# zhoujun-7/VPHO

Hardware: AMD Instinct MI355X
Metric: eval images/sec (bs=64, sample_num=100, steps=50); MPJPE delta vs ref (higher is better)
Workload: dtype f32; 1 GPU; vpho_net.forward(mode=predict), README eval config (BASELINE.json configs[1]); per_gpu_batch=64, sample_num=100, sampling_steps=50, topk_hand=30, topk_obj=10, crop=256x256, pipeline_depth=3, parallelism=dp1, score_mfma=f32, conv_mfma=f32, winograd_3x3=True

## Files before the change

include/vpho_hip.h:

```cpp
#ifndef VPHO_HIP_H
#define VPHO_HIP_H

#if defined(__GNUC__) || defined(__clang__)
#define VPHO_API __attribute__((visibility("default")))
#else
#define VPHO_API
#endif

#ifdef __cplusplus
extern "C" {
#endif

VPHO_API const char* vpho_last_error(void);
VPHO_API int vpho_abi_version(void);

VPHO_API int vpho_prof_enable(int kernel_class, int on);
VPHO_API int vpho_prof_collect(int kernel_class, double* total_ms, long long* launches, double* total_flops, double* total_bytes);

typedef struct {
    const float* x; const float* w; const float* bias;
    const float* in_scale; const float* in_shift;
    const float* res; float* y;
    int N, H, W, Cin, x_ld;
    int Cout, KH, KW, stride, pad_y, pad_x, OH, OW;
    long long y_sn, y_sy, y_sx;
    long long r_sn, r_sy, r_sx;
    float in_slope, out_slope;
    int w_ld, splits;
    long long x_split, w_split, y_split;
    const float* gate;
    float gate_slope;
    const int* row_map;
    const int* row_count;
    int rows_hint;
    int rows_scatter;
    const void* w_planes;
    int plane_terms;
    const float* res_up;
    int ru_H, ru_W, ru_ld;
    const float* x2;
    int Cin2, x2_ld, stride2, H2, W2;
    int groups;
    long long x_group, w_group, bias_group, y_group, res_group, x2_group, pre_group, ru_group;
    float* stats;
    int* stats_rows;
    int stats_cap;
    const float* bn_x; const float* bn_mean; const float* bn_invstd; const float* bn_gamma; const float* bn_beta;
} vpho_conv_desc;
VPHO_API int vpho_conv2d_nhwc_f32(const vpho_conv_desc* d, void* stream);
VPHO_API int vpho_conv3x3_winograd_nhwc_f32(const float* x, const float* u, const float* bias, int N, int H, int W, int Cin, int x_ld, int Cout,
                                   float out_slope, float* y, int y_ld, void* stream);
VPHO_API int vpho_conv3x3_winograd_grouped_nhwc_f32(const float* x, long long x_group, const float* u, const float* bias, int groups, int N, int H, int W,
                                           int Cin, int x_ld, int Cout, float out_slope, float* y, int y_ld, void* stream);
VPHO_API int vpho_winograd_window_tiles_i32(const int* wins, int N, int* tile_base, void* stream);
VPHO_API int vpho_conv3x3_winograd_scatter_nhwc_f32(const float* x, const float* u, const float* bias, int N, int H, int W, int Cin, int x_ld, int Cout,
                                           float out_slope, const int* wins, const int* tile_base, float* y, int y_ld, void* stream);
VPHO_API int vpho_winograd_weights_f32(const float* w_packed, int Cout, int Cin, int for_input_gradient, float* u, void* stream);
VPHO_API int vpho_winograd_weights_multi_f32(const void* segments, int n_segments, long long total_blocks, void* stream);
VPHO_API int vpho_conv3x3_winograd_gate_nhwc_f32(const float* x, const float* u, const float* gate, float gate_slope, int N, int H, int W, int Cin,
                                        int x_ld, int Cout, float* y, int y_ld, void* stream);
VPHO_API int vpho_conv3x3_winograd_stats_nhwc_f32(const float* x, const float* u, const float* bias, int N, int H, int W, int Cin, int x_ld, int Cout,
                                         float out_slope, float* y, int y_ld, float* stats, int stats_cap, int* stats_rows, const float* bn_x,
                                         const float* bn_mean, const float* bn_invstd, const float* bn_gamma, const float* bn_beta,
                                         float gate_slope, void* stream);
VPHO_API int vpho_conv3x3_winograd_rows_nhwc_f32(const float* x, const float* u, const float* bias, int N, int H, int W, int Cin, int x_ld, int Cout,
                                        float out_slope, const int* wins, const int* tile_base, int tiles_hint, float* y_rows, int y_ld,
                                        void* stream);

typedef struct {
    int D, Dp, nheads;
    const float *t_W, *t_w, *t_b, *pe0_w, *pe0_b, *pe2_w, *pe2_b, *w1_t, *w1_p, *w1_f, *b1, *w2, *b2;
    const void* w1_p_split;
    int split_terms;
} vpho_score_weights;

VPHO_API long long vpho_score_workspace_bytes(const vpho_score_weights* w, int bs, int S);

VPHO_API int vpho_score_eval(const vpho_score_weights* w, const float* feat_img, int bs, int S, const float* x, float t,
                    float* out, void* workspace, long long workspace_bytes, void* stream);

typedef struct {
    int nfev;
    int n_accepted, n_rejected;
    int nan_count;
    int status;
    int n_log;
} vpho_ode_stats;

VPHO_API int vpho_ode_sample(const vpho_score_weights* w, const float* feat_img, int bs, int S, const float* init_x,
                    double T0, double eps, int num_steps, double rtol, double atol,
                    void* xs_out, int xs_is_f64, void* x_out, int x_is_f64,
                    void* workspace, long long workspace_bytes,
                    vpho_ode_stats* stats_host, double* step_log_host, int step_log_cap, void* stream);

VPHO_API int vpho_nchw_to_nhwc_f32(const float* x, int N, int C, int H, int W, float* y, int ldy, void* stream);
VPHO_API int vpho_nhwc_to_nchw_f32(const float* x, int N, int H, int W, int C, int ldx, float* y, void* stream);
VPHO_API int vpho_maxpool_nhwc_f32(const float* x, int N, int H, int W, int C, int k, int stride, int pad, float* y, void* stream);
VPHO_API int vpho_resize_bilinear_nhwc_f32(const float* x, int N, int H, int W, int C, int ldx, int OH, int OW,
                                  float* y, int ldy, int c_off, int accumulate, void* stream);
VPHO_API int vpho_roi_align_nhwc_f32(const float* feat, int N, int H, int W, int C, const float* boxes, float spatial_scale,
                            int out_size, const unsigned char* flip_w, float* out, int ldo, int c_off, void* stream);
VPHO_API int vpho_roi_windows_i32(const float* boxes_a, const float* boxes_b, int N, int H, int W, float spatial_scale, int dilate,
                         int* wins, int* row_map, int* row_count, void* stream);
VPHO_API int vpho_resize_bilinear_rows_nhwc_f32(const float* x, int N, int H, int W, int C, int ldx, int OH, int OW, float* y, int ldy, int c_off,
                                       int accumulate, const int* row_map, const int* row_count, int rows_hint, void* stream);
VPHO_API int vpho_roi_align_window_nhwc_f32(const float* feat_rows, const int* wins, int N, int H, int W, int C, const float* boxes,
                                   float spatial_scale, int out_size, const unsigned char* flip_w, float* out, int ldo, int c_off, int rows_hint,
                                   void* stream);
VPHO_API int vpho_roi_align_window_dual_nhwc_f32(const float* feat_rows, const int* wins, int N, int H, int W, int C, const float* boxes,
                                        float spatial_scale, int out_size, const unsigned char* flip_w, float* out, int ldo, int c_off,
                                        const unsigned char* flip_w2, float* out2, int ldo2, int c_off2, int rows_hint, void* stream);
VPHO_API int vpho_align_heatmap_nhwc_f32(const float* hm, int N, int size, int C, const float* bbox, const float* bbox_rect,
                                const unsigned char* flip_w, float* out, void* stream);
VPHO_API int vpho_linear_acc64_f32(const float* x, int rows, int cin, int ld_x, const float* w, const float* bias, int cout, float out_slope,
                          float* y, int ld_y, void* stream);
VPHO_API int vpho_nerf_embed_f32(const float* g, int N, const unsigned char* flip_x, float* out, void* stream);
VPHO_API int vpho_cross_tokens_f32(const float* proj_hand, const float* proj_obj, const float* grav_emb, const float* pe,
                          int bs, float* out, void* stream);
VPHO_API int vpho_mha_f32(const float* qkv, int S, int B, int E, int nhead, float* out, void* stream);
VPHO_API int vpho_mha_dropout_f32(const float* qkv, int S, int B, int E, int nhead, const float* drop_mask, float* out, void* stream);
VPHO_API int vpho_add_layernorm_f32(const float* x, const float* r, const float* gamma, const float* beta, long long rows, int E,
                           float eps, float* out, void* stream);
VPHO_API int vpho_force_local_f32(const float* scale, int ld_scale, const float* logits, int ld_logits, const float* anchor,
                         float friction, long long rows, int group, int group_stride, int off_scale, int off_logits,
                         float* out, void* stream);
VPHO_API int vpho_rot6d_to_axis_angle_f32(const float* x, long long rows, int rot_per_row, int ldx, float* out, int ldo, void* stream);
VPHO_API int vpho_append_betas_f32(const float* betas, long long rows, long long rows_per_image, float* out, int ldo, void* stream);

typedef struct {
    const float *v_template;
    const float *shapedirs;
    const float *posedirs_t;
    const float *J_regressor;
    const float *weights;
    const float *tip_posedirs_t;
    const float *posedirs_mfma;
} vpho_mano_tables;
VPHO_API int vpho_mano_shape_f32(const vpho_mano_tables* t, const float* betas, int n_img, float* v_shaped, float* J, void* stream);
VPHO_API int vpho_mano_fk_f32(const vpho_mano_tables* t, const float* pose, int ld_pose, long long n_hands, int hands_per_image,
                     const float* v_shaped, const float* J, const unsigned char* ho3d_per_image,
                     float* verts, float* joints, void* stream);

typedef struct { const float* kpt; const float* vert; const float* com; int n_kpt, n_vert, n_obj; } vpho_obj_tables;
typedef struct { const int* face_idx; const float* anchor_weight; const float* vert2joint; const int* skeleton; } vpho_anchor_tables;

VPHO_API int vpho_hand_candidates_f32(const float* diff_pose, int ld_diff, const float* reg_pose, int bs, int S, float* pose, void* stream);
VPHO_API int vpho_hand_heat_f32(const float* joints, const float* root, const float* Kmat, const float* bbox, const float* heatmap,
                       int bs, int C, int J, int H, int W, const int* observe_host, int n_obs, float* out, void* stream);
VPHO_API int vpho_hand_fuse_level_f32(const float* hv, int n_obs, float* pose, int bs, int C, int k, int level,
                             float* val, int* idx, float* topk_pose, float* score_out, void* stream);
VPHO_API int vpho_topk_f32(const float* scores, int rows_outer, int n, int F, int k, float* val, int* idx, void* stream);
VPHO_API int vpho_topk_weights_f32(const float* val, int rows, int k, float* w, void* stream);
VPHO_API int vpho_obj_heat_score(const double* pose, int n, const double* transl_override, const float* root, const vpho_obj_tables* t,
                        const int* obj_id, const unsigned char* is_right, const float* Kmat, const float* bbox,
                        const float* heatmap, int bs, int H, int W, float* score, void* stream);
VPHO_API int vpho_obj_cross_candidates(const double* pose, int n, const int* transl_idx, const int* rot_idx, int bs, int ko, double* cand, void* stream);
VPHO_API int vpho_obj_physics_score(const double* cand, int n, const float* root, const vpho_obj_tables* t, const int* obj_id,
                           const unsigned char* is_right, const float* force_point, const float* force_global, int bs,
                           float* score, void* stream);
VPHO_API int vpho_obj_fuse_f64(const double* pose, int n, const int* idx_a, const float* w_a, const int* idx_b, const float* w_b,
                      const unsigned char* pick_b, int bs, int k, double* fused, void* stream);
VPHO_API int vpho_obj_verts_f32(const double* pose, const float* root, const vpho_obj_tables* t, const int* obj_id,
                       const unsigned char* is_right, int bs, float* out, void* stream);
VPHO_API int vpho_force_anchor_f32(const vpho_anchor_tables* t, const float* verts, const float* root, const float* force_local,
                          long long n_hands, int hands_per_image, float* force_point, float* force_global, void* stream);
VPHO_API int vpho_hand_phys_candidates_f32(const float* agg_pose, int ld_agg, const float* betas, const float* topk_pose, int bs, int k,
                                  float* out, void* stream);
VPHO_API int vpho_hand_phys_score_f32(const float* force_point, const float* force_global, const float* obj_vert, int n_vert,
                             int bs, int n_cand, float* finger_score, void* stream);
VPHO_API int vpho_hand_phys_fuse_f32(const float* cand, int n_cand, const int* idx, int bs, int k, float* out, void* stream);

VPHO_API int vpho_heatmap_peak_f32(const float* heatmap, long long n_maps, int H, int W, float* peak, int* ind, void* stream);
VPHO_API int vpho_hand_pt2d_score_f32(const float* joints, const float* root, const float* Kmat, const float* bbox, const float* peak,
                             int bs, int C, int per_joint, float* score, void* stream);
VPHO_API int vpho_obj_pt2d_score(const double* pose, int n, const float* root, const vpho_obj_tables* t, const int* obj_id,
                        const unsigned char* is_right, const float* Kmat, const float* bbox, const float* peak, int bs,
                        float* score, void* stream);
VPHO_API int vpho_hand_pose_fuse_f32(const float* pose, int ld_pose, int C, const int* idx, const float* w, int bs, int n, float* fused,
                            void* stream);
VPHO_API int vpho_hand_joint_gather_mean_f32(const float* joints, const int* idx, int bs, int C, int k, float* fused, void* stream);

VPHO_API int vpho_hand_metrics_f32(const float* pd, const float* gt, int n_img, int n_pts, float* mean_err, float* pa_mean_err,
                          float* per_point, void* stream);

typedef struct vpho_obj_metric_tables {
    const double* bbox3d;
    const double* verts_sampled;
    const double* verts;
    const int* vert_offset;
    const double* diameter;
    int n_obj, n_sampled;
} vpho_obj_metric_tables;
VPHO_API int vpho_obj_9d_to_rt_f64(const double* pose9, const float* root_joint, int n, double* rt, void* stream);
VPHO_API long long vpho_obj_metrics_workspace_bytes(const vpho_obj_metric_tables* t, int n_img, int max_verts);
VPHO_API int vpho_obj_metrics_f64(const vpho_obj_metric_tables* t, const double* pd_rt, const double* gt_rt, const double* cam_intr,
                         const int* obj_id, int n_img, int max_verts, double* out, void* workspace, long long workspace_bytes,
                         void* stream);

VPHO_API int vpho_hand_metrics_multi_f32(const float* pd, const float* gt, const float* root_joint, const unsigned char* is_right, int n_img,
                                int n_hyp, int n_pts, float* mean_err, float* pa_mean_err, void* stream);
VPHO_API long long vpho_obj_metrics_multi_workspace_bytes(const vpho_obj_metric_tables* t, int n_img, int n_hyp, int max_verts);
VPHO_API int vpho_obj_metrics_multi_f64(const vpho_obj_metric_tables* t, const double* pd_rt, const double* gt_rt, const double* cam_intr,
                               const int* obj_id, int n_img, int n_hyp, int max_verts, double* out, double* best, double* mean,
                               void* workspace, long long workspace_bytes, void* stream);

VPHO_API int vpho_hand_bench_multi_f32(const float* pd, const float* gt, const float* root_joint, const unsigned char* is_right, int n_img,
                              int n_hyp, int n_pts, double f_thresh_lo, double f_thresh_hi, const double* auc_thresh, const double* auc_g,
                              int n_thresh, int with_fscore, double* values, int* counts, void* stream);
VPHO_API int vpho_hand_bench_table_f64(const double* per, int n_img, int n_hyp, double* one, double* best, double* mean, void* stream);

VPHO_API long long vpho_infer_record_bytes(int n_joint, int n_vert);
VPHO_API int vpho_infer_pack_f32(const float* reg_hand_joint, const float* reg_hand_vert, const float* agg_hand_joint, const float* agg_hand_vert,
                        const double* agg_obj_6d, const float* root_joint, const unsigned char* is_right, int n_img, int n_joint,
                        int n_vert, void* records, void* records_host, void* stream);

#define VPHO_PEN_TRI_STRIDE 28
#define VPHO_PEN_RESOLUTION 512
typedef struct vpho_obj_mesh_tables {
    const double* tri;
    const int* tri_offset;
    const double* scale;
    const double* translate;
    int n_obj;
} vpho_obj_mesh_tables;
VPHO_API int vpho_hand_obj_penetration_f64(const vpho_obj_mesh_tables* t, const float* verts, int n, int V, const double* obj_rt,
                                  const int* obj_id, double contact_thresh, double* sd, unsigned char* inside, double* per_image,
                                  void* stream);

#define VPHO_PEN_COLUMNS 64
#define VPHO_PEN_CLUSTER 16
typedef struct vpho_obj_mesh_accel {
    const int* col_offset;
    const int* col_tri;
    const int* clu_offset;
    const double* clu_sphere;
    const double* clu_geo;
} vpho_obj_mesh_accel;
VPHO_API int vpho_hand_obj_penetration_multi_f64(const vpho_obj_mesh_tables* t, const vpho_obj_mesh_accel* acc, const float* verts, int n, int S,
                                        int V, const double* obj_rt, const int* obj_id, double contact_thresh, double* per_hyp,
                                        double* sd, unsigned char* inside, double* table, void* stream);

#define VPHO_VOL_TRI_STRIDE 19
typedef struct vpho_obj_solids {
    const float* pts;
    const int* pt_offset;
    int n_obj, max_pts;
} vpho_obj_solids;
VPHO_API long long vpho_hand_obj_intersection_workspace_bytes(int n, int F);
VPHO_API int vpho_hand_obj_intersection_f64(const vpho_obj_mesh_tables* t, const vpho_obj_solids* solids, const int* faces, int F, const float* verts,
                                   int n, int V, const double* obj_rt, const int* obj_id, double pitch, double* out, unsigned char* flags,
                                   void* workspace, long long workspace_bytes, void* stream);
typedef struct vpho_obj_solid_columns {
    const int* col_start;
    const int* col_offset;
    int n_obj, max_cols;
} vpho_obj_solid_columns;
VPHO_API long long vpho_hand_obj_intersection_multi_workspace_bytes(int n, int S, int F);
VPHO_API int vpho_hand_obj_intersection_multi_f64(const vpho_obj_mesh_tables* t, const vpho_obj_solids* solids, const vpho_obj_solid_columns* cols,
        const int* faces, int F, const float* verts , int n, int S, int V, const double* obj_rt ,
        const int* obj_id , double pitch, double* per_hyp , double* table ,
        unsigned char* flags , void* workspace, long long workspace_bytes, void* stream);

VPHO_API int vpho_anchor_frames_f32(const vpho_anchor_tables* t, const float* verts, long long n_hands, float* pts, float* frames, void* stream);
VPHO_API int vpho_force_optimize_f32(const float* pts, const float* frames, const float* gravity, const float* com, const float* force_contact,
                            const unsigned char* is_grasped, int n_batches, int B, int iters, int phase1_iters, float lr,
                            float* force_local, float* force_global, float* scale, float* weight, float* losses, void* stream);
// ... 84 lines not shown
```

vpho_amd/csrc/metrics.hip:

```cpp
#include <type_traits>
#include "common.h"
#include "rot.h"
#include "procrustes.h"
#include <algorithm>
#include "../../include/vpho_hip.h"

namespace {

using vpho::sym3_eig;
using vpho::wave_sum;
using vpho::similarity_from_cov;

__device__ inline double block_sum(double v, double* red) {
    const int tid = threadIdx.x;
    red[tid] = v;
    __syncthreads();
    for (int o = blockDim.x / 2; o > 0; o >>= 1) {
        if (tid < o) red[tid] += red[tid + o];
        __syncthreads();
    }
    const double r = red[0];
    __syncthreads();
    return r;
}

__global__ __launch_bounds__(256) void hand_metrics_kernel(const float* __restrict__ pd, const float* __restrict__ gt, int n,
                                                           float* __restrict__ mean_err, float* __restrict__ pa_mean_err,
                                                           float* __restrict__ per_point) {
    __shared__ double red[256];
    __shared__ double T[12];
    const int b = blockIdx.x, tid = threadIdx.x;
    const float* A = pd + (long long)b * n * 3;
    const float* B = gt + (long long)b * n * 3;
    double sa[3] = {0, 0, 0}, sb[3] = {0, 0, 0}, se = 0;
    for (int i = tid; i < n; i += 256) {
        double d2 = 0;
        for (int c = 0; c < 3; ++c) { sa[c] += A[i * 3 + c]; sb[c] += B[i * 3 + c]; const double d = (double)B[i * 3 + c] - A[i * 3 + c]; d2 += d * d; }
        const double e = sqrt(d2);
        se += e;
        if (per_point) per_point[(long long)b * n + i] = (float)e;
    }
    double cA[3], cB[3];
    for (int c = 0; c < 3; ++c) { cA[c] = block_sum(sa[c], red) / n; cB[c] = block_sum(sb[c], red) / n; }
    const double me = block_sum(se, red) / n;
    double h[9] = {0}, va = 0;
    for (int i = tid; i < n; i += 256) {
        double a[3], bb[3];
        for (int c = 0; c < 3; ++c) { a[c] = A[i * 3 + c] - cA[c]; bb[c] = B[i * 3 + c] - cB[c]; va += a[c] * a[c]; }
        for (int r = 0; r < 3; ++r) for (int c = 0; c < 3; ++c) h[r * 3 + c] += a[r] * bb[c];
    }
    double H[3][3];
    for (int k = 0; k < 9; ++k) H[k / 3][k % 3] = block_sum(h[k], red) / n;
    const double varA = block_sum(va, red) / n;
    if (tid == 0) {
        double M[3][3], w[3], V[3][3], U[3][3], s[3];
        for (int i = 0; i < 3; ++i) for (int j = 0; j < 3; ++j) { M[i][j] = 0; for (int k = 0; k < 3; ++k) M[i][j] += H[k][i] * H[k][j]; }
        sym3_eig(M, w, V);
        for (int k = 0; k < 3; ++k) s[k] = sqrt(w[k] > 0 ? w[k] : 0.0);
        for (int k = 0; k < 3; ++k) {
            double u[3] = {0, 0, 0};
            for (int i = 0; i < 3; ++i) for (int j = 0; j < 3; ++j) u[i] += H[i][j] * V[j][k];
            const double nu = sqrt(u[0] * u[0] + u[1] * u[1] + u[2] * u[2]);
            if (k < 2 || nu > 1e-12 * (s[0] + 1e-300)) for (int i = 0; i < 3; ++i) U[i][k] = u[i] / (nu > 0 ? nu : 1.0);
            else {
                U[0][2] = U[1][0] * U[2][1] - U[2][0] * U[1][1];
                U[1][2] = U[2][0] * U[0][1] - U[0][0] * U[2][1];
                U[2][2] = U[0][0] * U[1][1] - U[1][0] * U[0][1];
            }
        }
        auto build = [&](double R[3][3]) { for (int i = 0; i < 3; ++i) for (int j = 0; j < 3; ++j) { R[i][j] = 0; for (int k = 0; k < 3; ++k) R[i][j] += V[i][k] * U[j][k]; } };
        double R[3][3];
        build(R);
        const double det = R[0][0] * (R[1][1] * R[2][2] - R[1][2] * R[2][1]) - R[0][1] * (R[1][0] * R[2][2] - R[1][2] * R[2][0]) +
                           R[0][2] * (R[1][0] * R[2][1] - R[1][1] * R[2][0]);
        if (det < 0) { s[2] = -s[2]; for (int i = 0; i < 3; ++i) V[i][2] = -V[i][2]; build(R); }
        const double c = (s[0] + s[1] + s[2]) / varA;
        for (int i = 0; i < 3; ++i) {
            double t = cB[i];
            for (int j = 0; j < 3; ++j) { T[i * 3 + j] = c * R[i][j]; t -= c * R[i][j] * cA[j]; }
            T[9 + i] = t;
        }
    }
    __syncthreads();
    double sp = 0;
    for (int i = tid; i < n; i += 256) {
        double d2 = 0;
        for (int r = 0; r < 3; ++r) {
            const double al = T[r * 3] * A[i * 3] + T[r * 3 + 1] * A[i * 3 + 1] + T[r * 3 + 2] * A[i * 3 + 2] + T[9 + r];
            const double d = (double)B[i * 3 + r] - al;
            d2 += d * d;
        }
        sp += sqrt(d2);
    }
    const double pa = block_sum(sp, red) / n;
    if (tid == 0) { mean_err[b] = (float)me; pa_mean_err[b] = (float)pa; }
}

__global__ void obj_9d_to_rt_kernel(const double* __restrict__ pose9, const float* __restrict__ root, int n, double* __restrict__ rt) {
    const int i = blockIdx.x * blockDim.x + threadIdx.x;
    if (i >= n) return;
    vpho::obj_9d_to_rt(pose9 + (long long)i * 9, root + (long long)i * 3, rt + (long long)i * 12);
}

struct ObjWs { float *pd_s, *gt_s, *pd_f, *gt_f, *d_s, *d_p2g, *d_g2p; long long bytes; };

__host__ __device__ inline long long ows_align(long long v) { return (v + 255) / 256 * 256; }

inline ObjWs obj_carve(int n_img, int ns, int vmax, char* base) {
    long long off = 0;
    ObjWs w;
    auto take = [&](long long b) { char* p = base ? base + off : nullptr; off += ows_align(b); return (float*)p; };
    w.pd_s = take((long long)n_img * ns * 12); w.gt_s = take((long long)n_img * ns * 12);
    w.pd_f = take((long long)n_img * vmax * 12); w.gt_f = take((long long)n_img * vmax * 12);
    w.d_s = take((long long)n_img * ns * 4); w.d_p2g = take((long long)n_img * vmax * 4); w.d_g2p = take((long long)n_img * vmax * 4);
    w.bytes = off;
    return w;
}

__device__ inline void rt_apply(const double* rt, const double* v, double* o) {
    for (int r = 0; r < 3; ++r) o[r] = v[0] * rt[r * 4 + 0] + v[1] * rt[r * 4 + 1] + v[2] * rt[r * 4 + 2] + rt[r * 4 + 3];
}

__global__ __launch_bounds__(256) void obj_transform_kernel(const vpho_obj_metric_tables t, const double* __restrict__ pd_rt,
                                                            const double* __restrict__ gt_rt, const int* __restrict__ obj_id,
                                                            int vmax, ObjWs w) {
    const int b = blockIdx.x, o = obj_id[b];
    const int nf = t.vert_offset[o + 1] - t.vert_offset[o];
    const int i = blockIdx.y * 256 + threadIdx.x;
    if (i >= t.n_sampled + nf) return;
    const bool full = i >= t.n_sampled;
    const int k = full ? i - t.n_sampled : i;
    const double* v = full ? t.verts + ((long long)t.vert_offset[o] + k) * 3 : t.verts_sampled + ((long long)o * t.n_sampled + k) * 3;
    double p[3], g[3];
    rt_apply(pd_rt + (long long)b * 12, v, p);
    rt_apply(gt_rt + (long long)b * 12, v, g);
    float* po = full ? w.pd_f + ((long long)b * vmax + k) * 3 : w.pd_s + ((long long)b * t.n_sampled + k) * 3;
    float* go = full ? w.gt_f + ((long long)b * vmax + k) * 3 : w.gt_s + ((long long)b * t.n_sampled + k) * 3;
    for (int c = 0; c < 3; ++c) { po[c] = (float)p[c]; go[c] = (float)g[c]; }
}

__global__ __launch_bounds__(256) void obj_nn_kernel(const vpho_obj_metric_tables t, const int* __restrict__ obj_id, int vmax, ObjWs w) {
    __shared__ float tile[256 * 3];
    const int b = blockIdx.x, job = blockIdx.y, o = obj_id[b];
    const int n = job == 0 ? t.n_sampled : t.vert_offset[o + 1] - t.vert_offset[o];
    const int ld = job == 0 ? t.n_sampled : vmax;
    const float* src = (job == 0 ? w.pd_s : job == 1 ? w.pd_f : w.gt_f) + (long long)b * ld * 3;
    const float* dst = (job == 0 ? w.gt_s : job == 1 ? w.gt_f : w.pd_f) + (long long)b * ld * 3;
    float* out = (job == 0 ? w.d_s : job == 1 ? w.d_p2g : w.d_g2p) + (long long)b * ld;
    if (blockIdx.z * 256 >= n) return;
    const int i = blockIdx.z * 256 + threadIdx.x;
    const bool live = i < n;
    const float x = live ? src[i * 3] : 0.f, y = live ? src[i * 3 + 1] : 0.f, z = live ? src[i * 3 + 2] : 0.f;
    float best = INFINITY;
    for (int j0 = 0; j0 < n; j0 += 256) {
        const int m = min(256, n - j0);
        __syncthreads();
        for (int q = threadIdx.x; q < m * 3; q += 256) tile[q] = dst[(long long)j0 * 3 + q];
        __syncthreads();
        for (int j = 0; j < m; ++j) {
            const float dx = x - tile[j * 3], dy = y - tile[j * 3 + 1], dz = z - tile[j * 3 + 2];
            const float d2 = (dx * dx + dy * dy) + dz * dz;
            best = d2 < best ? d2 : best;
        }
    }
    if (live) out[i] = sqrtf(best);
}

__device__ inline float block_minmax(float v, bool is_max, float* red) {
    const int tid = threadIdx.x;
    red[tid] = v;
    __syncthreads();
    for (int o = blockDim.x / 2; o > 0; o >>= 1) {
        if (tid < o) red[tid] = is_max ? fmaxf(red[tid], red[tid + o]) : fminf(red[tid], red[tid + o]);
        __syncthreads();
    }
    const float r = red[0];
    __syncthreads();
    return r;
// ... 292 lines not shown
    }
    double s_add = 0, s_rep = 0;
    float mn[2][3], mx[2][3];
    for (int c = 0; c < 3; ++c) { mn[0][c] = mn[1][c] = INFINITY; mx[0][c] = mx[1][c] = -INFINITY; }
    for (int i = tid; i < ns; i += 256) {
        double p[3], g[3], pp[2], gp[2];
        const double* v = t.verts_sampled + ((long long)o * ns + i) * 3;
        rt_apply(prt, v, p);
        rt_apply(grt, v, g);
        float pf[3], gf[3];
        for (int c = 0; c < 3; ++c) { pf[c] = (float)p[c]; gf[c] = (float)g[c]; }
        const float dx = pf[0] - gf[0], dy = pf[1] - gf[1], dz = pf[2] - gf[2];
        s_add += (double)sqrtf((dx * dx + dy * dy) + dz * dz);
        for (int c = 0; c < 3; ++c) {
            mn[0][c] = fminf(mn[0][c], pf[c]); mx[0][c] = fmaxf(mx[0][c], pf[c]);
            mn[1][c] = fminf(mn[1][c], gf[c]); mx[1][c] = fmaxf(mx[1][c], gf[c]);
        }
        for (int r = 0; r < 2; ++r) {
            pp[r] = (p[0] * K[r * 3] + p[1] * K[r * 3 + 1] + p[2] * K[r * 3 + 2]) / (p[2] + 1e-7);
            gp[r] = (g[0] * K[r * 3] + g[1] * K[r * 3 + 1] + g[2] * K[r * 3 + 2]) / (g[2] + 1e-7);
        }
        s_rep += sqrt((pp[0] - gp[0]) * (pp[0] - gp[0]) + (pp[1] - gp[1]) * (pp[1] - gp[1]));
    }
    const double add = block_sum(s_add, red) / ns, rep = block_sum(s_rep, red) / ns;
    float bmn[2][3], bmx[2][3];
    for (int k = 0; k < 2; ++k)
        for (int c = 0; c < 3; ++c) { bmn[k][c] = block_minmax(mn[k][c], false, redf); bmx[k][c] = block_minmax(mx[k][c], true, redf); }
    if (tid == 0) {
        double acc[3][7];
        for (int j = 0; j < 3; ++j)
            for (int c = 0; c < 7; ++c) {
                double a = 0;
                for (int q = 0; q < w.chunks; ++q) a += w.part[(((long long)bs * 3 + j) * w.chunks + q) * 8 + c];
                acc[j][c] = a;
            }
        const double adds = acc[0][0] / ns, mp = acc[1][0] / nf, mg = acc[2][0] / nf;
        const int sel[3][8] = {{0, 1, 0, 0, 1, 0, 1, 1}, {0, 0, 1, 0, 1, 1, 0, 1}, {0, 0, 0, 1, 0, 1, 1, 1}};
        float s2 = 0.f;
        for (int k = 0; k < 8; ++k) {
            float d2 = 0.f;
            for (int c = 0; c < 3; ++c) {
                const float a = sel[c][k] ? bmx[0][c] : bmn[0][c], g = sel[c][k] ? bmx[1][c] : bmn[1][c];
                d2 += (a - g) * (a - g);
            }
            s2 += sqrtf(d2);
        }
        const double diam = t.diameter[o];
        double* r = out + (long long)bs * 16;
        r[0] = mce; r[1] = oce; r[2] = (double)(s2 / 8.f); r[3] = add; r[4] = adds;
        r[5] = add <= diam * 0.1 ? 1.0 : 0.0; r[6] = adds <= diam * 0.1 ? 1.0 : 0.0; r[7] = rep; r[8] = rep < 5 ? 1.0 : 0.0;
        r[9] = 0.5 * (mp + mg);
        for (int k = 0; k < 6; ++k) {
            const float prec = (float)(acc[1][1 + k] / nf), rec = (float)(acc[2][1 + k] / nf);
            r[10 + k] = (double)((2.f * prec * rec) / ((prec + rec) + 1e-6f));
        }
    }
}

__global__ void obj_multi_reduce_kernel(const double* __restrict__ per, int n_img, int S, double* __restrict__ best, double* __restrict__ mean) {
    const int i = blockIdx.x * blockDim.x + threadIdx.x;
    if (i >= n_img * 16) return;
    const int b = i / 16, c = i % 16;
    const bool is_max = c == 5 || c == 6 || c == 8 || c >= 10;
    const double* p = per + (long long)b * S * 16 + c;
    double bv = p[0], sv = p[0];
    for (int s = 1; s < S; ++s) {
        const double v = p[(long long)s * 16];
        bv = is_max ? (v > bv ? v : bv) : (v < bv ? v : bv);
        sv += v;
    }
    if (best) best[i] = bv;
    if (mean) mean[i] = sv / S;
}

}

extern "C" int vpho_hand_metrics_f32(const float* pd, const float* gt, int n_img, int n_pts, float* mean_err, float* pa_mean_err,
                                     float* per_point, void* stream) {
    VPHO_REQUIRE(pd && gt && mean_err && pa_mean_err && n_img > 0 && n_pts >= 3, "vpho_hand_metrics_f32: bad argument");
    hipLaunchKernelGGL(hand_metrics_kernel, dim3(n_img), dim3(256), 0, (hipStream_t)stream, pd, gt, n_pts, mean_err, pa_mean_err, per_point);
    return vpho::check_launch("hand_metrics_kernel");
}

extern "C" long long vpho_obj_metrics_workspace_bytes(const vpho_obj_metric_tables* t, int n_img, int max_verts) {
    if (!t || n_img <= 0 || max_verts <= 0 || t->n_sampled <= 0) return -1;
    return obj_carve(n_img, t->n_sampled, max_verts, nullptr).bytes;
}

extern "C" int vpho_obj_metrics_f64(const vpho_obj_metric_tables* t, const double* pd_rt, const double* gt_rt, const double* cam_intr,
                                    const int* obj_id, int n_img, int max_verts, double* out, void* workspace, long long workspace_bytes,
                                    void* stream) {
    VPHO_REQUIRE(t && t->bbox3d && t->verts_sampled && t->verts && t->vert_offset && t->diameter && t->n_obj > 0 && t->n_sampled > 0,
                 "vpho_obj_metrics_f64: bad tables");
    VPHO_REQUIRE(pd_rt && gt_rt && cam_intr && obj_id && out && workspace && n_img > 0 && max_verts > 0, "vpho_obj_metrics_f64: bad argument");
    const ObjWs w = obj_carve(n_img, t->n_sampled, max_verts, (char*)workspace);
    VPHO_REQUIRE(workspace_bytes >= w.bytes, "vpho_obj_metrics_f64: workspace %lld < %lld bytes", workspace_bytes, w.bytes);
    hipStream_t s = (hipStream_t)stream;
    const int pts = t->n_sampled + max_verts;
    hipLaunchKernelGGL(obj_transform_kernel, dim3(n_img, (pts + 255) / 256), dim3(256), 0, s, *t, pd_rt, gt_rt, obj_id, max_verts, w);
    const int chunks = (std::max(t->n_sampled, max_verts) + 255) / 256;
    hipLaunchKernelGGL(obj_nn_kernel, dim3(n_img, 3, chunks), dim3(256), 0, s, *t, obj_id, max_verts, w);
    hipLaunchKernelGGL(obj_metrics_kernel, dim3(n_img), dim3(256), 0, s, *t, pd_rt, gt_rt, cam_intr, obj_id, max_verts, w, out);
    return vpho::check_launch("obj_metrics kernels");
}

extern "C" int vpho_obj_9d_to_rt_f64(const double* pose9, const float* root_joint, int n, double* rt, void* stream) {
    VPHO_REQUIRE(pose9 && root_joint && rt && n > 0, "vpho_obj_9d_to_rt_f64: bad argument");
    hipLaunchKernelGGL(obj_9d_to_rt_kernel, dim3((n + 255) / 256), dim3(256), 0, (hipStream_t)stream, pose9, root_joint, n, rt);
    return vpho::check_launch("obj_9d_to_rt_kernel");
}

extern "C" int vpho_hand_metrics_multi_f32(const float* pd, const float* gt, const float* root_joint, const unsigned char* is_right, int n_img,
                                           int n_hyp, int n_pts, float* mean_err, float* pa_mean_err, void* stream) {
    VPHO_REQUIRE(pd && gt && root_joint && is_right && mean_err && pa_mean_err && n_img > 0 && n_hyp > 0 && n_pts >= 3 &&
                 (long long)n_img * n_hyp <= 0x7fffffff, "vpho_hand_metrics_multi_f32: bad argument");
    hipLaunchKernelGGL(hand_metrics_multi_kernel, dim3(n_img * n_hyp), dim3(64), 0, (hipStream_t)stream, pd, gt, root_joint, is_right, n_hyp,
                       n_pts, mean_err, pa_mean_err);
    return vpho::check_launch("hand_metrics_multi_kernel");
}

extern "C" long long vpho_obj_metrics_multi_workspace_bytes(const vpho_obj_metric_tables* t, int n_img, int n_hyp, int max_verts) {
    if (!t || n_img <= 0 || n_hyp <= 0 || max_verts <= 0 || t->n_sampled <= 0 || (long long)n_img * n_hyp > 0x7fffffff) return -1;
    return mh_carve(n_img, n_hyp, t->n_sampled, max_verts, nullptr).bytes;
}

extern "C" int vpho_obj_metrics_multi_f64(const vpho_obj_metric_tables* t, const double* pd_rt, const double* gt_rt, const double* cam_intr,
                                          const int* obj_id, int n_img, int n_hyp, int max_verts, double* out, double* best, double* mean,
                                          void* workspace, long long workspace_bytes, void* stream) {
    VPHO_REQUIRE(t && t->bbox3d && t->verts_sampled && t->verts && t->vert_offset && t->diameter && t->n_obj > 0 && t->n_sampled > 0,
                 "vpho_obj_metrics_multi_f64: bad tables");
    VPHO_REQUIRE(pd_rt && gt_rt && cam_intr && obj_id && out && workspace && n_img > 0 && n_hyp > 0 && max_verts > 0 &&
                 (long long)n_img * n_hyp <= 0x7fffffff, "vpho_obj_metrics_multi_f64: bad argument");
    const MhWs w = mh_carve(n_img, n_hyp, t->n_sampled, max_verts, (char*)workspace);
    VPHO_REQUIRE(workspace_bytes >= w.bytes, "vpho_obj_metrics_multi_f64: workspace %lld < %lld bytes", workspace_bytes, w.bytes);
    VPHO_REQUIRE(w.chunks <= 65535, "vpho_obj_metrics_multi_f64: %d query chunks exceed the grid", w.chunks);
    hipStream_t s = (hipStream_t)stream;
    const int rows = n_img * n_hyp;
    hipLaunchKernelGGL(obj_multi_nn_kernel, dim3(rows, 3, w.chunks), dim3(256), 0, s, *t, pd_rt, gt_rt, obj_id, n_hyp, w);
    hipLaunchKernelGGL(obj_multi_metrics_kernel, dim3(rows), dim3(256), 0, s, *t, pd_rt, gt_rt, cam_intr, obj_id, n_hyp, w, out);
    if (best || mean)
        hipLaunchKernelGGL(obj_multi_reduce_kernel, dim3((n_img * 16 + 255) / 256), dim3(256), 0, s, out, n_img, n_hyp, best, mean);
    return vpho::check_launch("obj_metrics_multi kernels");
}
```

vpho_amd/csrc/misc.hip:

```cpp
#include "common.h"
#include <cstdint>
#include "rot.h"
#include "../../include/vpho_hip.h"

namespace {

inline int nblocks(long long n, int bs = 256) { return (int)((n + bs - 1) / bs); }

__global__ void nchw_to_nhwc_kernel(const float* __restrict__ x, int N, int C, int H, int W, float* __restrict__ y, int ldy) {
    const long long i = (long long)blockIdx.x * blockDim.x + threadIdx.x;
    const long long total = (long long)N * H * W * ldy;
    if (i >= total) return;
    const int c = (int)(i % ldy);
    const long long p = i / ldy;
    const long long hw = (long long)H * W;
    const long long n = p / hw, r = p - n * hw;
    y[i] = c < C ? x[(n * C + c) * hw + r] : 0.f;
}

__global__ void nhwc_to_nchw_kernel(const float* __restrict__ x, int N, int H, int W, int C, int ldx, float* __restrict__ y) {
    const long long i = (long long)blockIdx.x * blockDim.x + threadIdx.x;
    const long long hw = (long long)H * W, total = (long long)N * C * hw;
    if (i >= total) return;
    const long long r = i % hw;
    const long long nc = i / hw;
    const int c = (int)(nc % C);
    const long long n = nc / C;
    y[i] = x[(n * hw + r) * ldx + c];
}

__global__ void maxpool_nhwc_kernel(const float* __restrict__ x, int N, int H, int W, int C, int k, int stride, int pad,
                                    int OH, int OW, float* __restrict__ y) {
    const long long i = (long long)blockIdx.x * blockDim.x + threadIdx.x;
    const long long total = (long long)N * OH * OW * C;
    if (i >= total) return;
    const int c = (int)(i % C);
    long long p = i / C;
    const int ox = (int)(p % OW); p /= OW;
    const int oy = (int)(p % OH);
    const long long n = p / OH;
    float m = -INFINITY;
    for (int r = 0; r < k; ++r) {
        const int iy = oy * stride - pad + r;
        if (iy < 0 || iy >= H) continue;
        for (int s = 0; s < k; ++s) {
            const int ix = ox * stride - pad + s;
            if (ix < 0 || ix >= W) continue;
            m = fmaxf(m, x[((n * H + iy) * W + ix) * C + c]);
        }
    }
    y[i] = m;
}


template <int V>
__device__ inline void ldv(const float* __restrict__ p, float (&o)[V]) {
    if constexpr (V == 4) { const f32x4 t = *reinterpret_cast<const f32x4*>(p); o[0] = t[0]; o[1] = t[1]; o[2] = t[2]; o[3] = t[3]; }
    else o[0] = *p;
}
template <int V>
__device__ inline void stv(float* __restrict__ p, const float (&v)[V]) {
    if constexpr (V == 4) { f32x4 t; t[0] = v[0]; t[1] = v[1]; t[2] = v[2]; t[3] = v[3]; *reinterpret_cast<f32x4*>(p) = t; }
    else *p = v[0];
}

template <int V>
__global__ void resize_bilinear_nhwc_kernel(const float* __restrict__ x, int N, int H, int W, int C, int ldx, int OH, int OW,
                                            float* __restrict__ y, int ldy, int c_off, int accumulate,
                                            const int* __restrict__ row_map, const int* __restrict__ row_count) {
    const long long i = (long long)blockIdx.x * blockDim.x + threadIdx.x;
    const int CV = C / V;
    const long long total = (long long)N * OH * OW * CV;
    if (i >= total) return;
    const int c = (int)(i % CV) * V;
    long long p = i / CV;
    if (row_map) {
        if (p >= *row_count) return;
        p = row_map[p];
    }
    const int ox = (int)(p % OW); p /= OW;
    const int oy = (int)(p % OH);
    const long long n = p / OH;
    int y0, y1, x0, x1; float ly, lx;
    lin_src(oy, (float)H / (float)OH, H, y0, y1, ly);
    lin_src(ox, (float)W / (float)OW, W, x0, x1, lx);
    const float hy = 1.f - ly, hx = 1.f - lx;
    const float* b = x + n * H * W * (long long)ldx + c;
    float a00[V], a01[V], a10[V], a11[V], o[V];
    ldv<V>(b + ((long long)y0 * W + x0) * ldx, a00); ldv<V>(b + ((long long)y0 * W + x1) * ldx, a01);
    ldv<V>(b + ((long long)y1 * W + x0) * ldx, a10); ldv<V>(b + ((long long)y1 * W + x1) * ldx, a11);
    float* op = y + ((n * OH + oy) * OW + ox) * (long long)ldy + c_off + c;
    if (accumulate) ldv<V>(op, o);
#pragma unroll
    for (int u = 0; u < V; ++u) {
        const float v = hy * (hx * a00[u] + lx * a01[u]) + ly * (hx * a10[u] + lx * a11[u]);
        o[u] = accumulate ? (o[u] + v) : v;
    }
    stv<V>(op, o);
}

struct RoiWin { int base, y0, x0, w, h; };

template <int V>
__device__ inline void roi_bilinear(const float* __restrict__ f, int H, int W, int ld, float y, float x, float (&acc)[V],
                                    const RoiWin* win = nullptr) {
    if (y < -1.0f || y > (float)H || x < -1.0f || x > (float)W) {
#pragma unroll
        for (int u = 0; u < V; ++u) acc[u] += 0.f;
        return;
    }
    if (y <= 0.f) y = 0.f;
    if (x <= 0.f) x = 0.f;
    int yl = (int)y, xl = (int)x, yh, xh;
    if (yl >= H - 1) { yh = yl = H - 1; y = (float)yl; } else yh = yl + 1;
    if (xl >= W - 1) { xh = xl = W - 1; x = (float)xl; } else xh = xl + 1;
    const float ly = y - (float)yl, lx = x - (float)xl, hy = 1.f - ly, hx = 1.f - lx;
    float a[V], b[V], c[V], d[V];
    if (win) {
        const int wy0 = min(max(yl - win->y0, 0), win->h - 1), wy1 = min(max(yh - win->y0, 0), win->h - 1);
        const int wx0 = min(max(xl - win->x0, 0), win->w - 1), wx1 = min(max(xh - win->x0, 0), win->w - 1);
        ldv<V>(f + ((long long)wy0 * win->w + wx0) * ld, a); ldv<V>(f + ((long long)wy0 * win->w + wx1) * ld, b);
        ldv<V>(f + ((long long)wy1 * win->w + wx0) * ld, c); ldv<V>(f + ((long long)wy1 * win->w + wx1) * ld, d);
    } else {
        ldv<V>(f + ((long long)yl * W + xl) * ld, a); ldv<V>(f + ((long long)yl * W + xh) * ld, b);
        ldv<V>(f + ((long long)yh * W + xl) * ld, c); ldv<V>(f + ((long long)yh * W + xh) * ld, d);
    }
#pragma unroll
    for (int u = 0; u < V; ++u) acc[u] += hy * hx * a[u] + hy * lx * b[u] + ly * hx * c[u] + ly * lx * d[u];
}

template <int V>
__global__ void roi_align_nhwc_kernel(const float* __restrict__ feat, int N, int H, int W, int C, const float* __restrict__ boxes,
                                      float scale, int P, const unsigned char* __restrict__ flip_w,
                                      float* __restrict__ out, int ldo, int c_off, const RoiWin* __restrict__ wins,
                                      float* __restrict__ out2 = nullptr, int ldo2 = 0, int c_off2 = 0, const unsigned char* __restrict__ flip_w2 = nullptr) {
    const long long i = (long long)blockIdx.x * blockDim.x + threadIdx.x;
    const int CV = C / V;
    const long long total = (long long)N * P * P * CV;
    if (i >= total) return;
    const int c = (int)(i % CV) * V;
    long long p = i / CV;
    const int pw = (int)(p % P); p /= P;
    const int ph = (int)(p % P);
    const int n = (int)(p / P);
    const float x1 = boxes[n * 4 + 0] * scale, y1 = boxes[n * 4 + 1] * scale;
    const float x2 = boxes[n * 4 + 2] * scale, y2 = boxes[n * 4 + 3] * scale;
    const float rw = fmaxf(x2 - x1, 1.f), rh = fmaxf(y2 - y1, 1.f);
    const float bh = rh / (float)P, bw = rw / (float)P;
    const int gh = (int)ceilf(rh / (float)P), gw = (int)ceilf(rw / (float)P);
    const float cnt = fmaxf((float)(gh * gw), 1.f);
    RoiWin win;
    if (wins) win = wins[n];
    const float* f = feat + (wins ? (long long)win.base : (long long)n * H * W) * C + c;
    float acc[V];
#pragma unroll
    for (int u = 0; u < V; ++u) acc[u] = 0.f;
    for (int iy = 0; iy < gh; ++iy) {
        const float y = y1 + ph * bh + ((float)iy + 0.5f) * bh / (float)gh;
        for (int ix = 0; ix < gw; ++ix) {
            const float x = x1 + pw * bw + ((float)ix + 0.5f) * bw / (float)gw;
            roi_bilinear<V>(f, H, W, C, y, x, acc, wins ? &win : nullptr);
        }
    }
    const int ow = (flip_w && flip_w[n]) ? P - 1 - pw : pw;
#pragma unroll
    for (int u = 0; u < V; ++u) acc[u] = acc[u] / cnt;
    stv<V>(out + (((long long)n * P + ph) * P + ow) * ldo + c_off + c, acc);
    if (out2) {
        const int ow2 = (flip_w2 && flip_w2[n]) ? P - 1 - pw : pw;
        stv<V>(out2 + (((long long)n * P + ph) * P + ow2) * ldo2 + c_off2 + c, acc);
    }
}

__global__ __launch_bounds__(256) void roi_window_kernel(const float* __restrict__ boxes_a, const float* __restrict__ boxes_b, int N, int H, int W,
                                                         float scale, int dilate, RoiWin* __restrict__ wins, int* __restrict__ count) {
    for (int n0 = 0; n0 < N; n0 += 256) {
        const int n = n0 + threadIdx.x;
        if (n < N) {
            float lo_x = 3.0e38f, lo_y = 3.0e38f, hi_x = -3.0e38f, hi_y = -3.0e38f;
            for (int k = 0; k < 2; ++k) {
                const float* b = k == 0 ? boxes_a : boxes_b;
// ... 276 lines not shown
                                   const float* __restrict__ anchor, float friction, long long rows, int group, int group_stride,
                                   int off_scale, int off_logits, float* __restrict__ out) {
    const long long r = (long long)blockIdx.x * blockDim.x + threadIdx.x;
    if (r >= rows) return;
    const long long base = (r / group) * group_stride + r % group;
    const long long rs = base + off_scale, rl = base + off_logits;
    float w[8];
    for (int pass = 0; pass < 2; ++pass) {
        float mx = -INFINITY;
        for (int i = 0; i < 8; ++i) { if (pass == 0) w[i] = logits[rl * ld_logits + i]; mx = fmaxf(mx, w[i]); }
        float s = 0.f;
        for (int i = 0; i < 8; ++i) { w[i] = expf(w[i] - mx); s += w[i]; }
        for (int i = 0; i < 8; ++i) w[i] /= s;
    }
    float d[3] = {0.f, 0.f, 0.f};
    for (int i = 0; i < 8; ++i) {
        d[0] += w[i] * (anchor[i * 3 + 0] * friction);
        d[1] += w[i] * (anchor[i * 3 + 1] * friction);
        d[2] += w[i] * anchor[i * 3 + 2];
    }
    const float nrm = sqrtf(d[0] * d[0] + d[1] * d[1] + d[2] * d[2]) + 1e-8f;
    const float sc = fabsf(scale[rs * ld_scale]);
    for (int k = 0; k < 3; ++k) out[r * 3 + k] = d[k] / nrm * sc;
}

__global__ void rot6d_to_aa_kernel(const float* __restrict__ x, long long n_rot, int rot_per_row, int ldx, float* __restrict__ out, int ldo) {
    const long long i = (long long)blockIdx.x * blockDim.x + threadIdx.x;
    if (i >= n_rot) return;
    const long long row = i / rot_per_row;
    const int j = (int)(i - row * rot_per_row);
    float R[9], q[4], aa[3];
    vpho::rot6d_to_matrix(x + row * ldx + 6 * j, R);
    vpho::matrix_to_quaternion(R, q);
    vpho::quaternion_to_axis_angle(q, aa);
    float* o = out + row * ldo + 3 * j;
    o[0] = aa[0]; o[1] = aa[1]; o[2] = aa[2];
}

__global__ void append_betas_kernel(const float* __restrict__ betas, long long rows, long long rows_per_image, float* __restrict__ out, int ldo) {
    const long long i = (long long)blockIdx.x * blockDim.x + threadIdx.x;
    if (i >= rows * 10) return;
    const long long row = i / 10;
    const int k = (int)(i - row * 10);
    out[row * ldo + 48 + k] = betas[(row / rows_per_image) * 10 + k];
}

}

#define LAUNCH1D(kernel, total, stream, ...) \
    hipLaunchKernelGGL(kernel, dim3(nblocks(total)), dim3(256), 0, (hipStream_t)(stream), __VA_ARGS__)

extern "C" int vpho_nchw_to_nhwc_f32(const float* x, int N, int C, int H, int W, float* y, int ldy, void* stream) {
    VPHO_REQUIRE(x && y && N > 0 && C > 0 && H > 0 && W > 0 && ldy >= C, "vpho_nchw_to_nhwc_f32: bad argument");
    LAUNCH1D(nchw_to_nhwc_kernel, (long long)N * H * W * ldy, stream, x, N, C, H, W, y, ldy);
    return vpho::check_launch("nchw_to_nhwc_kernel");
}

extern "C" int vpho_nhwc_to_nchw_f32(const float* x, int N, int H, int W, int C, int ldx, float* y, void* stream) {
    VPHO_REQUIRE(x && y && N > 0 && C > 0 && H > 0 && W > 0 && ldx >= C, "vpho_nhwc_to_nchw_f32: bad argument");
    LAUNCH1D(nhwc_to_nchw_kernel, (long long)N * H * W * C, stream, x, N, H, W, C, ldx, y);
    return vpho::check_launch("nhwc_to_nchw_kernel");
}

extern "C" int vpho_maxpool_nhwc_f32(const float* x, int N, int H, int W, int C, int k, int stride, int pad, float* y, void* stream) {
    VPHO_REQUIRE(x && y && N > 0 && C > 0 && k > 0 && stride > 0 && pad >= 0 && 2 * pad <= k, "vpho_maxpool_nhwc_f32: bad argument");
    const int OH = (H + 2 * pad - k) / stride + 1, OW = (W + 2 * pad - k) / stride + 1;
    VPHO_REQUIRE(OH > 0 && OW > 0, "vpho_maxpool_nhwc_f32: empty output");
    LAUNCH1D(maxpool_nhwc_kernel, (long long)N * OH * OW * C, stream, x, N, H, W, C, k, stride, pad, OH, OW, y);
    return vpho::check_launch("maxpool_nhwc_kernel");
}

extern "C" int vpho_resize_bilinear_nhwc_f32(const float* x, int N, int H, int W, int C, int ldx, int OH, int OW,
                                             float* y, int ldy, int c_off, int accumulate, void* stream) {
    VPHO_REQUIRE(x && y && N > 0 && C > 0 && H > 0 && W > 0 && OH > 0 && OW > 0 && ldx >= C && ldy >= c_off + C && c_off >= 0,
                 "vpho_resize_bilinear_nhwc_f32: bad argument");
    vpho::ProfScope prof(vpho::PROF_RESIZE, (hipStream_t)stream, 0.0, 4.0 * N * C * ((double)H * W + (double)OH * OW * (accumulate ? 2 : 1)));
    if (C % 4 == 0 && ldx % 4 == 0 && ldy % 4 == 0 && c_off % 4 == 0 && ((uintptr_t)x | (uintptr_t)y) % 16 == 0)
        LAUNCH1D(resize_bilinear_nhwc_kernel<4>, (long long)N * OH * OW * (C / 4), stream, x, N, H, W, C, ldx, OH, OW, y, ldy, c_off, accumulate, (const int*)nullptr, (const int*)nullptr);
    else
        LAUNCH1D(resize_bilinear_nhwc_kernel<1>, (long long)N * OH * OW * C, stream, x, N, H, W, C, ldx, OH, OW, y, ldy, c_off, accumulate, (const int*)nullptr, (const int*)nullptr);
    return vpho::check_launch("resize_bilinear_nhwc_kernel");
}

extern "C" int vpho_resize_bilinear_rows_nhwc_f32(const float* x, int N, int H, int W, int C, int ldx, int OH, int OW, float* y, int ldy, int c_off,
                                                  int accumulate, const int* row_map, const int* row_count, int rows_hint, void* stream) {
    VPHO_REQUIRE(x && y && row_map && row_count && N > 0 && H > 0 && W > 0 && C > 0 && OH > 0 && OW > 0 && ldx >= C && ldy >= c_off + C && c_off >= 0,
                 "vpho_resize_bilinear_rows_nhwc_f32: bad argument");
    const double px = rows_hint > 0 ? (double)rows_hint : (double)N * OH * OW;
    vpho::ProfScope prof(vpho::PROF_RESIZE, (hipStream_t)stream, 0.0, 4.0 * C * ((double)N * H * W + px * (accumulate ? 2 : 1)));
    if (C % 4 == 0 && ldx % 4 == 0 && ldy % 4 == 0 && c_off % 4 == 0 && ((uintptr_t)x | (uintptr_t)y) % 16 == 0)
        LAUNCH1D(resize_bilinear_nhwc_kernel<4>, (long long)N * OH * OW * (C / 4), stream, x, N, H, W, C, ldx, OH, OW, y, ldy, c_off, accumulate, row_map, row_count);
    else
        LAUNCH1D(resize_bilinear_nhwc_kernel<1>, (long long)N * OH * OW * C, stream, x, N, H, W, C, ldx, OH, OW, y, ldy, c_off, accumulate, row_map, row_count);
    return vpho::check_launch("resize_bilinear_nhwc_kernel(rows)");
}

extern "C" int vpho_roi_align_nhwc_f32(const float* feat, int N, int H, int W, int C, const float* boxes, float spatial_scale,
                                       int out_size, const unsigned char* flip_w, float* out, int ldo, int c_off, void* stream) {
    VPHO_REQUIRE(feat && boxes && out && N > 0 && C > 0 && out_size > 0 && ldo >= c_off + C && c_off >= 0, "vpho_roi_align_nhwc_f32: bad argument");
    vpho::ProfScope prof(vpho::PROF_ROI_ALIGN, (hipStream_t)stream, 0.0, 4.0 * N * C * ((double)H * W + (double)out_size * out_size));
    if (C % 4 == 0 && ldo % 4 == 0 && c_off % 4 == 0 && ((uintptr_t)feat | (uintptr_t)out) % 16 == 0)
        LAUNCH1D(roi_align_nhwc_kernel<4>, (long long)N * out_size * out_size * (C / 4), stream, feat, N, H, W, C, boxes, spatial_scale, out_size, flip_w, out, ldo, c_off, (const RoiWin*)nullptr);
    else
        LAUNCH1D(roi_align_nhwc_kernel<1>, (long long)N * out_size * out_size * C, stream, feat, N, H, W, C, boxes, spatial_scale, out_size, flip_w, out, ldo, c_off, (const RoiWin*)nullptr);
    return vpho::check_launch("roi_align_nhwc_kernel");
}

extern "C" int vpho_roi_windows_i32(const float* boxes_a, const float* boxes_b, int N, int H, int W, float spatial_scale, int dilate,
                                    int* wins, int* row_map, int* row_count, void* stream) {
    VPHO_REQUIRE(boxes_a && wins && row_map && row_count && N > 0 && H > 0 && W > 0 && dilate >= 0, "vpho_roi_windows_i32: bad argument");
    VPHO_REQUIRE((long long)N * H * W < (1ll << 31), "vpho_roi_windows_i32: map too large");
    static_assert(sizeof(RoiWin) == 5 * sizeof(int), "window record = 5 ints");
    hipStream_t s = (hipStream_t)stream;
    hipLaunchKernelGGL(roi_window_kernel, dim3(1), dim3(256), 0, s, boxes_a, boxes_b, N, H, W, spatial_scale, dilate, (RoiWin*)wins, row_count);
    hipLaunchKernelGGL(roi_rows_kernel, dim3((H * W + 255) / 256, N), dim3(256), 0, s, (const RoiWin*)wins, H, W, row_map);
    return vpho::check_launch("roi_window_kernel");
}

extern "C" int vpho_roi_align_window_nhwc_f32(const float* feat_rows, const int* wins, int N, int H, int W, int C, const float* boxes,
                                              float spatial_scale, int out_size, const unsigned char* flip_w, float* out, int ldo, int c_off,
                                              int rows_hint, void* stream) {
    VPHO_REQUIRE(feat_rows && wins && boxes && out && N > 0 && C > 0 && out_size > 0 && ldo >= c_off + C && c_off >= 0, "vpho_roi_align_window_nhwc_f32: bad argument");
    const double rows_read = rows_hint > 0 ? (double)rows_hint : (double)N * H * W;
    vpho::ProfScope prof(vpho::PROF_ROI_ALIGN, (hipStream_t)stream, 0.0, 4.0 * C * (rows_read + (double)N * out_size * out_size));
    if (C % 4 == 0 && ldo % 4 == 0 && c_off % 4 == 0 && ((uintptr_t)feat_rows | (uintptr_t)out) % 16 == 0)
        LAUNCH1D(roi_align_nhwc_kernel<4>, (long long)N * out_size * out_size * (C / 4), stream, feat_rows, N, H, W, C, boxes, spatial_scale, out_size, flip_w, out, ldo, c_off, (const RoiWin*)wins);
    else
        LAUNCH1D(roi_align_nhwc_kernel<1>, (long long)N * out_size * out_size * C, stream, feat_rows, N, H, W, C, boxes, spatial_scale, out_size, flip_w, out, ldo, c_off, (const RoiWin*)wins);
    return vpho::check_launch("roi_align_nhwc_kernel(window)");
}

extern "C" int vpho_roi_align_window_dual_nhwc_f32(const float* feat_rows, const int* wins, int N, int H, int W, int C, const float* boxes,
                                                   float spatial_scale, int out_size, const unsigned char* flip_w, float* out, int ldo, int c_off,
                                                   const unsigned char* flip_w2, float* out2, int ldo2, int c_off2, int rows_hint, void* stream) {
    VPHO_REQUIRE(feat_rows && wins && boxes && out && out2 && N > 0 && C > 0 && out_size > 0 && ldo >= c_off + C && c_off >= 0 && ldo2 >= c_off2 + C && c_off2 >= 0,
                 "vpho_roi_align_window_dual_nhwc_f32: bad argument");
    const double rows_read = rows_hint > 0 ? (double)rows_hint : (double)N * H * W;
    vpho::ProfScope prof(vpho::PROF_ROI_ALIGN, (hipStream_t)stream, 0.0, 4.0 * C * (rows_read + 2.0 * N * out_size * out_size));
    if (C % 4 == 0 && ldo % 4 == 0 && c_off % 4 == 0 && ldo2 % 4 == 0 && c_off2 % 4 == 0 && ((uintptr_t)feat_rows | (uintptr_t)out | (uintptr_t)out2) % 16 == 0)
        LAUNCH1D(roi_align_nhwc_kernel<4>, (long long)N * out_size * out_size * (C / 4), stream, feat_rows, N, H, W, C, boxes, spatial_scale, out_size, flip_w, out, ldo, c_off, (const RoiWin*)wins, out2, ldo2, c_off2, flip_w2);
    else
        LAUNCH1D(roi_align_nhwc_kernel<1>, (long long)N * out_size * out_size * C, stream, feat_rows, N, H, W, C, boxes, spatial_scale, out_size, flip_w, out, ldo, c_off, (const RoiWin*)wins, out2, ldo2, c_off2, flip_w2);
    return vpho::check_launch("roi_align_nhwc_kernel(window, two destinations)");
}

extern "C" int vpho_align_heatmap_nhwc_f32(const float* hm, int N, int size, int C, const float* bbox, const float* bbox_rect,
                                           const unsigned char* flip_w, float* out, void* stream) {
    VPHO_REQUIRE(hm && bbox && bbox_rect && out && N > 0 && size > 1 && C > 0, "vpho_align_heatmap_nhwc_f32: bad argument");
    LAUNCH1D(align_heatmap_kernel, (long long)N * size * size * C, stream, hm, N, size, C, bbox, bbox_rect, flip_w, out);
    return vpho::check_launch("align_heatmap_kernel");
}

extern "C" int vpho_nerf_embed_f32(const float* g, int N, const unsigned char* flip_x, float* out, void* stream) {
    VPHO_REQUIRE(g && out && N > 0, "vpho_nerf_embed_f32: bad argument");
    LAUNCH1D(nerf_embed_kernel, (long long)N * 64, stream, g, N, flip_x, out);
    return vpho::check_launch("nerf_embed_kernel");
}

extern "C" int vpho_cross_tokens_f32(const float* proj_hand, const float* proj_obj, const float* grav_emb, const float* pe,
                                     int bs, float* out, void* stream) {
    VPHO_REQUIRE(proj_hand && proj_obj && grav_emb && pe && out && bs > 0 && bs <= 5000, "vpho_cross_tokens_f32: bad argument");
    LAUNCH1D(cross_tokens_kernel, (long long)bs * 65 * 512, stream, proj_hand, proj_obj, grav_emb, pe, bs, out);
    return vpho::check_launch("cross_tokens_kernel");
}

extern "C" int vpho_mha_dropout_f32(const float* qkv, int S, int B, int E, int nhead, const float* drop_mask, float* out, void* stream) {
// ... 77 lines not shown
```

vpho_amd/csrc/score_ode.hip:

```cpp
#include "common.h"
#include <type_traits>
#include "../../include/vpho_hip.h"
#include <cmath>
#include <cstdlib>
#include <cstring>
#include <vector>
#include <mutex>
#include <unordered_map>
#include <algorithm>

VPHO_STAMP_DECL(head)

namespace {

#ifndef HEAD_ABLATE
#define HEAD_ABLATE 0
#endif
constexpr int HB_K = 16;
constexpr double SIGMA_MIN = 0.01, SIGMA_MAX = 50.0;

struct TimeList { float t[8]; };

struct RkCtl {
    double t, h_abs, h, t_new, err, dense_h;
// ... 954 lines not shown
    const int row = r0 + lrow_out;
    const bool live = row < a.R;
    const float* cim = a.cimg + (long long)(live ? row / a.S : 0) * a.NH + n * 256;
    float o0 = 0.f, o1 = 0.f, o2 = 0.f;
#pragma unroll
    for (int i = 0; i < TI; ++i) {
#pragma unroll
        for (int e = 0; e < 16; ++e) {
            const int j = 32 * TI * hh + 32 * i + (e & 3) + 8 * (e >> 2) + 4 * lh;
            const f32x4 t = *reinterpret_cast<const f32x4*>(Eb + j * 4);
            float h = acc[i][e] + cim[j] + t[0];
            h = h > 0.f ? h : 0.f;
            o0 += h * t[1]; o1 += h * t[2]; o2 += h * t[3];
        }
    }
    o0 += __shfl_xor(o0, 32);
    o1 += __shfl_xor(o1, 32);
    o2 += __shfl_xor(o2, 32);
    if (lh == 0) {
        float* ob = Ob + (hh * ROWS + lrow_out) * 4;
        ob[0] = o0; ob[1] = o1; ob[2] = o2;
    }
    __syncthreads();
    if (tid < ROWS) {
        const int orow = r0 + tid;
        float inv_std = a.inv_std_den, coef = a.coef;
        float* outp = a.out;
        if (a.ctl && a.ctl_mode == 1) {
            inv_std = a.ctl->inv_std[a.stage]; coef = a.ctl->coef[a.stage];
            outp = a.kbase + (long long)kslot(a.out_slot, a.ctl->kswap) * a.n_el;
        }
        if (orow < a.R) {
            int nans = 0;
#pragma unroll
            for (int dd = 0; dd < 3; ++dd) {
                float acc2 = Ob[tid * 4 + dd];
#pragma unroll
                for (int part = 1; part < PARTS; ++part) acc2 += Ob[(part * ROWS + tid) * 4 + dd];
                float sv = (acc2 + a.b2[n * 3 + dd]) / inv_std;
                if (a.rhs_mode) {
                    if (sv != sv) { sv = 0.f; ++nans; } else if (fabsf(sv) == INFINITY) sv = 0.f;
                    sv = 0.f - coef * sv;
                }
                outp[(long long)orow * a.D + n * 3 + dd] = sv;
            }
            if (nans) atomicAdd(a.nan_count, nans);
        }
    }
}

template <int TERMS>
__global__ __launch_bounds__(512) void score_head_split_kernel(const HeadArgs a) {
    extern __shared__ __attribute__((aligned(1024))) float smem[];
    if (ctl_skip(a.ctl, a.ctl_mode)) return;
    const int b = blockIdx.x, n_full = a.nheads * a.full_tiles;
    if (b < n_full) {
        head_tile_split<4, TERMS>(a, smem, b / a.full_tiles, (b % a.full_tiles) * 128);
    } else {
        const int q = b - n_full;
        head_tile_split<1, TERMS>(a, smem, q / a.tail_tiles, a.full_tiles * 128 + (q % a.tail_tiles) * 32);
    }
}

__global__ void stage_input_kernel(const double* __restrict__ y, KSlots ks, long long n_el, int D, int Dp,
                                   LinComb lc, float* __restrict__ X, double* __restrict__ ynew,
                                   const RkCtl* __restrict__ ctl, int ctl_mode, const double* ybuf0, const double* ybuf1) {
    if (ctl_skip(ctl, ctl_mode)) return;
    if (ctl && ctl_mode == 1) lc.h = ctl->h;
    if (ctl && ctl_mode == 2) y = ctl->parity ? ybuf1 : ybuf0;
    const long long i = (long long)blockIdx.x * blockDim.x + threadIdx.x;
    const long long R = n_el / D;
    if (i >= R * Dp) return;
    const long long r = i / Dp;
    const int c = (int)(i - r * Dp);
    if (c >= D) { X[i] = 0.f; return; }
    const long long e = r * D + c;
    double s = 0.0;
    for (int j = 0; j < lc.n; ++j) s += (double)ks.p[j][e] * lc.c[j];
    const double v = y[e] + s * lc.h;
    X[i] = (float)v;
    if (ynew) ynew[e] = v;
}

__global__ void f32_to_state_kernel(const float* __restrict__ x, long long n_el, int D, int Dp, double* __restrict__ y, float* __restrict__ X) {
    const long long i = (long long)blockIdx.x * blockDim.x + threadIdx.x;
    const long long R = n_el / D;
    if (i >= R * Dp) return;
    const long long r = i / Dp;
    const int c = (int)(i - r * Dp);
    if (c >= D) { X[i] = 0.f; return; }
    const float v = x[r * D + c];
    y[r * D + c] = (double)v;
    X[i] = v;
}

struct NormArgs {
    const double* y; const double* ynew; const float* Ka; const float* Kb; KSlots ks; long long n_el;
    double rtol, atol, h; double E[7]; int mode; double* partial;
    const RkCtl* ctl; const float* kbase; const double *ybuf0, *ybuf1;
};
__global__ __launch_bounds__(256) void norm_partial_kernel(const NormArgs a) {
    __shared__ double red[256];
    double s = 0.0;
    if (ctl_skip(a.ctl, 1)) return;
    KSlots ks = a.ks;
    const double *yv = a.y, *yn = a.ynew;
    double h = a.h;
    if (a.ctl) {
        const int par = a.ctl->parity, sw = a.ctl->kswap;
        yv = par ? a.ybuf1 : a.ybuf0; yn = par ? a.ybuf0 : a.ybuf1; h = a.ctl->h;
#pragma unroll
        for (int j = 0; j < 7; ++j) ks.p[j] = a.kbase + (long long)kslot(j, sw) * a.n_el;
    }
    for (long long i = (long long)blockIdx.x * 256 + threadIdx.x; i < a.n_el; i += (long long)gridDim.x * 256) {
        double v, scale;
        if (a.mode == 3) {
            double e = 0.0;
            for (int j = 0; j < 7; ++j) e += (double)ks.p[j][i] * a.E[j];
            v = e * h;
            scale = a.atol + fmax(fabs(yv[i]), fabs(yn[i])) * a.rtol;
        } else {
            scale = a.atol + fabs(yv[i]) * a.rtol;
            v = a.mode == 0 ? yv[i] : (a.mode == 1 ? (double)a.Ka[i] : (double)a.Kb[i] - (double)a.Ka[i]);
        }
        const double q = v / scale;
        s += q * q;
    }
    red[threadIdx.x] = s;
    __syncthreads();
    for (int o = 128; o > 0; o >>= 1) {
        if (threadIdx.x < o) red[threadIdx.x] += red[threadIdx.x + o];
        __syncthreads();
    }
    if (threadIdx.x == 0) a.partial[blockIdx.x] = red[0];
}
__global__ __launch_bounds__(256) void norm_final_kernel(const double* __restrict__ partial, int n, double* __restrict__ out,
                                                         const RkCtl* __restrict__ ctl) {
    __shared__ double red[256];
    if (ctl_skip(ctl, 1)) return;
    double s = 0.0;
    for (int i = threadIdx.x; i < n; i += 256) s += partial[i];
    red[threadIdx.x] = s;
    __syncthreads();
    for (int o = 128; o > 0; o >>= 1) {
        if (threadIdx.x < o) red[threadIdx.x] += red[threadIdx.x + o];
        __syncthreads();
    }
    if (threadIdx.x == 0) *out = red[0];
}

constexpr int DENSE_MAX = 48;
struct DenseArgs { double P[7][4]; double p[DENSE_MAX][4]; int idx[DENSE_MAX]; int n; double h; };
__global__ void dense_kernel(const double* __restrict__ y_old, KSlots ks, long long n_el, int D,
                             DenseArgs da, void* __restrict__ xs, int is_f64, int num_steps) {
    const long long i = (long long)blockIdx.x * blockDim.x + threadIdx.x;
    if (i >= n_el) return;
    double q[4];
    for (int m = 0; m < 4; ++m) {
        double s = 0.0;
        for (int j = 0; j < 7; ++j) s += (double)ks.p[j][i] * da.P[j][m];
        q[m] = s;
    }
    const double y0 = y_old[i];
    const long long r = i / D;
    const int c = (int)(i - r * D);
    for (int st = 0; st < da.n; ++st) {
        double acc = 0.0;
        for (int m = 0; m < 4; ++m) acc += q[m] * da.p[st][m];
        const double v = da.h * acc + y0;
        const long long o = (r * num_steps + da.idx[st]) * D + c;
        if (is_f64) reinterpret_cast<double*>(xs)[o] = v; else reinterpret_cast<float*>(xs)[o] = (float)v;
    }
}

// ... 119 lines not shown
__global__ void dense_ctl_kernel(const RkCtl* __restrict__ c, const double* ybuf0, const double* ybuf1, const float* __restrict__ kbase,
                                 long long n_el, int D, DenseP dp, void* __restrict__ xs, int is_f64, int num_steps) {
    const int first = c->dense_first, last = c->dense_last;
    if (first >= last) return;
    const long long i = (long long)blockIdx.x * blockDim.x + threadIdx.x;
    if (i >= n_el) return;
    const double* y_old = c->dense_parity ? ybuf1 : ybuf0;
    const int sw = c->dense_kswap;
    double q[4];
    for (int m = 0; m < 4; ++m) {
        double s = 0.0;
        for (int j = 0; j < 7; ++j) s += (double)kbase[(long long)kslot(j, sw) * n_el + i] * dp.P[j][m];
        q[m] = s;
    }
    const double y0 = y_old[i], h = c->dense_h;
    const long long r = i / D;
    const int cc = (int)(i - r * D);
    for (int st = first; st < last; ++st) {
        const double* p = c->dense_p + 4 * st;
        double acc = 0.0;
        for (int m = 0; m < 4; ++m) acc += q[m] * p[m];
        const double v = h * acc + y0;
        const long long o = (r * num_steps + st) * D + cc;
        if (is_f64) reinterpret_cast<double*>(xs)[o] = v; else reinterpret_cast<float*>(xs)[o] = (float)v;
    }
}

inline long long align_up(long long v) { return (v + 255) / 256 * 256; }

struct Workspace {
    float *cimg, *ct, *X, *P1, *P2, *K, *tmp;
    double *y, *ynew, *partial, *result;
    int* nan_count;
    RkCtl* ctl; double *te, *dense_p, *log;
    long long bytes;
};
constexpr int CTL_MAX_STEPS = 1024, CTL_LOG_CAP = 512;

Workspace carve(const vpho_score_weights& w, int bs, int S, char* base) {
    const long long R = (long long)bs * S, NH = (long long)w.nheads * 256;
    long long off = 0;
    Workspace ws;
    auto take = [&](long long b) { char* p = base ? base + off : nullptr; off += align_up(b); return p; };
    ws.cimg = (float*)take(bs * NH * 4);
    ws.ct = (float*)take(8 * NH * 4);
    ws.X = (float*)take(R * w.Dp * 4);
    ws.P1 = (float*)take(R * 256 * 4);
    ws.P2 = (float*)take(R * 256 * 4);
    ws.K = (float*)take(7 * R * w.D * 4);
    ws.tmp = (float*)take(R * w.D * 4);
    ws.y = (double*)take(R * w.D * 8);
    ws.ynew = (double*)take(R * w.D * 8);
    ws.partial = (double*)take(1024 * 8);
    ws.result = (double*)take(64);
    ws.nan_count = (int*)take(64);
    ws.ctl = (RkCtl*)take(sizeof(RkCtl));
    ws.te = (double*)take(CTL_MAX_STEPS * 8);
    ws.dense_p = (double*)take(CTL_MAX_STEPS * 4 * 8);
    ws.log = (double*)take(CTL_LOG_CAP * 4 * 8);
    ws.bytes = off;
    return ws;
}

int check_weights(const vpho_score_weights* w) {
    VPHO_REQUIRE(w != nullptr, "score weights: null");
    VPHO_REQUIRE(w->nheads > 0 && w->D == w->nheads * 3 && w->Dp >= w->D && w->Dp % 4 == 0, "score weights: D=%d Dp=%d nheads=%d inconsistent", w->D, w->Dp, w->nheads);
    VPHO_REQUIRE(w->t_W && w->t_w && w->t_b && w->pe0_w && w->pe0_b && w->pe2_w && w->pe2_b && w->w1_t && w->w1_p && w->w1_f && w->b1 && w->w2 && w->b2, "score weights: null tensor");
    return 0;
}

int linear(const float* x, int rows, int cin, const float* wt, const float* bias, int cout, float slope, float* y, hipStream_t s) {
    vpho_conv_desc d;
    memset(&d, 0, sizeof(d));
    d.x = x; d.w = wt; d.bias = bias; d.y = y;
    d.N = rows; d.H = 1; d.W = 1; d.Cin = cin; d.x_ld = cin; d.Cout = cout; d.KH = 1; d.KW = 1; d.stride = 1;
    d.OH = 1; d.OW = 1; d.y_sx = cout; d.y_sy = cout; d.y_sn = cout; d.in_slope = 1.f; d.out_slope = slope;
    return vpho_conv2d_nhwc_f32(&d, s);
}

float sigma_f32(float t) { return (float)SIGMA_MIN * (float)std::pow(SIGMA_MAX / SIGMA_MIN, (double)t); }

struct Ctx {
    const vpho_score_weights* w; Workspace ws; int bs, S; long long R, n_el; int NH; hipStream_t s;
};

int prepare_cimg(Ctx& c, const float* feat_img) {
    return linear(feat_img, c.bs, 1024, c.w->w1_f, c.w->b1, c.NH, 1.f, c.ws.cimg, c.s);
}

int embed_times(Ctx& c, const float* ts, int n, int ctl_mode = 0) {
    TimeList tl;
    for (int i = 0; i < 8; ++i) tl.t[i] = (ts && i < n) ? ts[i] : 0.f;
    hipLaunchKernelGGL(time_embed_kernel, dim3((c.NH + 255) / 256, n), dim3(256), 0, c.s, *c.w, tl, c.NH, c.ws.ct,
                       ctl_mode ? c.ws.ctl : (const RkCtl*)nullptr, ctl_mode);
    return vpho::check_launch("time_embed_kernel");
}

struct CtlCall { int mode = 0, stage = 0, out_slot = 0, write_ynew = 0; };

int eval_net(Ctx& c, const float* X, float t, int rhs_mode, float coef, float* out, int ct_slot = -1,
             const LinComb* lc = nullptr, const double* y = nullptr, double* ynew = nullptr, const KSlots* ks = nullptr,
             CtlCall cc = CtlCall()) {
    if (ct_slot < 0) {
        if (int e = embed_times(c, &t, 1, cc.mode == 2 ? 2 : 0)) return e;
        ct_slot = 0;
    }
    {
        PoseEncArgs pa;
        memset(&pa, 0, sizeof(pa));
        pa.X = X; pa.Dp = c.w->Dp; pa.w0 = c.w->pe0_w; pa.b0 = c.w->pe0_b; pa.w2 = c.w->pe2_w; pa.b2 = c.w->pe2_b;
        pa.out = c.ws.P2; pa.R = (int)c.R;
        if (lc) { pa.use_lc = 1; pa.lc = *lc; pa.y = y; if (ks) pa.ks = *ks; pa.D = c.w->D; pa.ynew = ynew; }
        pa.ctl = cc.mode ? c.ws.ctl : nullptr; pa.ctl_mode = cc.mode; pa.write_ynew = cc.write_ynew; pa.kbase = c.ws.K; pa.n_el = c.n_el;
        pa.ybuf0 = c.ws.y; pa.ybuf1 = c.ws.ynew;
        const int K1 = (pa.Dp + 31) / 32 * 32;
        const char* pe_env = getenv("VPHO_PE_RING");
        const bool pe_ring = pe_env && atoi(pe_env);
        const dim3 pe_grid((unsigned)((c.R + PE_ROWS - 1) / PE_ROWS));
        vpho::ProfScope pe_prof(vpho::PROF_POSE_ENC, c.s, 2.0 * (double)c.R * 256.0 * (K1 + 256.0), 0.0);
        if (pe_ring) {
            const size_t pe_lds = (size_t)(PE_NST * PE_STAGE + PE_ROWS * PE_H_LD + 512 + PE_ROWS * (K1 + 4)) * sizeof(float);
            VPHO_DYN_LDS(pose_encoder_kernel, 150 * 1024);
            VPHO_REQUIRE(pe_lds <= 150 * 1024, "pose encoder: input dimension %d too large for the LDS tile", pa.Dp);
            hipLaunchKernelGGL(pose_encoder_kernel, pe_grid, dim3(512), pe_lds, c.s, pa);
        } else {
            const size_t pe_lds = (size_t)(PE_ROWS * PE_H_LD + 512) * sizeof(float);
            VPHO_REQUIRE(K1 <= 128 && (pa.Dp & 3) == 0, "pose encoder: input dimension %d (padded %d) not supported (<= 128, multiple of 4)", c.w->D, pa.Dp);
            const char* rows_env = getenv("VPHO_PE_ROWS");
            const bool rows64 = rows_env ? atoi(rows_env) == 64 : c.R > 8192;
            if (rows64) {
                const size_t lds64 = (size_t)(2 * PE_ROWS * PE_H_LD + 512) * sizeof(float);
                const dim3 grid64((unsigned)((c.R + 2 * PE_ROWS - 1) / (2 * PE_ROWS)));
                VPHO_DYN_LDS(pose_encoder_reg64_kernel<1>, lds64); VPHO_DYN_LDS(pose_encoder_reg64_kernel<2>, lds64);
                VPHO_DYN_LDS(pose_encoder_reg64_kernel<3>, lds64); VPHO_DYN_LDS(pose_encoder_reg64_kernel<4>, lds64);
                switch (K1 / 32) {
                    case 1: hipLaunchKernelGGL(pose_encoder_reg64_kernel<1>, grid64, dim3(512), lds64, c.s, pa); break;
                    case 2: hipLaunchKernelGGL(pose_encoder_reg64_kernel<2>, grid64, dim3(512), lds64, c.s, pa); break;
                    case 3: hipLaunchKernelGGL(pose_encoder_reg64_kernel<3>, grid64, dim3(512), lds64, c.s, pa); break;
                    default: hipLaunchKernelGGL(pose_encoder_reg64_kernel<4>, grid64, dim3(512), lds64, c.s, pa); break;
                }
            } else
            switch (K1 / 32) {
                case 1: hipLaunchKernelGGL(pose_encoder_reg_kernel<1>, pe_grid, dim3(512), pe_lds, c.s, pa); break;
                case 2: hipLaunchKernelGGL(pose_encoder_reg_kernel<2>, pe_grid, dim3(512), pe_lds, c.s, pa); break;
                case 3: hipLaunchKernelGGL(pose_encoder_reg_kernel<3>, pe_grid, dim3(512), pe_lds, c.s, pa); break;
                default: hipLaunchKernelGGL(pose_encoder_reg_kernel<4>, pe_grid, dim3(512), pe_lds, c.s, pa); break;
            }
        }
        if (int e = vpho::check_launch("pose_encoder_kernel")) return e;
    }
    VPHO_REQUIRE((double)c.R * 256.0 * 4.0 < 4.0e9, "score head: %lld hypothesis rows exceed the 32-bit buffer offsets", (long long)c.R);
    HeadArgs a;
    a.w1p = c.w->w1_p; a.p2 = c.ws.P2; a.cimg = c.ws.cimg; a.ct = c.ws.ct + (long long)ct_slot * c.NH; a.w2 = c.w->w2; a.b2 = c.w->b2;
    a.out = out; a.nan_count = c.ws.nan_count; a.R = (int)c.R; a.S = c.S; a.NH = c.NH; a.D = c.w->D;
    a.inv_std_den = sigma_f32(t) + 1e-7f; a.coef = coef; a.rhs_mode = rhs_mode;
    a.ctl = cc.mode ? c.ws.ctl : nullptr; a.ctl_mode = cc.mode; a.stage = cc.stage; a.out_slot = cc.out_slot; a.kbase = c.ws.K; a.n_el = c.n_el;
    size_t lds = (size_t)(2 * (256 + 128) * HB_K + 256 * 4 + 2 * 128 * 4) * sizeof(float);
    if (getenv("VPHO_HEAD_LDS")) lds = (size_t)atoi(getenv("VPHO_HEAD_LDS"));
    VPHO_DYN_LDS(score_head_kernel<true>, lds);
    VPHO_DYN_LDS(score_head_kernel<false>, lds);
    VPHO_DYN_LDS(score_head_epi0_kernel<true>, lds);
    VPHO_DYN_LDS(score_head_epi0_kernel<false>, lds);
    static const int tail_on = getenv("VPHO_HEAD_TAIL") ? atoi(getenv("VPHO_HEAD_TAIL")) : 1;
    static int slots_of[64] = {0};
    int dev = 0;
    VPHO_HIP(hipGetDevice(&dev));
// ... 37 lines not shown
            return vpho::check_launch("score_head_pers_kernel");
        }
        const char* epi_s = getenv("VPHO_HEAD_EPI");
        if (epi_s && atoi(epi_s) == 0) {
            if (cb) hipLaunchKernelGGL(score_head_epi0_kernel<true>, grid, dim3(512), lds, c.s, a);
            else    hipLaunchKernelGGL(score_head_epi0_kernel<false>, grid, dim3(512), lds, c.s, a);
        } else if (cb) hipLaunchKernelGGL(score_head_kernel<true>, grid, dim3(512), lds, c.s, a);
        else           hipLaunchKernelGGL(score_head_kernel<false>, grid, dim3(512), lds, c.s, a);
    }
    return vpho::check_launch("score_head_kernel");
}

int eval_rhs(Ctx& c, const float* X, double t, float* out, int ct_slot = -1, const LinComb* lc = nullptr,
             const double* y = nullptr, double* ynew = nullptr, const KSlots* ks = nullptr, bool first_call = false) {
    const float tf = (float)t;
    const double sigma = first_call ? (double)sigma_f32(tf) : SIGMA_MIN * std::pow(SIGMA_MAX / SIGMA_MIN, t);
    const double g = sigma * std::sqrt(2.0 * (std::log(SIGMA_MAX) - std::log(SIGMA_MIN)));
    const float coef = (float)(0.5 * g * g);
    return eval_net(c, X, tf, 1, coef, out, ct_slot, lc, y, ynew, ks);
}

double* pinned_slot() {
    static thread_local double* p = nullptr;
    if (!p) { if (hipHostMalloc((void**)&p, 64, hipHostMallocDefault) != hipSuccess) p = nullptr; }
    return p;
}

int enqueue_norm(Ctx& c, NormArgs na, double* out_dev, bool ctl = false) {
    const int nb = (int)std::min<long long>(1024, (c.n_el + 255) / 256);
    na.n_el = c.n_el; na.partial = c.ws.partial;
    na.ctl = ctl ? c.ws.ctl : nullptr; na.kbase = c.ws.K; na.ybuf0 = c.ws.y; na.ybuf1 = c.ws.ynew;
    hipLaunchKernelGGL(norm_partial_kernel, dim3(nb), dim3(256), 0, c.s, na);
    hipLaunchKernelGGL(norm_final_kernel, dim3(1), dim3(256), 0, c.s, c.ws.partial, nb, out_dev, ctl ? c.ws.ctl : (const RkCtl*)nullptr);
    return vpho::check_launch("norm kernels");
}

int reduce_norm(Ctx& c, NormArgs na, double* value) {
    if (int e = enqueue_norm(c, na, c.ws.result)) return e;
    double* h = pinned_slot();
    VPHO_REQUIRE(h != nullptr, "hipHostMalloc failed");
    VPHO_HIP(hipMemcpyAsync(h, c.ws.result, 8, hipMemcpyDeviceToHost, c.s));
    VPHO_HIP(hipStreamSynchronize(c.s));
    *value = std::sqrt(*h) / std::sqrt((double)c.n_el);
    return 0;
}

const double RK_C[6] = {0, 1.0 / 5, 3.0 / 10, 4.0 / 5, 8.0 / 9, 1};
const double RK_A[6][5] = {
    {0, 0, 0, 0, 0},
    {1.0 / 5, 0, 0, 0, 0},
    {3.0 / 40, 9.0 / 40, 0, 0, 0},
    {44.0 / 45, -56.0 / 15, 32.0 / 9, 0, 0},
    {19372.0 / 6561, -25360.0 / 2187, 64448.0 / 6561, -212.0 / 729, 0},
    {9017.0 / 3168, -355.0 / 33, 46732.0 / 5247, 49.0 / 176, -5103.0 / 18656}};
const double RK_B[6] = {35.0 / 384, 0, 500.0 / 1113, 125.0 / 192, -2187.0 / 6784, 11.0 / 84};
const double RK_E[7] = {-71.0 / 57600, 0, 71.0 / 16695, -71.0 / 1920, 17253.0 / 339200, -22.0 / 525, 1.0 / 40};
const double RK_P[7][4] = {
    {1, -8048581381.0 / 2820520608, 8663915743.0 / 2820520608, -12715105075.0 / 11282082432},
    {0, 0, 0, 0},
    {0, 131558114200.0 / 32700410799, -68118460800.0 / 10900136933, 87487479700.0 / 32700410799},
    {0, -1754552775.0 / 470086768, 14199869525.0 / 1410260304, -10690763975.0 / 1880347072},
    {0, 127303824393.0 / 49829197408, -318862633887.0 / 49829197408, 701980252875.0 / 199316789632},
    {0, -282668133.0 / 205662961, 2019193451.0 / 616988883, -1453857185.0 / 822651844},
    {0, 40617522.0 / 29380423, -110615467.0 / 29380423, 69997945.0 / 29380423}};

}

extern "C" long long vpho_score_workspace_bytes(const vpho_score_weights* w, int bs, int S) {
    if (!w || bs <= 0 || S <= 0) return -1;
    return carve(*w, bs, S, nullptr).bytes;
}

extern "C" int vpho_score_eval(const vpho_score_weights* w, const float* feat_img, int bs, int S, const float* x, float t,
                               float* out, void* workspace, long long workspace_bytes, void* stream) {
    if (int e = check_weights(w)) return e;
    VPHO_REQUIRE(bs > 0 && S > 0 && feat_img && x && out && workspace, "vpho_score_eval: bad argument");
    Ctx c;
    c.w = w; c.bs = bs; c.S = S; c.R = (long long)bs * S; c.n_el = c.R * w->D; c.NH = w->nheads * 256; c.s = (hipStream_t)stream;
    c.ws = carve(*w, bs, S, (char*)workspace);
    VPHO_REQUIRE(workspace_bytes >= c.ws.bytes, "vpho_score_eval: workspace %lld < %lld bytes", workspace_bytes, c.ws.bytes);
    VPHO_HIP(hipMemsetAsync(c.ws.nan_count, 0, 4, c.s));
    if (int e = prepare_cimg(c, feat_img)) return e;
    const int nb = (int)((c.R * w->Dp + 255) / 256);
    hipLaunchKernelGGL(f32_to_state_kernel, dim3(nb), dim3(256), 0, c.s, x, c.n_el, w->D, w->Dp, c.ws.y, c.ws.X);
    return eval_net(c, c.ws.X, t, 0, 0.f, out);
}

namespace {

int ode_sample_host(Ctx& c, const float* feat_img, const float* init_x, double T0, double eps, int num_steps, double rtol, double atol,
                    void* xs_out, int xs_is_f64, void* x_out, int x_is_f64, vpho_ode_stats* st, double* step_log, int step_log_cap) {
    const vpho_score_weights* w = c.w;
    const long long n_el = c.n_el;
    const int D = w->D, Dp = w->Dp;
    const int nbX = (int)((c.R * Dp + 255) / 256), nbE = (int)((n_el + 255) / 256);
    KSlots ks;
    for (int j = 0; j < 7; ++j) ks.p[j] = c.ws.K + (long long)j * n_el;
    auto Kp = [&](int j) { return const_cast<float*>(ks.p[j]); };

    VPHO_HIP(hipMemsetAsync(c.ws.nan_count, 0, 4, c.s));
    if (int e = prepare_cimg(c, feat_img)) return e;
    double* y = c.ws.y;
    double* ynew = c.ws.ynew;
    hipLaunchKernelGGL(f32_to_state_kernel, dim3(nbX), dim3(256), 0, c.s, init_x, n_el, D, Dp, y, c.ws.X);

    std::vector<double> te(num_steps);
    {
        const int div = num_steps > 1 ? num_steps - 1 : 1;
        const double step = (eps - T0) / div;
        for (int i = 0; i < num_steps; ++i) te[i] = (double)i * step + T0;
        if (num_steps > 1) te[num_steps - 1] = eps;
    }
    const double direction = -1.0, tf = eps, max_step = 10.0;
    double t = T0;
    int next_idx = 0;
    auto log_step = [&](double tt, double hh, double err, int acc) {
        if (step_log && st->n_log < step_log_cap) {
            double* p = step_log + 4 * st->n_log;
            p[0] = tt; p[1] = hh; p[2] = err; p[3] = acc;
        }
        ++st->n_log;
    };

    if (int e = eval_rhs(c, c.ws.X, t, Kp(0), -1, nullptr, nullptr, nullptr, nullptr, true)) return e;
    ++st->nfev;
    double h_abs;
    {
        NormArgs na;
        memset(&na, 0, sizeof(na));
        na.y = y; na.rtol = rtol; na.atol = atol;
        double d0, d1, d2;
        na.mode = 0;
        if (int e = reduce_norm(c, na, &d0)) return e;
        na.mode = 1; na.Ka = Kp(0);
        if (int e = reduce_norm(c, na, &d1)) return e;
        const double interval = std::fabs(tf - t);
        double h0 = (d0 < 1e-5 || d1 < 1e-5) ? 1e-6 : 0.01 * d0 / d1;
        h0 = std::min(h0, interval);
        LinComb lc;
        memset(&lc, 0, sizeof(lc));
        lc.n = 1; lc.c[0] = 1.0; lc.h = h0 * direction;
        hipLaunchKernelGGL(stage_input_kernel, dim3(nbX), dim3(256), 0, c.s, y, ks, n_el, D, Dp, lc, c.ws.X, (double*)nullptr,
                           (const RkCtl*)nullptr, 0, (const double*)nullptr, (const double*)nullptr);
        if (int e = eval_rhs(c, c.ws.X, t + h0 * direction, Kp(1))) return e;
        ++st->nfev;
        na.mode = 2; na.Ka = Kp(0); na.Kb = Kp(1);
        if (int e = reduce_norm(c, na, &d2)) return e;
        d2 /= h0;
        double h1 = (d1 <= 1e-15 && d2 <= 1e-15) ? std::max(1e-6, h0 * 1e-3) : std::pow(0.01 / std::max(d1, d2), 1.0 / 5.0);
        h_abs = std::min(std::min(100 * h0, h1), std::min(interval, max_step));
    }

    const double SAFETY = 0.9, MIN_FACTOR = 0.2, MAX_FACTOR = 10.0, ERR_EXP = -1.0 / 5.0;
    while (t != tf) {
        const double min_step = 10 * std::fabs(std::nextafter(t, direction * INFINITY) - t);
        if (h_abs > max_step) h_abs = max_step; else if (h_abs < min_step) h_abs = min_step;
        bool accepted = false, rejected = false;
        double h = 0, t_new = t;
        while (!accepted) {
            if (h_abs < min_step) { st->status = 1; return vpho::fail("vpho_ode_sample: step size underflow at t=%g", t); }
            h = h_abs * direction;
            t_new = t + h;
            if (direction * (t_new - tf) > 0) t_new = tf;
            h = t_new - t;
            h_abs = std::fabs(h);
            {
                float ts[6];
                for (int s = 1; s < 6; ++s) ts[s - 1] = (float)(t + RK_C[s] * h);
                ts[5] = (float)(t + h);
                if (int e = embed_times(c, ts, 6)) return e;
            }
            for (int s = 1; s < 6; ++s) {
                LinComb lc;
                memset(&lc, 0, sizeof(lc));
                lc.n = s; lc.h = h;
                for (int j = 0; j < s; ++j) lc.c[j] = RK_A[s][j];
                if (int e = eval_rhs(c, nullptr, t + RK_C[s] * h, Kp(s), s - 1, &lc, y, nullptr, &ks)) return e;
            }
            {
                LinComb lc;
                memset(&lc, 0, sizeof(lc));
                lc.n = 6; lc.h = h;
                for (int j = 0; j < 6; ++j) lc.c[j] = RK_B[j];
                if (int e = eval_rhs(c, nullptr, t + h, Kp(6), 5, &lc, y, ynew, &ks)) return e;
            }
            st->nfev += 6;
            NormArgs na;
// ... 7 lines not shown
                if (rejected) factor = std::min(1.0, factor);
                log_step(t, h, err, 1);
                h_abs *= factor;
                accepted = true;
                ++st->n_accepted;
            } else {
                log_step(t, h, err, 0);
                h_abs *= std::max(MIN_FACTOR, SAFETY * std::pow(err, ERR_EXP));
                rejected = true;
                ++st->n_rejected;
            }
        }
        while (next_idx < num_steps && te[next_idx] >= t_new) {
            DenseArgs da;
            for (int j = 0; j < 7; ++j) for (int m = 0; m < 4; ++m) da.P[j][m] = RK_P[j][m];
            da.h = h;
            da.n = 0;
            while (da.n < DENSE_MAX && next_idx < num_steps && te[next_idx] >= t_new) {
                const double x = (te[next_idx] - t) / h;
                double* pp = da.p[da.n];
                pp[0] = x; pp[1] = x * x; pp[2] = pp[1] * x; pp[3] = pp[2] * x;
                da.idx[da.n++] = next_idx++;
            }
            hipLaunchKernelGGL(dense_kernel, dim3(nbE), dim3(256), 0, c.s, y, ks, n_el, D, da, xs_out, xs_is_f64, num_steps);
        }
        std::swap(y, ynew);
        std::swap(ks.p[0], ks.p[6]);
        t = t_new;
    }
    {
        const float tfl = (float)eps;
        hipLaunchKernelGGL(stage_input_kernel, dim3(nbX), dim3(256), 0, c.s, y, ks, n_el, D, Dp, LinComb{{0}, 0, 0.0}, c.ws.X, (double*)nullptr,
                           (const RkCtl*)nullptr, 0, (const double*)nullptr, (const double*)nullptr);
        if (int e = eval_net(c, c.ws.X, tfl, 0, 0.f, c.ws.tmp)) return e;
        ++st->nfev;
        const float g = sigma_f32(tfl) * (float)std::sqrt(2.0 * (std::log(SIGMA_MAX) - std::log(SIGMA_MIN)));
        const float stepf = (float)((1.0 - eps) / num_steps);
        hipLaunchKernelGGL(denoise_kernel, dim3(nbE), dim3(256), 0, c.s, y, c.ws.tmp, n_el, g, stepf, x_out, x_is_f64,
                           (const RkCtl*)nullptr, (const double*)nullptr, (const double*)nullptr);
    }
    if (int e = vpho::check_launch("ode tail")) return e;
    int nan_host = 0;
    VPHO_HIP(hipMemcpyAsync(&nan_host, c.ws.nan_count, 4, hipMemcpyDeviceToHost, c.s));
    VPHO_HIP(hipStreamSynchronize(c.s));
    st->nan_count = nan_host;
    return 0;
}

struct CtlHdr { RkCtl c; };
double* pinned_block(size_t bytes) {
    static thread_local char* p = nullptr;
    static thread_local size_t cap = 0;
    if (cap < bytes) {
        if (p) (void)hipHostFree(p);
        if (hipHostMalloc((void**)&p, bytes, hipHostMallocDefault) != hipSuccess) { p = nullptr; cap = 0; return nullptr; }
        cap = bytes;
    }
    return (double*)p;
}

int blocking_wait(hipStream_t s) {
    static thread_local hipEvent_t ev = nullptr;
    if (!ev) VPHO_HIP(hipEventCreateWithFlags(&ev, hipEventBlockingSync | hipEventDisableTiming));
    VPHO_HIP(hipEventRecord(ev, s));
    VPHO_HIP(hipEventSynchronize(ev));
    return 0;
}

int ode_sample_device(Ctx& c, const float* feat_img, const float* init_x, double T0, double eps, int num_steps, double rtol, double atol,
                      void* xs_out, int xs_is_f64, void* x_out, int x_is_f64, vpho_ode_stats* st, double* step_log, int step_log_cap) {
    const vpho_score_weights* w = c.w;
    const long long n_el = c.n_el;
    const int D = w->D, Dp = w->Dp;
    const int nbX = (int)((c.R * Dp + 255) / 256), nbE = (int)((n_el + 255) / 256);
    RkCtl* ctl = c.ws.ctl;
    KSlots ks;
    for (int j = 0; j < 7; ++j) ks.p[j] = c.ws.K + (long long)j * n_el;
    const double g_scale = std::sqrt(2.0 * (std::log(SIGMA_MAX) - std::log(SIGMA_MIN)));

    VPHO_HIP(hipMemsetAsync(c.ws.nan_count, 0, 4, c.s));
    RkSetup su{T0, eps, rtol, atol, g_scale, num_steps, CTL_LOG_CAP, c.ws.te, c.ws.dense_p, c.ws.log};
    hipLaunchKernelGGL(rk_setup_kernel, dim3(1), dim3(1), 0, c.s, ctl, su);
    if (int e = prepare_cimg(c, feat_img)) return e;
    hipLaunchKernelGGL(f32_to_state_kernel, dim3(nbX), dim3(256), 0, c.s, init_x, n_el, D, Dp, c.ws.y, c.ws.X);

    if (int e = eval_rhs(c, c.ws.X, T0, c.ws.K, -1, nullptr, nullptr, nullptr, nullptr, true)) return e;
    {
        NormArgs na;
        memset(&na, 0, sizeof(na));
        na.y = c.ws.y; na.rtol = rtol; na.atol = atol;
        na.mode = 0;
        if (int e = enqueue_norm(c, na, &ctl->d[0])) return e;
        na.mode = 1; na.Ka = ks.p[0];
        if (int e = enqueue_norm(c, na, &ctl->d[1])) return e;
        hipLaunchKernelGGL(rk_init1_kernel, dim3(1), dim3(1), 0, c.s, ctl, n_el);
        LinComb lc;
        memset(&lc, 0, sizeof(lc));
        lc.n = 1; lc.c[0] = 1.0;
        hipLaunchKernelGGL(stage_input_kernel, dim3(nbX), dim3(256), 0, c.s, c.ws.y, ks, n_el, D, Dp, lc, c.ws.X, (double*)nullptr,
                           (const RkCtl*)ctl, 1, (const double*)c.ws.y, (const double*)c.ws.ynew);
        if (int e = embed_times(c, nullptr, 1, 1)) return e;
        CtlCall cc;
        cc.mode = 1; cc.stage = 0; cc.out_slot = 1;
        if (int e = eval_net(c, c.ws.X, 0.f, 1, 0.f, nullptr, 0, nullptr, nullptr, nullptr, nullptr, cc)) return e;
        na.mode = 2; na.Ka = ks.p[0]; na.Kb = ks.p[1];
        if (int e = enqueue_norm(c, na, &ctl->d[2])) return e;
        hipLaunchKernelGGL(rk_init2_kernel, dim3(1), dim3(1), 0, c.s, ctl, n_el);
    }

    RkC kc;
    for (int i = 0; i < 6; ++i) kc.C[i] = RK_C[i];
    DenseP dp;
    for (int j = 0; j < 7; ++j) for (int m = 0; m < 4; ++m) dp.P[j][m] = RK_P[j][m];
    auto enqueue_attempt = [&]() -> int {
        hipLaunchKernelGGL(rk_begin_kernel, dim3(1), dim3(1), 0, c.s, ctl, kc);
        if (int e = embed_times(c, nullptr, 6, 1)) return e;
        for (int s = 1; s <= 6; ++s) {
            LinComb lc;
            memset(&lc, 0, sizeof(lc));
            lc.n = s < 6 ? s : 6;
            for (int j = 0; j < lc.n; ++j) lc.c[j] = s < 6 ? RK_A[s][j] : RK_B[j];
            CtlCall cc;
            cc.mode = 1; cc.stage = s - 1; cc.out_slot = s; cc.write_ynew = s == 6;
            if (int e = eval_net(c, nullptr, 0.f, 1, 0.f, nullptr, s - 1, &lc, nullptr, nullptr, nullptr, cc)) return e;
        }
        NormArgs na;
        memset(&na, 0, sizeof(na));
        na.mode = 3; na.rtol = rtol; na.atol = atol;
        for (int j = 0; j < 7; ++j) na.E[j] = RK_E[j];
        if (int e = enqueue_norm(c, na, c.ws.result, true)) return e;
        hipLaunchKernelGGL(rk_end_kernel, dim3(1), dim3(1), 0, c.s, ctl, (const double*)c.ws.result, n_el);
        hipLaunchKernelGGL(dense_ctl_kernel, dim3(nbE), dim3(256), 0, c.s, (const RkCtl*)ctl, (const double*)c.ws.y, (const double*)c.ws.ynew,
                           (const float*)c.ws.K, n_el, D, dp, xs_out, xs_is_f64, num_steps);
        return vpho::check_launch("rk attempt");
    };
    auto enqueue_final = [&]() -> int {
        const float tfl = (float)eps;
        hipLaunchKernelGGL(stage_input_kernel, dim3(nbX), dim3(256), 0, c.s, (const double*)c.ws.y, ks, n_el, D, Dp, LinComb{{0}, 0, 0.0}, c.ws.X,
                           (double*)nullptr, (const RkCtl*)ctl, 2, (const double*)c.ws.y, (const double*)c.ws.ynew);
        CtlCall cc;
        cc.mode = 2;
        if (int e = eval_net(c, c.ws.X, tfl, 0, 0.f, c.ws.tmp, -1, nullptr, nullptr, nullptr, nullptr, cc)) return e;
        const float g = sigma_f32(tfl) * (float)g_scale;
        const float stepf = (float)((1.0 - eps) / num_steps);
        hipLaunchKernelGGL(denoise_kernel, dim3(nbE), dim3(256), 0, c.s, (const double*)c.ws.y, c.ws.tmp, n_el, g, stepf, x_out, x_is_f64,
                           (const RkCtl*)ctl, (const double*)c.ws.y, (const double*)c.ws.ynew);
        return vpho::check_launch("ode tail");
    };

    static std::mutex hint_mu;
    static std::unordered_map<const void*, int> hint;
    int n_first = 10;
    {
        std::lock_guard<std::mutex> lk(hint_mu);
        auto it = hint.find((const void*)ctl);
        if (it != hint.end()) n_first = it->second;
    }
    const size_t hdr_bytes = sizeof(RkCtl) + 8;
    char* host = (char*)pinned_block(hdr_bytes + (size_t)CTL_LOG_CAP * 32);
    VPHO_REQUIRE(host != nullptr, "hipHostMalloc failed");
    RkCtl* hc = (RkCtl*)host;
    int* nan_host = (int*)(host + sizeof(RkCtl));
    int enq = 0;
    for (int round = 0;; ++round) {
        const int n = round == 0 ? std::max(1, n_first) : 2;
        for (int i = 0; i < n; ++i) if (int e = enqueue_attempt()) return e;
        enq += n;
        if (int e = enqueue_final()) return e;
        VPHO_HIP(hipMemcpyAsync(hc, ctl, sizeof(RkCtl), hipMemcpyDeviceToHost, c.s));
        VPHO_HIP(hipMemcpyAsync(nan_host, c.ws.nan_count, 4, hipMemcpyDeviceToHost, c.s));
        if (int e = blocking_wait(c.s)) return e;
        if (hc->done) break;
        VPHO_REQUIRE(enq < CTL_LOG_CAP, "vpho_ode_sample: no convergence after %d attempted steps", enq);
    }
    {
        std::lock_guard<std::mutex> lk(hint_mu);
        hint[(const void*)ctl] = hc->n_attempts;
    }
    st->nfev = hc->nfev + 1;
    st->n_accepted = hc->n_accepted; st->n_rejected = hc->n_rejected; st->status = hc->status; st->n_log = hc->n_log;
    st->nan_count = *nan_host;
    if (step_log && hc->n_log > 0) {
        const int n = std::min(std::min(hc->n_log, step_log_cap), CTL_LOG_CAP);
        if (n > 0) {
            double* lg = (double*)(host + hdr_bytes);
            VPHO_HIP(hipMemcpyAsync(lg, c.ws.log, (size_t)n * 32, hipMemcpyDeviceToHost, c.s));
            if (int e = blocking_wait(c.s)) return e;
            memcpy(step_log, lg, (size_t)n * 32);
        }
    }
    if (hc->status == 1) return vpho::fail("vpho_ode_sample: step size underflow at t=%g", hc->t);
    return 0;
}

}

extern "C" int vpho_ode_sample(const vpho_score_weights* w, const float* feat_img, int bs, int S, const float* init_x,
                               double T0, double eps, int num_steps, double rtol, double atol,
                               void* xs_out, int xs_is_f64, void* x_out, int x_is_f64, void* workspace, long long workspace_bytes,
                               vpho_ode_stats* st, double* step_log, int step_log_cap, void* stream) {
    if (int e = check_weights(w)) return e;
    VPHO_REQUIRE(bs > 0 && S > 0 && num_steps >= 1 && feat_img && init_x && xs_out && x_out && workspace && st, "vpho_ode_sample: bad argument");
    VPHO_REQUIRE(T0 > eps, "vpho_ode_sample: T0 must exceed eps (backward integration)");
    Ctx c;
    c.w = w; c.bs = bs; c.S = S; c.R = (long long)bs * S; c.n_el = c.R * w->D; c.NH = w->nheads * 256; c.s = (hipStream_t)stream;
    c.ws = carve(*w, bs, S, (char*)workspace);
    VPHO_REQUIRE(workspace_bytes >= c.ws.bytes, "vpho_ode_sample: workspace %lld < %lld bytes", workspace_bytes, c.ws.bytes);
    memset(st, 0, sizeof(*st));
    static const bool host_ctl = getenv("VPHO_RK_HOST") && atoi(getenv("VPHO_RK_HOST")) != 0;
    if (host_ctl || num_steps > CTL_MAX_STEPS)
        return ode_sample_host(c, feat_img, init_x, T0, eps, num_steps, rtol, atol, xs_out, xs_is_f64, x_out, x_is_f64, st, step_log, step_log_cap);
    return ode_sample_device(c, feat_img, init_x, T0, eps, num_steps, rtol, atol, xs_out, xs_is_f64, x_out, x_is_f64, st, step_log, step_log_cap);
}
```

vpho_amd/evaluate.py:

```python
import torch
import torch.distributed as dist

from .eval_layout import BLOCKS, RowLayout
from .ops_names import HAND_BENCH_SOURCES, HAND_BENCH_TABLE, HAND_METRIC_NAMES, MULTI_TABLES, OBJ_METRIC_NAMES, PHYSICS_SOURCES

ROW, MULTI, PHYS, PHYS_MULTI, VOL_MULTI, VOL, HAND_BENCH, HAND_BENCH_MULTI = (width for _, _, width, _ in BLOCKS)
ROW_BEST = ROW + MULTI
OBJ_COL = 12


def row_width(eval_best=False, eval_physics=False, physics_multi=False, volume_multi=False, eval_volume=False):
    return RowLayout.resolve(eval_best, eval_physics, physics_multi, eval_volume, volume_multi).width


def mje_mm(pd, gt):
    return (pd - gt).norm(dim=-1).mean(dim=-1) * 1000.0


def postprocess(out, root_joint, is_right):
    sgn = torch.where(is_right.bool(), 1.0, -1.0).to(out['agg_hand_joint'].dtype)[:, None, None]
    res = {}
    for k in ('reg_hand_joint', 'agg_hand_joint', 'reg_hand_vert', 'agg_hand_vert'):
        v = out[k].clone()
        v[..., 0] = v[..., 0] * sgn[..., 0]
# ... 101 lines not shown
        blk[:, 2:4] = meshes.volume(gt_vert.float().contiguous(), data['gt_obj_rt'].double().contiguous(), ids, h).flip(1).float()
    return blk


def hypotheses_to_camera(x, root_joint, is_right):
    sgn = torch.where(is_right.bool(), 1.0, -1.0).to(x.dtype)[:, None, None]
    v = x.clone()
    v[..., 0] = v[..., 0] * sgn
    return v + root_joint[:, None, None]


def _hypothesis_pairs(out, data):
    root = data['root_joint'].float().contiguous()
    return hypotheses_to_camera(out['diff_final_hand_vert'].float(), root, data['is_right']).contiguous(), _hypothesis_obj_rt(out, root)


def physics_multi_block(out, data, meshes):
    from .configs.args import cfg
    if not out['diff_final_hand_vert'].is_cuda:
        raise RuntimeError('physics_multi_block: the penetration metrics run on the GPU only (no CPU path)')
    verts, pd_rt = _hypothesis_pairs(out, data)
    table, _ = meshes.multi(verts, pd_rt, meshes.obj_ids(data['obj_name']), contact_thresh=float(cfg.physics_contact_thresh))
    return table.float()


def volume_multi_block(out, data, meshes):
    from .configs.args import cfg
    if not out['diff_final_hand_vert'].is_cuda:
        raise RuntimeError('volume_multi_block: the intersection volume runs on the GPU only (no CPU path)')
    verts, pd_rt = _hypothesis_pairs(out, data)
    table, _ = meshes.volume_multi(verts, pd_rt, meshes.obj_ids(data['obj_name']), float(cfg.physics_voxel_pitch))
    return table.float()


def hand_bench_width(multi=False):
    return HAND_BENCH + (HAND_BENCH_MULTI if multi else 0)


def _hand_bench_pair(pd_joint, pd_vert, data, gt_joint, gt_vert):
    from . import ops
    root = data['root_joint'].float().contiguous()
    c = lambda t: t.float().contiguous()
    j = ops.hand_bench_multi(c(pd_joint), c(gt_joint), root, data['is_right'], with_fscore=False)
    v = ops.hand_bench_multi(c(pd_vert), c(gt_vert), root, data['is_right'])
    return torch.cat([j[..., :2], v], -1)


def hand_bench_block(out, data, gt_joint, gt_vert):
    if not gt_joint.is_cuda:
        raise RuntimeError('hand_bench_block: the hand benchmark metrics run on the GPU only (no CPU path)')
    agg = _hand_bench_pair(out['agg_hand_joint'][:, None], out['agg_hand_vert'][:, None], data, gt_joint, gt_vert)[:, 0]
    reg = _hand_bench_pair(out['reg_hand_joint'][:, None], out['reg_hand_vert'][:, None], data, gt_joint, gt_vert)[:, 0]
    blk = torch.cat([agg, reg], 1).float()
    from .configs.args import cfg
    if cfg.aggregation_mode_hand == '2D_pt_joint':
        blk[:, 2:8] = float('nan')
    return blk


def hand_bench_multi_block(out, data, gt_joint, gt_vert):
    from . import ops
    if not gt_joint.is_cuda:
        raise RuntimeError('hand_bench_multi_block: the hand benchmark metrics run on the GPU only (no CPU path)')
    per = _hand_bench_pair(out['diff_final_hand_joint'], out['diff_final_hand_vert'], data, gt_joint, gt_vert).contiguous()
    return torch.cat(ops.hand_bench_table(per), 1).float()


def hand_bench_table(block):
    if block.shape[1] not in (HAND_BENCH, HAND_BENCH + HAND_BENCH_MULTI):
        raise ValueError(f'hand_bench_table: {block.shape[1]} columns, expected {HAND_BENCH} or {HAND_BENCH + HAND_BENCH_MULTI}')
    mean = block.double().mean(0)
    names = HAND_BENCH_SOURCES + (MULTI_TABLES if block.shape[1] > HAND_BENCH else ())
    return {src: {k: float(mean[8 * s + i]) for i, k in enumerate(HAND_BENCH_TABLE)} for s, src in enumerate(names)}


def metric_rows(out, data, gt_joint, gt_vert, first_index, assets=None, eval_best=False, eval_physics=False, physics_multi=False, volume_multi=False,
                eval_volume=False, eval_hand_bench=False, hand_bench_multi=False, layout=None):
    if layout is None:
        layout = RowLayout.resolve(eval_best, eval_physics, physics_multi, eval_volume, volume_multi, eval_hand_bench, hand_bench_multi)
    if assets is None and layout.has('physics'):
        raise ValueError('metric_rows: eval_physics needs the asset tables (object meshes)')
    if assets is None and layout.has('volume'):
        raise ValueError('metric_rows: eval_volume needs the asset tables (object meshes, hand faces)')
    pp = postprocess(out, data['root_joint'], data['is_right'])
    bs, dev = gt_joint.shape[0], gt_joint.device
    rows = torch.empty((bs, layout.width), device=dev, dtype=torch.float32)
    if torch.is_tensor(first_index):
        rows[:, 0] = first_index.to(device=rows.device, dtype=torch.float32).reshape(bs)
    else:
        rows[:, 0] = torch.arange(first_index, first_index + bs, device=rows.device, dtype=torch.float32)
    rows[:, 1] = mje_mm(pp['reg_hand_joint'], gt_joint)
    rows[:, 2] = mje_mm(pp['first_hand_joint'], gt_joint)
    rows[:, 3] = mje_mm(pp['agg_hand_joint'], gt_joint)
    rows[:, 4] = mje_mm(pp['agg_hand_vert'], gt_vert)
    rows[:, 5] = mje_mm(pp['agg_hand_joint'], pp['reg_hand_joint'])
    rows[:, 6] = out['agg_obj_6d'][:, 6:].float().norm(dim=-1)
    rows[:, 7] = data['is_right'].float()
    rows[:, 8:ROW] = 0.0
    if gt_joint.is_cuda:
        from . import ops
        c = lambda t: t.float().contiguous()
        rows[:, 8] = ops.hand_metrics(c(pp['reg_hand_joint']), c(gt_joint))[1] * 1000.0
        rows[:, 9] = ops.hand_metrics(c(pp['agg_hand_joint']), c(gt_joint))[1] * 1000.0
        rows[:, 10] = ops.hand_metrics(c(pp['agg_hand_vert']), c(gt_vert))[1] * 1000.0
        if assets is not None and 'gt_obj_rt' in data:
            rows[:, OBJ_COL:OBJ_COL + 16] = object_metric_block(out, data, assets).float()
    for name, block in (('multi', lambda: multi_hypothesis_block(out, data, gt_joint, gt_vert, assets)),
                        ('physics', lambda: physics_block(pp, out, data, gt_vert, physics_meter(assets, dev))),
                        ('physics_multi', lambda: physics_multi_block(out, data, physics_meter(assets, dev, multi=True))),
                        ('volume', lambda: volume_block(pp, out, data, gt_vert, physics_meter(assets, dev, volume=True))),
                        ('volume_multi', lambda: volume_multi_block(out, data, physics_meter(assets, dev, volume_multi=True))),
                        ('hand_bench', lambda: hand_bench_block(out, data, gt_joint, gt_vert)),
                        ('hand_bench_multi', lambda: hand_bench_multi_block(out, data, gt_joint, gt_vert))):
        if layout.has(name):
            rows[:, layout.slice(name)] = block()
    from .configs.args import cfg
    if cfg.aggregation_mode_hand == '2D_pt_joint':
        rows[:, 4] = float('nan')
        rows[:, 10] = float('nan')
        if layout.has('physics'):
            rows[:, layout.slice('physics')][:, 0:4] = float('nan')
        if layout.has('volume'):
            rows[:, layout.slice('volume')][:, 0:2] = float('nan')
    return rows


class _Pending:

    def __init__(self, fut):
        self._fut = fut

    def result(self, timeout=None):
        res, done = self._fut.result(timeout)
        done.synchronize()
        return res

    def done(self):
        return self._fut.done() and self._fut.result()[1].query()


class PipelinedPredictor:

    def __init__(self, model, depth=3):
        import threading
        from concurrent.futures import ThreadPoolExecutor
        from .model.engine import Engine
        self.model, self.depth = model, depth
        self.engines = [Engine(model) for _ in range(depth)]
        self.dev = self.engines[0].dev
        self.streams = [torch.cuda.Stream(device=self.dev) for _ in range(depth)]
        self.locks = [threading.Lock() for _ in range(depth)]
        self.pools = [ThreadPoolExecutor(max_workers=1, thread_name_prefix=f'vpho-predict-{i}') for i in range(depth)]
        self.n = 0
        import os
        self.sync_in_worker = os.environ.get('VPHO_PIPE_SYNC_IN_WORKER', '0') == '1'

    def submit(self, batch, post=None):
        from .configs.args import cfg
        bs = batch['rgb'].shape[0]
        noise_h = torch.randn(bs * cfg.sample_num, 96)
        noise_o = torch.randn(bs * cfg.sample_num, 9)
        slot = self.n % self.depth
        self.n += 1
        ready = torch.cuda.Event()
        ready.record(torch.cuda.current_stream(self.dev))

        def work():
            with self.locks[slot], torch.cuda.device(self.dev), torch.cuda.stream(self.streams[slot]), torch.no_grad():
                self.streams[slot].wait_event(ready)
                eng = self.engines[slot]
                out = eng.predict(batch, noise_hand=noise_h, noise_obj=noise_o)
                res = post(out, batch, eng) if post is not None else out
                done = torch.cuda.Event(blocking=True)
                done.record(self.streams[slot])
                if self.sync_in_worker:
                    done.synchronize()
                return res, done

        return _Pending(self.pools[slot].submit(work))

    def close(self):
        for p in self.pools:
            p.shutdown(wait=True)


def gather_rows(rows):
    from .launch import group_active
    if not group_active():
        return rows
# ... 85 lines not shown
```

vpho_amd/model/engine.py:

```python
import os

import torch

from .. import ops
from ..configs.args import cfg, AGGREGATION_MODES_HAND, AGGREGATION_MODES_OBJ
from . import pack as P

MANO_JOINT_LEVEL = {0: [0], 1: [1, 5, 9, 13, 17], 2: [2, 6, 10, 14, 18], 3: [3, 7, 11, 15, 19], 4: [4, 8, 12, 16, 20]}
PHY_TOPK = 5
DEFAULT_MODE = 'heatmap_cascade'


def _signature(model):
    import itertools
    v = p = 0
    for t in itertools.chain(model.parameters(), model.buffers()):
        v += t._version
        p ^= t.data_ptr()
    return v, p, str(next(model.parameters()).device)


def _stack2(a, b):
    if torch.is_tensor(a):
        return torch.stack([a, b]).contiguous()
# ... 127 lines not shown
        if b['down'] is not None and self.down_fuse and x.shape[-1] % 32 == 0 and y.shape[-1] % 32 == 0:
            return ops.conv2d_nhwc(y, *b['c3_down'], x2=x, stride2=b['stride'], out_slope=0.01, out=out, groups=groups, x2_shared=x_shared)
        r = x if b['down'] is None else ops.conv2d_nhwc(x, *b['down'], stride=b['stride'], groups=groups, x_shared=x_shared)
        return ops.conv2d_nhwc(y, *b['c3'], res=r, out_slope=0.01, out=out, groups=groups)

    def _layer(self, x, blocks, out=None, groups=1, x_shared=False):
        for i, b in enumerate(blocks):
            x = self._bottleneck(x, b, out if i == len(blocks) - 1 else None, groups, x_shared and i == 0)
        return x

    def _side(self):
        import contextlib
        if not self._two_streams:
            return contextlib.nullcontext()
        if self._feat_side is None:
            self._feat_side = torch.cuda.Stream(self.dev)
        self._feat_side.wait_stream(torch.cuda.current_stream())
        return torch.cuda.stream(self._feat_side)

    def _join(self):
        if self._two_streams:
            torch.cuda.current_stream().wait_stream(self._feat_side)

    def _stem(self, rgb):
        x = ops.nchw_to_nhwc(rgb, 4)
        c1 = ops.maxpool_nhwc(ops.conv2d_nhwc(x, *self.stem, kh=7, kw=7, stride=2, pad=3, out_slope=0.01), 3, 2, 1)
        return self._layer(c1, self.layers['layer1_h'])

    def _lateral(self, c, wb, p, rows=None, groups=1):
        if self.fpn_fuse:
            return ops.conv2d_nhwc(c, *wb, rows=rows, rows_scatter=rows is not None, res_up=p, groups=groups)
        q = ops.conv2d_nhwc(c, *wb, rows=rows, rows_scatter=rows is not None, groups=groups)
        return ops.resize_bilinear_nhwc(p, q.shape[1], q.shape[2], out=q, accumulate=True, rows=rows)

    def _top_down(self, fpn, sfx, c5, c4, c3, groups=1):
        p = ops.conv2d_nhwc(c5, *fpn['toplayer' + sfx], groups=groups)
        p = self._lateral(c4, fpn['latlayer1' + sfx], p, groups=groups)
        return self._lateral(c3, fpn['latlayer2' + sfx], p, groups=groups)

    def _fpn_out(self, br, c2, p3, win, halo):
        p = self._lateral(c2, self.fpn[f'latlayer3_{br}'], p3, rows=halo)
        return ops.conv3x3(p, *self.fpn[f'smooth3_{br}'], winograd=self.winograd, rows=win)

    def _hm_up(self, x, h, groups=1):
        y = ops.conv3x3(x, *h['c0'], winograd=self.winograd, groups=groups)
        y = ops.conv3x3(y, *h['c1'], winograd=self.winograd, groups=groups)
        N, H, W, _ = y.shape
        co = h['deconv_b'].shape[-1]
        up = torch.empty((N, 2 * H, 2 * W, co), device=y.device)
        for (py, px), (w, pady, padx) in h['deconv'].items():
            ops.conv2d_nhwc(y, w, h['deconv_b'], kh=2, kw=2, pad_y=pady, pad_x=padx, out_hw=(H, W), out_slope=0.0, groups=groups,
                            out_view=(up, 4 * H * W * co, 4 * W * co, 2 * co, (py * 2 * W + px) * co))
        return up

    def _encoder(self, x, e, groups=1):
        x = ops.conv2d_nhwc(x, *e['project'], groups=groups)
        stages = []
        for i, b in enumerate(e['blocks']):
            y = ops.conv2d_nhwc(x, *b['c1'], in_scale=b['pre'][0], in_shift=b['pre'][1], in_slope=0.01, out_slope=0.01, groups=groups)
            y = ops.conv3x3(y, *b['c2'], out_slope=0.01, winograd=self.winograd, groups=groups)
            x = ops.conv2d_nhwc(y, *b['c3'], res=x, groups=groups)
            if i % 2 == 1:
                x = ops.maxpool_nhwc(x, 2, 2, 0)
                stages.append(x)
        N = x.shape[0]
        return ops.nhwc_to_nchw(x).view(N, -1), stages

    def _cross(self, c, st_h, st_o, grav, flip_u8):
        bs = st_h.shape[0]
        ph = ops.conv3x3(st_h, *c['proj_hand'], winograd=self.winograd)
        po = ops.conv3x3(st_o, *c['proj_obj'], winograd=self.winograd)
        ge = ops.linear(ops.nerf_embed(grav, flip_u8), *c['grav'])
        x = ops.cross_tokens(ph, po, ge, c['pe']).view(bs * 65, 512)
        qkv = ops.linear(x, *c['in_proj'])
        o = ops.linear(ops.mha(qkv, bs, 65, 512, 2).view(bs * 65, 512), *c['out_proj'])
        x = ops.add_layernorm(x, o, *c['n1'])
        ff = ops.linear(ops.linear(x, *c['l1'], out_slope=0.0), *c['l2'])
        return ops.add_layernorm(x, ff, *c['n2'])

    def features(self, data):
        grouped = self.grouped and self.conv_terms == 0
        self._two_streams = self.feature_streams >= 2 and not grouped
        with ops.conv_split(self.conv_terms):
            rgb = data['rgb'].float().contiguous()
            bs = rgb.shape[0]
            f32 = lambda k: data[k].float().contiguous()
            left_u8 = (~data['is_right'].bool()).to(torch.uint8).contiguous()
            bb_h, bb_o, bb_hr, bb_or = f32('bbox_hand'), f32('bbox_obj'), f32('bbox_hand_rect'), f32('bbox_obj_rect')
            win_h = win_o = halo_h = halo_o = None
            if self.roi_window:
                fh, fw = rgb.shape[2] // 4, rgb.shape[3] // 4
                win_h = ops.roi_windows(bb_h, bb_hr, bs, fh, fw, 0.25)
                win_o = ops.roi_windows(bb_or, None, bs, fh, fw, 0.25)
                halo_h, halo_o = ops.roi_windows(bb_h, bb_hr, bs, fh, fw, 0.25, dilate=1), ops.roi_windows(bb_or, None, bs, fh, fw, 0.25, dilate=1)
            grav = f32('gravity').view(bs, 3)
            twin = self._twin_grouped if grouped else self._twin_per_branch
            (hand_feat, obj_feat, hf_hr, in_h, in_o, hm_hand, hm_obj, hand_heatmap, obj_heatmap, enc_h, enc_o, st_h, st_o) = twin(
                rgb, (bb_h, bb_o, bb_hr, bb_or), (win_h, win_o, halo_h, halo_o), left_u8)
            with self._side():
                tok_o = self._cross(self.cross['obj'], st_h, st_o, grav, left_u8)
            hmn = self.head_mano
            a64 = self.head64
            h = ops.linear(ops.linear(enc_h, *hmn['l0'], out_slope=0.01, acc64=a64), *hmn['l2'], out_slope=0.01, acc64=a64)
            pose = ops.rot6d_to_axis_angle(ops.linear(h, *hmn['pose'], acc64=a64), 16)
            shape = ops.linear(h, *hmn['shape'], acc64=a64)
            ctx = self.mano.shape(shape)
            ho3d = data['is_ho3d'].to(torch.uint8).contiguous() if 'is_ho3d' in data else None
            reg_vert, reg_joint = self.mano.fk(pose, ctx, 1, True, ho3d)
            tok_h = self._cross(self.cross['hand'], st_h, st_o, grav, left_u8)
            self._join()
            ph = self.phys
            scale = ops.linear(ops.linear(tok_h, *ph['s0'], out_slope=0.01), *ph['s2'])
            logits = ops.linear(ops.linear(tok_o, *ph['w0'], out_slope=0.01), *ph['w2'])
            force_local = ops.force_local(scale, logits, ph['anchor'], bs * 32, 32, 65, 0, 32).view(bs, 32, 3)
            return dict(hand_feat=hand_feat, obj_feat=obj_feat, roi_win_hand=win_h, roi_win_obj=win_o, hf_hr=hf_hr, enc_in_hand=in_h, enc_in_obj=in_o,
                        hm_hand_nhwc=hm_hand, hm_obj_nhwc=hm_obj, hand_heatmap=hand_heatmap, obj_heatmap=obj_heatmap,
                        encoding_hand=enc_h, encoding_obj=enc_o, stage_hand=st_h, stage_obj=st_o, mano_pose=pose, mano_shape=shape,
                        mano_ctx=ctx, reg_hand_vert=reg_vert, reg_hand_joint=reg_joint, tok_hand=tok_h, tok_obj=tok_o, force_local=force_local)

    def _twin_grouped(self, rgb, bb, win, left_u8):
        (bb_h, bb_o, bb_hr, bb_or), (win_h, win_o, halo_h, halo_o) = bb, win
        bs, R = rgb.shape[0], cfg.roi_size
        c2 = self._stem(rgb)
        c3 = self._layer(c2, self.g_layers['layer2'], groups=2, x_shared=True)
        c4 = self._layer(c3, self.g_layers['layer3'], groups=2)
        c5 = self._layer(c4, self.layers['layer4_h'])
        p3 = self._top_down(self.g_fpn, '', c5, c4, c3, groups=2)
        hand_feat = self._fpn_out('h', c2, p3[:bs], win_h, halo_h)
        obj_feat = self._fpn_out('o', c2, p3[bs:], win_o, halo_o)
        crop = torch.empty((2 * bs, R, R, 256), device=self.dev)
        enc_in = torch.zeros((2 * bs, R, R, self.g_enc['cin_pad']), device=self.dev)
        in_h, in_o = enc_in[:bs], enc_in[bs:]
        hf_hr = ops.roi_align_nhwc(hand_feat, bb_h, R, 0.25, win=win_h, out=crop[:bs])
        ops.roi_align_nhwc(hand_feat, bb_hr, R, 0.25, out=in_h, win=win_h)
        if win_o is not None:
            ops.roi_align_dual_nhwc(obj_feat, bb_or, R, 0.25, win_o, in_o, flip_w2=left_u8, out=crop[bs:])
        else:
            ops.roi_align_nhwc(obj_feat, bb_or, R, 0.25, out=crop[bs:])
            ops.roi_align_nhwc(obj_feat, bb_or, R, 0.25, flip_w=left_u8, out=in_o)
        up = self._hm_up(crop, self.g_hm, groups=2)
        hm_hand = ops.conv2d_nhwc(up[:bs], *self.hm['hand']['final'])
        hm_obj = ops.conv2d_nhwc(up[bs:], *self.hm['obj']['final'])
        ops.resize_bilinear_nhwc(ops.align_heatmap_nhwc(hm_hand, bb_h, bb_hr), R, R, out=in_h, c_off=256)
        ops.resize_bilinear_nhwc(ops.align_heatmap_nhwc(hm_obj, bb_o, bb_or, flip_w=left_u8), R, R, out=in_o, c_off=256)
        enc, st = self._encoder(enc_in, self.g_enc, groups=2)
        hand_heatmap, obj_heatmap = ops.nhwc_to_nchw(hm_hand), ops.nhwc_to_nchw(hm_obj)
        return (hand_feat, obj_feat, hf_hr, in_h[..., :self.enc['hand']['cin_pad']], in_o, hm_hand, hm_obj, hand_heatmap, obj_heatmap,
                enc[:bs], enc[bs:], st[1][:bs], st[1][bs:])

    def _twin_per_branch(self, rgb, bb, win, left_u8):
        (bb_h, bb_o, bb_hr, bb_or), (win_h, win_o, halo_h, halo_o) = bb, win
        bs, R, L = rgb.shape[0], cfg.roi_size, self.layers
        eh, eo = self.enc['hand'], self.enc['obj']
        in_h = torch.zeros((bs, R, R, eh['cin_pad']), device=self.dev)
        in_o = torch.zeros((bs, R, R, eo['cin_pad']), device=self.dev)
        c2 = self._stem(rgb)
        c4 = torch.empty((2 * bs, c2.shape[1] // 4, c2.shape[2] // 4, L['layer3_h'][-1]['c3'][0].shape[0]), device=c2.device)
        with self._side():
            c3o = self._layer(c2, L['layer2_o'])
            c4o = self._layer(c3o, L['layer3_o'], out=c4[bs:])
        c3h = self._layer(c2, L['layer2_h'])
        c4h = self._layer(c3h, L['layer3_h'], out=c4[:bs])
        self._join()
        c5 = self._layer(c4, L['layer4_h'])
        with self._side():
            obj_feat = self._fpn_out('o', c2, self._top_down(self.fpn, '_o', c5[bs:], c4o, c3o), win_o, halo_o)
            if win_o is not None:
                of_or_rect = ops.roi_align_dual_nhwc(obj_feat, bb_or, R, 0.25, win_o, in_o, flip_w2=left_u8)
            else:
                of_or_rect = ops.roi_align_nhwc(obj_feat, bb_or, R, 0.25)
                ops.roi_align_nhwc(obj_feat, bb_or, R, 0.25, flip_w=left_u8, out=in_o)
            hm_obj = ops.conv2d_nhwc(self._hm_up(of_or_rect, self.hm['obj']), *self.hm['obj']['final'])
            ops.resize_bilinear_nhwc(ops.align_heatmap_nhwc(hm_obj, bb_o, bb_or, flip_w=left_u8), R, R, out=in_o, c_off=256)
            enc_o, st_o = self._encoder(in_o, eo)
            obj_heatmap = ops.nhwc_to_nchw(hm_obj)
        hand_feat = self._fpn_out('h', c2, self._top_down(self.fpn, '_h', c5[:bs], c4h, c3h), win_h, halo_h)
        hf_hr = ops.roi_align_nhwc(hand_feat, bb_h, R, 0.25, win=win_h)
        ops.roi_align_nhwc(hand_feat, bb_hr, R, 0.25, out=in_h, win=win_h)
        hm_hand = ops.conv2d_nhwc(self._hm_up(hf_hr, self.hm['hand']), *self.hm['hand']['final'])
        ops.resize_bilinear_nhwc(ops.align_heatmap_nhwc(hm_hand, bb_h, bb_hr), R, R, out=in_h, c_off=256)
        enc_h, st_h = self._encoder(in_h, eh)
        hand_heatmap = ops.nhwc_to_nchw(hm_hand)
        self._join()
        return hand_feat, obj_feat, hf_hr, in_h, in_o, hm_hand, hm_obj, hand_heatmap, obj_heatmap, enc_h, enc_o, st_h[1], st_o[1]

    def _prior(self, rows, dim):
        if self.device_prior:
            return torch.randn((rows, dim), device=self.dev)
        key = (rows, dim)
        slot = self._pin.setdefault(key, dict(bufs=[torch.empty((rows, dim), pin_memory=True) for _ in range(2)], i=0))
        slot['i'] ^= 1
        return slot['bufs'][slot['i']].normal_()

    _AGG_F = ('mano_pose', 'mano_shape', 'hand_heatmap', 'obj_heatmap', 'force_local')
    _AGG_D = ('root_joint_flip', 'root_joint', 'cam_intr_crop_flip', 'bbox_hand', 'bbox_obj_rect', 'is_right', 'is_grasped')

    def _aggregate_from_tensors(self, t):
        f = {k: t['f_' + k] for k in self._AGG_F}
        f['mano_ctx'] = (t['f_ctx_v'], t['f_ctx_j'])
        data = {k: t['d_' + k] for k in self._AGG_D}
        S = t['obj_pose'].shape[1]
        k_hand, k_obj, mode_hand, mode_obj, weighted = self._agg_k
        return self.aggregate(f, data, t['final58'], t['obj_pose'], S, k_hand, k_obj, oid=t['oid'], mode_hand=mode_hand, mode_obj=mode_obj,
                              weighted=weighted)

    def aggregate_graphed(self, f, data, final58, obj_pose, S, k_hand, k_obj, mode_hand=DEFAULT_MODE, mode_obj=DEFAULT_MODE, weighted=True):
        self._check_modes(f, S, k_hand, k_obj, mode_hand, mode_obj)
        t = {'f_' + k: f[k] for k in self._AGG_F}
        t['f_ctx_v'], t['f_ctx_j'] = f['mano_ctx']
        t.update({'d_' + k: data[k] for k in self._AGG_D})
        t.update(final58=final58, obj_pose=obj_pose, oid=self.agg.obj_ids(data['obj_name']))
        self._agg_k = (k_hand, k_obj, mode_hand, mode_obj, bool(weighted))
        return self._aggregate_graph(t, (k_hand, k_obj, self.keep_states, mode_hand, mode_obj, bool(weighted)))

    @staticmethod
    def _check_modes(f, S, k_hand, k_obj, mode_hand, mode_obj):
        if mode_hand not in AGGREGATION_MODES_HAND:
            raise ops.VphoError(f'aggregation_mode_hand {mode_hand!r}: one of {AGGREGATION_MODES_HAND}')
        if mode_obj not in AGGREGATION_MODES_OBJ:
            raise ops.VphoError(f'aggregation_mode_obj {mode_obj!r}: one of {AGGREGATION_MODES_OBJ}')
        if mode_hand != DEFAULT_MODE and k_hand > S:
            raise ops.VphoError(f'aggregation_mode_hand {mode_hand}: topk_hand = {k_hand} exceeds sample_num = {S} (only the cascade adds the '
                                f'regression candidates)')
        if mode_obj != DEFAULT_MODE and k_obj > S:
            raise ops.VphoError(f'aggregation_mode_obj {mode_obj}: topk_obj = {k_obj} exceeds sample_num = {S}')
        for side, mode in (('hand', mode_hand), ('obj', mode_obj)):
            H, W = f[f'{side}_heatmap'].shape[-2:]
            if mode.startswith('2D_pt') and H != W:
                raise ops.VphoError(f'aggregation_mode_{side} {mode}: the heat maps must be square (got {H} x {W}); the reference reads the '
                                    f'peak through a transposed grid that is only defined for H = W')

    def _aggregate_hand_mode(self, mode, f, final58, root_flip, Kmat, bb_h, S, k, weighted):
        A, M = self.agg, self.mano
        bs = final58.shape[0] // S
        ctx = f['mano_ctx']
        cand = final58.view(bs, S, 58)
        info = {}
        if mode in ('heatmap', '2D_pt_pose', '2D_pt_joint'):
            _, joints = M.fk(final58, ctx, S, False)
            joints = joints.view(bs, S, 21, 3)
        if mode == 'heatmap':
            hv = A.hand_heat(joints, root_flip, Kmat, bb_h, f['hand_heatmap'], list(range(21)))
            val, idx, _, score = A.hand_fuse_level(hv, cand[:, :, :48].contiguous(), k, 0, want_scores=True)
            val, idx = val.view(bs, k), idx.view(bs, k)
            w = A.topk_weights(val) if weighted else None
            pose48 = A.hand_pose_fuse(cand, idx, w)
            info.update(topk=idx, val=val, score=score.view(bs, S), weight=w)
        elif mode == '2D_pt_pose':
            peak, ind = A.heatmap_peak(f['hand_heatmap'])
            score = A.hand_pt2d_score(joints, root_flip, Kmat, bb_h, peak)
            val, idx = A.topk(score, k)
            val, idx = val.view(bs, k), idx.view(bs, k)
            pose48 = A.hand_pose_fuse(cand, idx, None)
            info.update(topk=idx, val=val, score=score, peak=peak, peak_index=ind)
        elif mode == '2D_pt_joint':
            peak, ind = A.heatmap_peak(f['hand_heatmap'])
            score = A.hand_pt2d_score(joints, root_flip, Kmat, bb_h, peak, per_joint=True)
            val, idx = A.topk(score, k, 21)
            joint = A.hand_joint_gather_mean(joints, idx)
            info.update(topk=idx, val=val, score=score, peak=peak, peak_index=ind)
            return (torch.zeros((bs, 58), device=self.dev), torch.zeros((bs, 778, 3), device=self.dev), joint), info
        elif mode == 'average_all':
            pose48 = A.hand_pose_fuse(cand, None, None, n=S)
        else:
            pose48 = cand[:, 0, :48]
        mano = torch.cat([pose48, cand[:, 0, 48:]], -1).contiguous()
        vert, joint = M.fk(mano, ctx, 1, True)
        return (mano, vert, joint), info

    def _aggregate_obj_mode(self, mode, f, obj_pose, root, oid, isr, Kmat, bb_or, k):
        A = self.agg
        bs = obj_pose.shape[0]
        info = {}
        if mode == 'heatmap':
            score = A.obj_heat_score(obj_pose, root, oid, isr, Kmat, bb_or, f['obj_heatmap'])
            val, idx = A.topk(score, k)
            info.update(val=val.view(bs, k), score=score)
        elif mode == '2D_pt_pose':
            peak, ind = A.heatmap_peak(f['obj_heatmap'])
            score = A.obj_pt2d_score(obj_pose, root, oid, isr, Kmat, bb_or, peak)
            val, idx = A.topk(score, k)
            info.update(val=val.view(bs, k), score=score, peak=peak, peak_index=ind)
        else:
            n = k if mode == 'average_all' else 1
            idx = torch.arange(n, device=self.dev, dtype=torch.int32).repeat(bs, 1)
        idx = idx.view(bs, -1).contiguous()
        info['topk'] = idx
        return A.obj_fuse(obj_pose, idx, None), info

    def aggregate(self, f, data, final58, obj_pose, S, k_hand, k_obj, oid=None, mode_hand=DEFAULT_MODE, mode_obj=DEFAULT_MODE, weighted=True):
        self._check_modes(f, S, k_hand, k_obj, mode_hand, mode_obj)
        A, M = self.agg, self.mano
        bs = obj_pose.shape[0]
        if mode_hand != DEFAULT_MODE or mode_obj != DEFAULT_MODE:
            f32 = lambda k: data[k].float().contiguous()
            Kmat = f32('cam_intr_crop_flip').view(bs, 9)
            res, dbg = {}, {}
            if mode_hand == DEFAULT_MODE or mode_obj == DEFAULT_MODE:
                res, dbg = self.aggregate(f, data, final58, obj_pose, S, k_hand, k_obj, oid=oid)
            dbg.update(mode_hand=mode_hand, mode_obj=mode_obj)
            if mode_hand != DEFAULT_MODE:
                (mano, vert, joint), dbg['hand_mode'] = self._aggregate_hand_mode(mode_hand, f, final58, f32('root_joint_flip'), Kmat, f32('bbox_hand'),
                                                                                  S, k_hand, weighted)
                res.update(hand_agg_mano=mano, hand_agg_vert=vert, hand_agg_joint=joint)
            if mode_obj != DEFAULT_MODE:
                oid = A.obj_ids(data['obj_name']) if oid is None else oid
                isr = data['is_right'].to(torch.uint8).contiguous()
                res['obj_agg_6d'], dbg['obj_mode'] = self._aggregate_obj_mode(mode_obj, f, obj_pose, f32('root_joint'), oid, isr, Kmat,
                                                                              f32('bbox_obj_rect'), k_obj)
            return res, dbg
        f32 = lambda k: data[k].float().contiguous()
        root_flip, root, Kmat = f32('root_joint_flip'), f32('root_joint'), f32('cam_intr_crop_flip').view(bs, 9)
        bb_h, bb_or = f32('bbox_hand'), f32('bbox_obj_rect')
        isr = data['is_right'].to(torch.uint8).contiguous()
        ungrasp = (~data['is_grasped'].bool()).to(torch.uint8).contiguous()
        oid = A.obj_ids(data['obj_name']) if oid is None else oid
        ctx = f['mano_ctx']
        dbg = dict(hand_topk=[], hand_val=[])
        if self.keep_states:
            dbg['cascade_state'], dbg['hand_score'] = [], []
        pose = A.hand_candidates(final58, f['mano_pose'], bs, S)
        tp = None
        for level in range(4):
            observe = [j for l in range(level + 1, 5) for j in MANO_JOINT_LEVEL[l]]
            if self.keep_states:
                dbg['cascade_state'].append(pose.clone())
            _, joints = M.fk(pose.view(-1, 48), ctx, 2 * S, False)
            hv = A.hand_heat(joints.view(bs, 2 * S, 21, 3), root_flip, Kmat, bb_h, f['hand_heatmap'], observe)
            if self.keep_states:
                val, idx, tp, sc = A.hand_fuse_level(hv, pose, k_hand, level, want_topk_pose=(level == 3), want_scores=True)
                dbg['hand_score'].append(sc)
            else:
                val, idx, tp = A.hand_fuse_level(hv, pose, k_hand, level, want_topk_pose=(level == 3))
            dbg['hand_topk'].append(idx)
            dbg['hand_val'].append(val)
        fused_rows = pose.view(bs, 2 * S * 48)
        agg_vert, _ = M.fk(fused_rows, ctx, 1, True)
        fpnt, fglob = A.force_anchor(agg_vert, root_flip, f['force_local'], 1)
        hm_o = f['obj_heatmap']
        sc = A.obj_heat_score(obj_pose, root, oid, isr, Kmat, bb_or, hm_o)
        tv, ti = A.topk(sc, k_obj)
        transl = A.obj_fuse(obj_pose, ti.view(bs, -1), A.topk_weights(tv).view(bs, -1))[:, 6:].contiguous()
        sc2 = A.obj_heat_score(obj_pose, root, oid, isr, Kmat, bb_or, hm_o, transl_override=transl)
        _, ri = A.topk(sc2, k_obj)
        cand = A.obj_cross(obj_pose, ti.view(bs, -1), ri.view(bs, -1))
        ps = A.obj_physics_score(cand, root, oid, isr, fpnt, fglob)
        _, pi = A.topk(ps, PHY_TOPK)
        hs = A.obj_heat_score(cand, root, oid, isr, Kmat, bb_or, hm_o)
        hval, hi = A.topk(hs, PHY_TOPK)
        obj_fused = A.obj_fuse(cand, pi.view(bs, -1), None, hi.view(bs, -1), A.topk_weights(hval).view(bs, -1), ungrasp)
        obj_vert = A.obj_verts(obj_fused, root, oid, isr)
        cand58 = A.hand_phys_candidates(fused_rows, f['mano_shape'], tp)
        n_c = cand58.shape[1]
        cverts, _ = M.fk(cand58.view(-1, 58), ctx, n_c, True)
        fp2, fg2 = A.force_anchor(cverts, root_flip, f['force_local'], n_c)
        fs = A.hand_phys_score(fp2, fg2, obj_vert, bs, n_c)
        _, fidx = A.topk(fs, PHY_TOPK, 5)
        out58 = A.hand_phys_fuse(cand58, fidx)
        out_vert, out_joint = M.fk(out58, ctx, 1, True)
        dbg.update(transl_topk=ti, rot_topk=ri, phys_topk=pi, heat_topk=hi, phys_score=ps, transl_score=sc, rot_score=sc2, heat_score=hs, hand_phys_topk=fidx, hand_phys_score=fs, cand58=cand58, cand_vert=cverts, cand_force_point=fp2, cand_force_global=fg2,
                   cascade_pose=fused_rows[:, :48], force_point=fpnt, force_global=fglob, obj_vert=obj_vert, pose6d_candidate=cand, transl=transl)
        return dict(obj_agg_6d=obj_fused, hand_agg_mano=out58, hand_agg_vert=out_vert, hand_agg_joint=out_joint), dbg

    @torch.no_grad()
    def predict(self, data, noise_hand=None, noise_obj=None, mode_hand=None, mode_obj=None):
        S, T0, steps = cfg.sample_num, cfg.sample_T0, cfg.sampling_steps
        modes = dict(mode_hand=cfg.aggregation_mode_hand if mode_hand is None else mode_hand,
                     mode_obj=cfg.aggregation_mode_obj if mode_obj is None else mode_obj, weighted=bool(cfg.do_weighted_average))
        with torch.cuda.device(self.dev):
            if self.use_graphs:
                f = self._features_graph({k: v for k, v in data.items() if torch.is_tensor(v)}, (cfg.roi_size, cfg.heatmap_size, self.conv_terms, self.roi_window, self.feature_streams, self.winograd, self.fpn_fuse, self.down_fuse))
                keep = lambda t: t.clone()
            else:
                f = self.features(data)
                keep = lambda t: t
            bs = f['mano_pose'].shape[0]
            sig = 0.01 * (50 / 0.01) ** T0
            init_h = self._prior(bs * S, 96) if noise_hand is None else noise_hand.float()
            init_o = self._prior(bs * S, 9) if noise_obj is None else noise_obj.float()
            init_h, init_o = init_h.to(self.dev, non_blocking=True) * sig, init_o.to(self.dev, non_blocking=True) * sig
            out = dict(reg_hand_vert=keep(f['reg_hand_vert']), reg_hand_joint=keep(f['reg_hand_joint']), hand_heatmap=keep(f['hand_heatmap']),
                       obj_heatmap=keep(f['obj_heatmap']), force_local=keep(f['force_local']))
            main = torch.cuda.current_stream()
            if self._obj_stream is None:
                self._obj_stream = torch.cuda.Stream(device=self.dev)
            obj_stream = self._obj_stream
            obj_stream.wait_stream(main)

            def run_obj():
                with torch.cuda.device(self.dev), torch.cuda.stream(obj_stream):
                    return self.score_obj.sample(f['encoding_obj'], init_o, S, T0, steps, xs_f64=True, x_f64=True)

            concurrent = os.environ.get('VPHO_SERIAL_SAMPLERS', '0') != '1' and not self.serial_samplers
            fut = self._obj_worker.submit(run_obj) if concurrent else None
            xs_h, x_h, st_h = self.score_hand.sample(f['encoding_hand'], init_h, S, T0, steps, xs_f64=False, x_f64=False)
            inproc = torch.empty((bs * S * steps, 58), device=self.dev)
            ops.rot6d_to_axis_angle(xs_h.view(bs * S * steps, 96), 16, out=inproc)
            ops.append_betas(f['mano_shape'], inproc, S * steps)
            final = torch.empty((bs * S, 58), device=self.dev)
            ops.rot6d_to_axis_angle(x_h, 16, out=final)
            ops.append_betas(f['mano_shape'], final, S)
            out['diff_inprocess_hand_mano'] = inproc.view(bs, S, steps, 58)
            out['diff_final_hand_mano'] = final.view(bs, S, 58)
            ctx = f['mano_ctx']
            viz = inproc.view(bs * S, steps, 58)[0, ::10].contiguous()
            vv, vj = self.mano.fk(viz, ctx, viz.shape[0], True)
            out['diff_inprocess_hand_vert'], out['diff_inprocess_hand_joint'] = vv, vj
            fv, fj = self.mano.fk(final, ctx, S, True)
            out['diff_final_hand_vert'] = fv.view(bs, S, 778, 3)
            out['diff_final_hand_joint'] = fj.view(bs, S, 21, 3)
            xs_o, x_o, st_o = fut.result() if fut is not None else run_obj()
            main.wait_stream(obj_stream)
            for t in (xs_o, x_o):
                t.record_stream(main)
            out['diff_inprocess_obj_6d'] = xs_o.view(bs, S, steps, 9)
            out['diff_final_obj_6d'] = x_o.view(bs, S, 9)
            for name, st in (('hand', st_h), ('obj', st_o)):
                if st['nan_count']:
                    print("\033[31mWarning: NaN detected in score evaluation. \033[0m")
            x_o9 = out['diff_final_obj_6d']
            if self.use_graphs:
                agg, dbg = self.aggregate_graphed(f, data, final, x_o9, S, cfg.topk_hand, cfg.topk_obj, **modes)
            else:
                agg, dbg = self.aggregate(f, data, final, x_o9, S, cfg.topk_hand, cfg.topk_obj, **modes)
            out['agg_obj_6d'] = keep(agg['obj_agg_6d'])
            out['agg_hand_mano'] = keep(agg['hand_agg_mano'])
            out['agg_hand_vert'] = keep(agg['hand_agg_vert'])
            out['agg_hand_joint'] = keep(agg['hand_agg_joint'])
            self.last_info = dict(features=f, hand_ode=st_h, obj_ode=st_o, agg=dbg, hand_x6d=x_h)
        return out
```

vpho_amd/ops.py:

```python
import ctypes as C
import os

import torch

_HERE = os.path.dirname(os.path.abspath(__file__))
LIB_PATH = os.environ.get('VPHO_HIP_LIB') or os.path.join(_HERE, 'libvpho_hip.so')

if not os.path.exists(LIB_PATH):
    raise ImportError(f'{LIB_PATH} is missing: build the HIP extension first (python -m vpho_amd.build or '
                      f'__graft_entry__.build()); vpho_amd has no CPU fallback')
lib = C.CDLL(LIB_PATH)
lib.vpho_last_error.restype = C.c_char_p
lib.vpho_abi_version.restype = C.c_int
ABI_VERSION = 13
if lib.vpho_abi_version() != ABI_VERSION:
    raise ImportError(f'{LIB_PATH} implements ABI version {lib.vpho_abi_version()}, this binding expects {ABI_VERSION}: rebuild the '
                      f'extension (python -m vpho_amd.build --force)')
lib.vpho_obj_metrics_workspace_bytes.restype = C.c_longlong
lib.vpho_obj_metrics_multi_workspace_bytes.restype = C.c_longlong
lib.vpho_bn_workspace_bytes.restype = C.c_longlong
lib.vpho_conv2d_wgrad_workspace_bytes.restype = C.c_longlong
lib.vpho_mha_bwd_workspace_bytes.restype = C.c_longlong
lib.vpho_grad_sqnorm_workspace_bytes.restype = C.c_longlong
lib.vpho_infer_record_bytes.restype = C.c_longlong
# ... 330 lines not shown
    cap = (N * H * W + 255) // 256
    bn.stats = torch.empty((cap, BN_STAT_PLANES, cout), device=x.device, dtype=torch.float32)
    rows_out = C.c_int(0)
    bx = (bn.x, bn.mean, bn.invstd, bn.gamma, bn.beta) if bn.x is not None else (None,) * 5
    if bn.x is not None:
        assert bn.x.shape == out.shape and bn.x.is_contiguous()
    _call('vpho_conv3x3_winograd_stats_nhwc_f32', _f32(x), _f32(u), _f32(bias), I(N), I(H), I(W), I(cin), I(x_ld), I(cout), F(out_slope), _f32(out), I(cout),
          _f32(bn.stats), I(cap), C.byref(rows_out), *[_f32(t) for t in bx], F(gate_slope))
    bn.rows, bn.calls = rows_out.value, 1
    return out


def conv3x3_train(x, w, bias=None, out_slope=1.0, rows=None, bn=None):
    N, H, W, x_ld = x.shape
    cout, cin = w.shape[0], w.shape[1] // 9
    if not _TRAIN_WINOGRAD or not winograd_ok(H, W, cin, cout, x_ld) or w.shape[1] != 9 * cin:
        return conv2d_nhwc(x, w, bias, kh=3, kw=3, pad=1, out_slope=out_slope, bn=bn)
    u = winograd_weights_device(w)
    if bn is not None and FUSE_BN and rows is None and not _wino8():
        return _winograd_bn(x, u, bias, out_slope, cin, cout, bn)
    if rows is not None:
        assert rows.shape == (N, H, W)
        out = torch.zeros((N, H, W, cout), device=x.device, dtype=torch.float32)
        _call('vpho_conv3x3_winograd_scatter_nhwc_f32', _f32(x), _f32(u), _f32(bias), I(N), I(H), I(W), I(cin), I(x_ld), I(cout), F(out_slope),
              _i32(rows.wins), _i32(rows.tiles()), _f32(out), I(cout))
        return out
    return conv3x3_winograd(x, u, bias, out_slope)


def conv3x3_dgrad_winograd(dy, w, gate=None, rows=None, bn=None):
    N, H, W, ld = dy.shape
    cout, cin = w.shape[0], w.shape[1] // 9
    if not _TRAIN_WINOGRAD or not winograd_ok(H, W, cout, cin, ld) or w.shape[1] != 9 * cin:
        return None
    u = winograd_weights_device(w, for_input_gradient=True)
    if rows is not None and gate is None:
        assert rows.shape == (N, H, W)
        out = torch.zeros((N, H, W, cin), device=dy.device, dtype=torch.float32)
        _call('vpho_conv3x3_winograd_scatter_nhwc_f32', _f32(dy), _f32(u), None, I(N), I(H), I(W), I(cout), I(ld), I(cin), F(1.0),
              _i32(rows.wins), _i32(rows.tiles()), _f32(out), I(cin))
        return out
    if gate is None:
        return conv3x3_winograd(dy, u, None, 1.0)
    g, slope = gate
    if bn is not None and bn.x is not None and FUSE_BN and not _wino8():
        return _winograd_bn(dy, u, None, 1.0, cout, cin, bn, gate_slope=slope)
    assert g.shape == (N, H, W, cin) and g.is_contiguous()
    out = torch.empty((N, H, W, cin), device=dy.device, dtype=torch.float32)
    _call('vpho_conv3x3_winograd_gate_nhwc_f32', _f32(dy), _f32(u), _f32(g), F(slope), I(N), I(H), I(W), I(cout), I(ld), I(cin), _f32(out), I(cin))
    return out


def linear(x, w, bias=None, out_slope=1.0, out=None, acc64=False):
    rows, cin = x.shape
    if acc64:
        assert x.is_contiguous() and w.is_contiguous() and w.shape[1] == cin
        y = torch.empty((rows, w.shape[0]), device=x.device, dtype=torch.float32) if out is None else out
        _call('vpho_linear_acc64_f32', _f32(x), I(rows), I(cin), I(cin), _f32(w), _f32(bias), I(w.shape[0]), F(out_slope), _f32(y), I(y.shape[-1]))
        return y
    y = conv2d_nhwc(x.view(rows, 1, 1, cin), w, bias, out_slope=out_slope,
                    out=None if out is None else out.view(rows, 1, 1, w.shape[0]))
    return y.view(rows, w.shape[0])


class ScoreWeights(C.Structure):
    _fields_ = [('D', C.c_int), ('Dp', C.c_int), ('nheads', C.c_int)] + \
               [(k, C.c_void_p) for k in ('t_W', 't_w', 't_b', 'pe0_w', 'pe0_b', 'pe2_w', 'pe2_b', 'w1_t', 'w1_p',
                                          'w1_f', 'b1', 'w2', 'b2')] + [('w1_p_split', C.c_void_p), ('split_terms', C.c_int)]


class OdeStats(C.Structure):
    _fields_ = [(k, C.c_int) for k in ('nfev', 'n_accepted', 'n_rejected', 'nan_count', 'status', 'n_log')]


lib.vpho_score_workspace_bytes.restype = C.c_longlong
lib.vpho_maxpool_bwd_workspace_bytes.restype = C.c_longlong
lib.vpho_maxpool_bwd_workspace_bytes.argtypes = [C.c_int] * 7
lib.vpho_score_workspace_bytes.argtypes = [C.POINTER(ScoreWeights), C.c_int, C.c_int]
lib.vpho_score_eval.argtypes = [C.POINTER(ScoreWeights), C.c_void_p, C.c_int, C.c_int, C.c_void_p, C.c_float, C.c_void_p,
                                C.c_void_p, C.c_longlong, C.c_void_p]
lib.vpho_ode_sample.argtypes = [C.POINTER(ScoreWeights), C.c_void_p, C.c_int, C.c_int, C.c_void_p, C.c_double, C.c_double,
                                C.c_int, C.c_double, C.c_double, C.c_void_p, C.c_int, C.c_void_p, C.c_int, C.c_void_p, C.c_longlong,
                                C.POINTER(OdeStats), C.c_void_p, C.c_int, C.c_void_p]


class ScoreNet:

    def __init__(self, sd, prefix, device):
        g = lambda k: sd[f'{prefix}.{k}'].detach().to(device=device, dtype=torch.float32)
        w1, b1 = g('head.head.0.weight'), g('head.head.0.bias')
        w2, b2 = g('head.head.2.weight'), g('head.head.2.bias')
        n = w1.shape[0]
        self.nheads, self.D = n, 3 * n
        self.Dp = (self.D + 3) // 4 * 4
        NH = n * 256
        pe0 = g('pose_encoder.0.weight')
        t = dict(
            t_W=g('t_encoder.0.W').contiguous(), t_w=g('t_encoder.1.weight').contiguous(), t_b=g('t_encoder.1.bias').contiguous(),
            pe0_w=torch.nn.functional.pad(pe0, (0, self.Dp - self.D)).contiguous(), pe0_b=g('pose_encoder.0.bias').contiguous(),
            pe2_w=g('pose_encoder.2.weight').contiguous(), pe2_b=g('pose_encoder.2.bias').contiguous(),
            w1_t=w1[:, :128, :].permute(1, 0, 2).reshape(128, NH).contiguous(),
            w1_p=w1[:, 128:384, :].permute(0, 2, 1).reshape(NH, 256).contiguous(),
            w1_f=w1[:, 384:, :].permute(0, 2, 1).reshape(NH, 1024).contiguous(),
            b1=b1.reshape(NH).contiguous(),
            w2=torch.nn.functional.pad(w2, (0, 1)).reshape(NH, 4).contiguous(), b2=b2.reshape(n * 3).contiguous())
        self.tensors = t
        self.c = ScoreWeights()
        self.c.D, self.c.Dp, self.c.nheads = self.D, self.Dp, n
        for k, v in t.items():
            setattr(self.c, k, v.data_ptr())
        self.device = device
        self._ws = None
        self.set_split(os.environ.get('VPHO_SCORE_MFMA', 'f32'))

    def set_split(self, mode):
        terms = {'f32': 0, 'bf16x6': 6, 'bf16x9': 9}[mode]
        if terms and 'w1_p_split' not in self.tensors:
            w = self.tensors['w1_p'].view(self.nheads, 256, 256)
            h = w.to(torch.bfloat16)
            m = (w - h.float()).to(torch.bfloat16)
            l = (w - h.float() - m.float()).to(torch.bfloat16)
            assert torch.equal(h.float() + m.float() + l.float(), w)
            self.tensors['w1_p_split'] = torch.stack([h, m, l], 1).contiguous()
        self.c.w1_p_split = self.tensors['w1_p_split'].data_ptr() if terms else None
        self.c.split_terms = terms
        self.split_mode = mode

    def workspace(self, bs, S):
        need = lib.vpho_score_workspace_bytes(C.byref(self.c), bs, S)
        if self._ws is None or self._ws.numel() < need:
            self._ws = torch.empty(need, dtype=torch.uint8, device=self.device)
        return self._ws

    def score(self, feat_img, x, t, S):
        bs = feat_img.shape[0]
        ws = self.workspace(bs, S)
        out = torch.empty((bs * S, self.D), device=self.device, dtype=torch.float32)
        _check(lib.vpho_score_eval(C.byref(self.c), _ptr(feat_img, torch.float32), bs, S, _ptr(x, torch.float32), float(t),
                                   _ptr(out), _ptr(ws), ws.numel(), _stream()))
        return out

    def sample(self, feat_img, init_x, S, T0, num_steps, xs_f64, x_f64=True, eps=1e-5, rtol=3e-3, atol=3e-4, log_cap=4096):
        bs = feat_img.shape[0]
        R = bs * S
        assert init_x.shape == (R, self.D)
        ws = self.workspace(bs, S)
        xs = torch.empty((R, num_steps, self.D), device=self.device, dtype=torch.float64 if xs_f64 else torch.float32)
        x = torch.empty((R, self.D), device=self.device, dtype=torch.float64 if x_f64 else torch.float32)
        st = OdeStats()
        log = (C.c_double * (4 * log_cap))()
        _check(lib.vpho_ode_sample(C.byref(self.c), _ptr(feat_img, torch.float32), bs, S, _ptr(init_x, torch.float32),
                                   float(T0), float(eps), int(num_steps), float(rtol), float(atol), _ptr(xs),
                                   1 if xs_f64 else 0, _ptr(x), 1 if x_f64 else 0, _ptr(ws), ws.numel(), C.byref(st), log, log_cap,
                                   _stream()))
        n = min(st.n_log, log_cap)
        steps = [(log[4 * i], log[4 * i + 1], log[4 * i + 2], bool(log[4 * i + 3])) for i in range(n)]
        return xs, x, dict(nfev=st.nfev, n_accepted=st.n_accepted, n_rejected=st.n_rejected, nan_count=st.nan_count,
                           steps=steps)


def _i32(t):
    return _ptr(t, torch.int32)


def _u8(t):
    return None if t is None else _ptr(t, torch.uint8)


def _f32(t):
    return None if t is None else _ptr(t, torch.float32)


def _f64(t):
    return None if t is None else _ptr(t, torch.float64)


def _call(name, *args):
    _check(getattr(lib, name)(*args, _stream()))


def _new(shape, like, dtype=torch.float32):
    return torch.empty(shape, device=like.device, dtype=dtype)


LL, I, F = C.c_longlong, C.c_int, C.c_float


def nchw_to_nhwc(x, ld=None):
    N, Cc, H, W = x.shape
    ld = Cc if ld is None else ld
    y = _new((N, H, W, ld), x)
    _call('vpho_nchw_to_nhwc_f32', _f32(x), I(N), I(Cc), I(H), I(W), _f32(y), I(ld))
    return y


def nhwc_to_nchw(x, channels=None):
    N, H, W, ld = x.shape
    Cc = ld if channels is None else channels
    y = _new((N, Cc, H, W), x)
    _call('vpho_nhwc_to_nchw_f32', _f32(x), I(N), I(H), I(W), I(Cc), I(ld), _f32(y))
    return y


def maxpool_nhwc(x, k, stride, pad):
    N, H, W, Cc = x.shape
    OH, OW = (H + 2 * pad - k) // stride + 1, (W + 2 * pad - k) // stride + 1
    y = _new((N, OH, OW, Cc), x)
    _call('vpho_maxpool_nhwc_f32', _f32(x), I(N), I(H), I(W), I(Cc), I(k), I(stride), I(pad), _f32(y))
    return y


def resize_bilinear_nhwc(x, OH, OW, out=None, c_off=0, accumulate=False, channels=None, rows=None):
    N, H, W, ldx = x.shape
    Cc = ldx if channels is None else channels
    if out is None:
        out = _new((N, OH, OW, Cc), x)
    assert out.shape[:3] == (N, OH, OW)
    if rows is not None:
        assert rows.shape == (N, OH, OW)
        _call('vpho_resize_bilinear_rows_nhwc_f32', _f32(x), I(N), I(H), I(W), I(Cc), I(ldx), I(OH), I(OW), _f32(out), I(out.shape[-1]),
              I(c_off), I(1 if accumulate else 0), _ptr(rows.row_map, torch.int32), _ptr(rows.count, torch.int32),
              I(int(rows.count.item()) if _prof_on else 0))
        return out
    _call('vpho_resize_bilinear_nhwc_f32', _f32(x), I(N), I(H), I(W), I(Cc), I(ldx), I(OH), I(OW), _f32(out), I(out.shape[-1]),
          I(c_off), I(1 if accumulate else 0))
    return out


class RoiWindows:
    def __init__(self, wins, row_map, count, shape):
        self.wins, self.row_map, self.count, self.shape = wins, row_map, count, shape
        self._tiles = None

    def tiles(self):
        if self._tiles is None:
            self._tiles = torch.empty((self.shape[0] + 1,), device=self.wins.device, dtype=torch.int32)
            _call('vpho_winograd_window_tiles_i32', _i32(self.wins), I(self.shape[0]), _i32(self._tiles))
        return self._tiles

    def to_map(self, rows):
        n = int(self.count.item())
        N, H, W = self.shape
        idx = self.row_map[:n].long()
        full = torch.zeros((N * H * W, rows.shape[-1]), device=rows.device, dtype=rows.dtype)
        full[idx] = rows[:n]
        mask = torch.zeros((N * H * W,), device=rows.device, dtype=torch.bool)
        mask[idx] = True
        return full.view(N, H, W, -1), mask.view(N, H, W)


def roi_windows(boxes_a, boxes_b, N, H, W, spatial_scale, dilate=0):
    dev = boxes_a.device
    wins = torch.empty((N, 5), device=dev, dtype=torch.int32)
    row_map = torch.empty((N * H * W,), device=dev, dtype=torch.int32)
    count = torch.empty((1,), device=dev, dtype=torch.int32)
    _call('vpho_roi_windows_i32', _f32(boxes_a), _f32(boxes_b), I(N), I(H), I(W), F(spatial_scale), I(dilate), _ptr(wins, torch.int32),
          _ptr(row_map, torch.int32), _ptr(count, torch.int32))
    return RoiWindows(wins, row_map, count, (N, H, W))


def roi_align_nhwc(feat, boxes, out_size, spatial_scale, flip_w=None, out=None, c_off=0, win=None):
    if win is not None:
        N, H, W = win.shape
        Cc = feat.shape[-1]
        if out is None:
            out = _new((N, out_size, out_size, Cc), feat)
        _call('vpho_roi_align_window_nhwc_f32', _f32(feat), _ptr(win.wins, torch.int32), I(N), I(H), I(W), I(Cc), _f32(boxes),
              F(spatial_scale), I(out_size), _u8(flip_w), _f32(out), I(out.shape[-1]), I(c_off), I(int(win.count.item()) if _prof_on else 0))
        return out
    N, H, W, Cc = feat.shape
    if out is None:
        out = _new((N, out_size, out_size, Cc), feat)
    _call('vpho_roi_align_nhwc_f32', _f32(feat), I(N), I(H), I(W), I(Cc), _f32(boxes), F(spatial_scale), I(out_size), _u8(flip_w),
          _f32(out), I(out.shape[-1]), I(c_off))
    return out


def roi_align_dual_nhwc(feat, boxes, out_size, spatial_scale, win, out2, flip_w2=None, c_off2=0, out=None):
    N, H, W = win.shape
    Cc = feat.shape[-1]
    if out is None:
        out = _new((N, out_size, out_size, Cc), feat)
    assert out.shape == (N, out_size, out_size, Cc) and out.is_contiguous()
    _call('vpho_roi_align_window_dual_nhwc_f32', _f32(feat), _ptr(win.wins, torch.int32), I(N), I(H), I(W), I(Cc), _f32(boxes),
          F(spatial_scale), I(out_size), _u8(None), _f32(out), I(Cc), I(0), _u8(flip_w2), _f32(out2), I(out2.shape[-1]), I(c_off2),
          I(int(win.count.item()) if _prof_on else 0))
    return out


def align_heatmap_nhwc(hm, bbox, bbox_rect, flip_w=None):
    N, S, _, Cc = hm.shape
    out = torch.empty_like(hm)
    _call('vpho_align_heatmap_nhwc_f32', _f32(hm), I(N), I(S), I(Cc), _f32(bbox), _f32(bbox_rect), _u8(flip_w), _f32(out))
    return out


def nerf_embed(g, flip_x=None):
    N = g.shape[0]
    out = _new((N, 64), g)
    _call('vpho_nerf_embed_f32', _f32(g), I(N), _u8(flip_x), _f32(out))
    return out


def cross_tokens(proj_hand, proj_obj, grav_emb, pe):
    bs = proj_hand.shape[0]
    out = _new((bs, 65, 512), proj_hand)
    _call('vpho_cross_tokens_f32', _f32(proj_hand), _f32(proj_obj), _f32(grav_emb), _f32(pe), I(bs), _f32(out))
    return out
# ... 207 lines not shown
        _call('vpho_contact_detect_f32', _f32(obj_verts), _f32(obj_normals), _f32(hand_verts), I(n), I(no), I(nh), *args, _f32(oc), _i32(o2h))
        return hc, oc, o2h

    def force_contact(self, hand_contact, thresh=0.0):
        n, ld = hand_contact.shape
        fc, gr = _new((n, 32), hand_contact), _new((n,), hand_contact, torch.uint8)
        _call('vpho_force_contact_f32', C.byref(self.anchor), _f32(hand_contact), I(ld), I(n), F(thresh), _f32(fc), _u8(gr))
        return fc, gr

    def anchor_frames(self, verts):
        n = verts.shape[0]
        pts, frames = _new((n, 32, 3), verts), _new((n, 32, 3, 3), verts)
        _call('vpho_anchor_frames_f32', C.byref(self.anchor), _f32(verts), LL(n), _f32(pts), _f32(frames))
        return pts, frames

    def force_optimize(self, verts, gravity, com, force_contact, is_grasped, batch_size, iters=3000, phase1=300, lr=1e-3):
        n = verts.shape[0]
        assert n % batch_size == 0, 'pad the last batch: the batch-mean force loss couples the samples of a batch'
        pts, frames = self.anchor_frames(verts)
        fl, fg = _new((n, 32, 3), verts), _new((n, 32, 3), verts)
        scale, weight, losses = _new((n, 32), verts), _new((n, 32, 8), verts), _new((n // batch_size, 4), verts)
        _call('vpho_force_optimize_f32', _f32(pts), _f32(frames), _f32(gravity), _f32(com), _f32(force_contact), _u8(is_grasped),
              I(n // batch_size), I(batch_size), I(iters), I(phase1), F(lr), _f32(fl), _f32(fg), _f32(scale), _f32(weight), _f32(losses))
        return dict(force_local=fl, force_global=fg, scale=scale, weight=weight, losses=losses, force_point=pts, frames=frames)

    def hand_phys_candidates(self, agg_pose, betas, topk_pose):
        bs, k = topk_pose.shape[:2]
        out = _new((bs, k + 1, 58), agg_pose)
        _call('vpho_hand_phys_candidates_f32', _f32(agg_pose), I(agg_pose.shape[-1]), _f32(betas), _f32(topk_pose), I(bs), I(k), _f32(out))
        return out

    def hand_phys_score(self, force_point, force_global, obj_vert, bs, n_cand):
        out = _new((bs, n_cand, 5), force_point)
        _call('vpho_hand_phys_score_f32', _f32(force_point), _f32(force_global), _f32(obj_vert), I(obj_vert.shape[1]), I(bs), I(n_cand), _f32(out))
        return out

    def hand_phys_fuse(self, cand, idx):
        bs, n_cand = cand.shape[:2]
        out = _new((bs, 58), cand)
        _call('vpho_hand_phys_fuse_f32', _f32(cand), I(n_cand), _i32(idx), I(bs), I(idx.shape[-1]), _f32(out))
        return out

    def heatmap_peak(self, heatmap):
        bs, J, H, W = heatmap.shape
        peak, ind = _new((bs, J, 2), heatmap), _new((bs, J), heatmap, torch.int32)
        _call('vpho_heatmap_peak_f32', _f32(heatmap), LL(bs * J), I(H), I(W), _f32(peak), _i32(ind))
        return peak, ind

    def hand_pt2d_score(self, joints, root, K, bbox, peak, per_joint=False):
        bs, Cn = joints.shape[:2]
        score = _new((bs, Cn, 21) if per_joint else (bs, Cn), joints)
        _call('vpho_hand_pt2d_score_f32', _f32(joints), _f32(root), _f32(K), _f32(bbox), _f32(peak), I(bs), I(Cn), I(int(per_joint)), _f32(score))
        return score

    def obj_pt2d_score(self, pose, root, obj_id, is_right, K, bbox, peak):
        bs, n = pose.shape[:2]
        assert peak.shape[1] == self.obj.n_kpt
        score = _new((bs, n), root)
        _call('vpho_obj_pt2d_score', _f64(pose), I(n), _f32(root), C.byref(self.obj), _i32(obj_id), _u8(is_right), _f32(K), _f32(bbox), _f32(peak),
              I(bs), _f32(score))
        return score

    def hand_pose_fuse(self, pose, idx=None, w=None, n=None):
        bs, Cn, ld = pose.shape
        n = idx.shape[-1] if idx is not None else (Cn if n is None else n)
        fused = _new((bs, 48), pose)
        _call('vpho_hand_pose_fuse_f32', _f32(pose), I(ld), I(Cn), None if idx is None else _i32(idx), _f32(w), I(bs), I(n), _f32(fused))
        return fused

    def hand_joint_gather_mean(self, joints, idx):
        bs, Cn = joints.shape[:2]
        fused = _new((bs, 21, 3), joints)
        _call('vpho_hand_joint_gather_mean_f32', _f32(joints), _i32(idx), I(bs), I(Cn), I(idx.shape[-1]), _f32(fused))
        return fused


def hand_metrics(pd, gt, per_point=False):
    n, P, _ = pd.shape
    assert gt.shape == pd.shape
    me, pa = _new((n,), pd), _new((n,), pd)
    pp = _new((n, P), pd) if per_point else None
    _call('vpho_hand_metrics_f32', _f32(pd), _f32(gt), I(n), I(P), _f32(me), _f32(pa), _f32(pp))
    return (me, pa, pp) if per_point else (me, pa)


def hand_metrics_multi(pd, gt, root_joint, is_right):
    n, S, P, _ = pd.shape
    assert gt.shape == (n, P, 3) and root_joint.shape == (n, 3) and is_right.shape == (n,)
    me, pa = _new((n, S), pd), _new((n, S), pd)
    flag = is_right.to(device=pd.device, dtype=torch.uint8).contiguous()
    _call('vpho_hand_metrics_multi_f32', _f32(pd), _f32(gt), _f32(root_joint), _u8(flag), I(n), I(S), I(P), _f32(me), _f32(pa))
    return me, pa


HAND_BENCH_MAX_POINTS = 1024
_HAND_BENCH_TABLES = {}


def hand_bench_tables(device):
    key = str(torch.device(device))
    if key not in _HAND_BENCH_TABLES:
        import numpy as np
        from .ops_names import HAND_BENCH_AUC
        t = np.linspace(HAND_BENCH_AUC[0], HAND_BENCH_AUC[1], HAND_BENCH_AUC[2])
        n_t = t.shape[0]
        g = np.zeros(n_t + 1)
        for c in range(1, n_t + 1):
            j0 = n_t - c
            g[c] = ((t[-1] - t[j0]) + ((t[j0] - t[j0 - 1]) / 2 if j0 >= 1 else 0.0)) / (t[-1] - t[0])
        _HAND_BENCH_TABLES[key] = (torch.from_numpy(t).to(device), torch.from_numpy(g).to(device))
    return _HAND_BENCH_TABLES[key]


def hand_bench_multi(pd, gt, root_joint, is_right, with_fscore=True, counts=False):
    from .ops_names import HAND_BENCH_F_THRESH
    n, S, P, _ = pd.shape
    assert pd.shape == (n, S, P, 3) and gt.shape == (n, P, 3) and root_joint.shape == (n, 3) and is_right.shape == (n,)
    if P > HAND_BENCH_MAX_POINTS or P < 3:
        raise VphoError(f'hand_bench_multi: {P} points per hand, the kernel takes 3 .. {HAND_BENCH_MAX_POINTS}')
    if n * S > 0x7fffffff:
        raise VphoError(f'hand_bench_multi: {n} x {S} pairs, at most 2^31 - 1 in one call')
    values = _new((n, S, 6), pd, torch.float64)
    cnt = _new((n, S, 10), pd, torch.int32) if counts else None
    if n * S > 0:
        t, g = hand_bench_tables(pd.device)
        flag = is_right.to(device=pd.device, dtype=torch.uint8).contiguous()
        _call('vpho_hand_bench_multi_f32', _f32(pd), _f32(gt), _f32(root_joint), _u8(flag), I(n), I(S), I(P), C.c_double(HAND_BENCH_F_THRESH[0]),
              C.c_double(HAND_BENCH_F_THRESH[1]), _f64(t), _f64(g), I(t.shape[0]), I(1 if with_fscore else 0), _f64(values),
              _i32(cnt) if counts else None)
    return (values, cnt) if counts else values


def hand_bench_table(per):
    n, S, k = per.shape
    assert k == 8 and S > 0
    one, best, mean = (_new((n, 8), per, torch.float64) for _ in range(3))
    if n > 0:
        _call('vpho_hand_bench_table_f64', _f64(per), I(n), I(S), _f64(one), _f64(best), _f64(mean))
    return one, best, mean


def obj_9d_to_rt(pose9, root_joint):
    n = pose9.shape[0]
    rt = _new((n, 3, 4), pose9, torch.float64)
    _call('vpho_obj_9d_to_rt_f64', _f64(pose9), _f32(root_joint), I(n), _f64(rt))
    return rt


def infer_record_dtype(n_joint=21, n_vert=778):
    import numpy as np
    size = lib.vpho_infer_record_bytes(I(n_joint), I(n_vert))
    if size < 0:
        raise VphoError(f'vpho_infer_record_bytes: n_joint = {n_joint}, n_vert = {n_vert} (both positive, n_vert even)')
    a = 24 * (n_joint + n_vert)
    return np.dtype({'names': ['reg_joint', 'reg_vert', 'agg_joint', 'agg_vert', 'agg_vert_f16', 'pd_obj_rt'],
                     'formats': [('<f4', (n_joint, 3)), ('<f4', (n_vert, 3)), ('<f4', (n_joint, 3)), ('<f4', (n_vert, 3)), ('<f2', (n_vert, 3)),
                                 ('<f8', (3, 4))],
                     'offsets': [0, 12 * n_joint, 12 * (n_joint + n_vert), 12 * (2 * n_joint + n_vert), a, size - 96], 'itemsize': size})


class InferPacker:

    def __init__(self, device, max_batch, slots=3, n_joint=21, n_vert=778):
        self.device, self.max_batch, self.slots = torch.device(device), int(max_batch), int(slots)
        self.n_joint, self.n_vert = n_joint, n_vert
        self.dtype = infer_record_dtype(n_joint, n_vert)
# ... 644 lines not shown
```

Baseline: 2223 images/s.

## Fuse prior scaling into ODE init, add padded resize and fused metric-row kernel

Scaling of the ODE prior noise by sigma moves out of separate torch ops and into the state-init kernel through a new vpho_ode_sample_prior entry point. A bilinear-resize kernel that also zero-fills padding channels is added, along with a single kernel that computes the per-image hand metric rows: post-processing transform, MPJPE, PA-MPJPE and the object translation norm. Host-side dtype and flag conversions are replaced with helpers that skip copies when a tensor is already in the right form. Together these cut small kernel launches and temporaries, at the cost of more custom code paths to keep numerically equivalent.

Result: no change. 2229 images/s, median of 6 (+0.3%).

```diff
diff --git a/include/vpho_hip.h b/include/vpho_hip.h
--- a/include/vpho_hip.h
+++ b/include/vpho_hip.h
@@ -92,12 +92,19 @@
                     void* xs_out, int xs_is_f64, void* x_out, int x_is_f64,
                     void* workspace, long long workspace_bytes,
                     vpho_ode_stats* stats_host, double* step_log_host, int step_log_cap, void* stream);
+VPHO_API int vpho_ode_sample_prior(const vpho_score_weights* w, const float* feat_img, int bs, int S, const float* prior, double sigma,
+                    double T0, double eps, int num_steps, double rtol, double atol,
+                    void* xs_out, int xs_is_f64, void* x_out, int x_is_f64,
+                    void* workspace, long long workspace_bytes,
+                    vpho_ode_stats* stats_host, double* step_log_host, int step_log_cap, void* stream);
 
 VPHO_API int vpho_nchw_to_nhwc_f32(const float* x, int N, int C, int H, int W, float* y, int ldy, void* stream);
 VPHO_API int vpho_nhwc_to_nchw_f32(const float* x, int N, int H, int W, int C, int ldx, float* y, void* stream);
 VPHO_API int vpho_maxpool_nhwc_f32(const float* x, int N, int H, int W, int C, int k, int stride, int pad, float* y, void* stream);
 VPHO_API int vpho_resize_bilinear_nhwc_f32(const float* x, int N, int H, int W, int C, int ldx, int OH, int OW,
                                   float* y, int ldy, int c_off, int accumulate, void* stream);
+VPHO_API int vpho_resize_bilinear_pad_nhwc_f32(const float* x, int N, int H, int W, int C, int ldx, int OH, int OW,
+                                      float* y, int ldy, int c_off, int c_end, void* stream);
 VPHO_API int vpho_roi_align_nhwc_f32(const float* feat, int N, int H, int W, int C, const float* boxes, float spatial_scale,
                             int out_size, const unsigned char* flip_w, float* out, int ldo, int c_off, void* stream);
 VPHO_API int vpho_roi_windows_i32(const float* boxes_a, const float* boxes_b, int N, int H, int W, float spatial_scale, int dilate,
@@ -182,6 +189,12 @@
 
 VPHO_API int vpho_hand_metrics_f32(const float* pd, const float* gt, int n_img, int n_pts, float* mean_err, float* pa_mean_err,
                           float* per_point, void* stream);
+
+VPHO_API int vpho_metric_rows_base_f32(const float* reg_joint, const float* agg_joint, const float* agg_vert, const float* first_joint,
+                              long long first_stride, const float* root_joint, const unsigned char* is_right, const float* gt_joint,
+                              const float* gt_vert, const void* agg_obj_9d, int obj_is_f64, const float* first_ids, long long first_index,
+                              int n_img, int n_joint, int n_vert, float* rows, long long pitch, int row_cols, float* agg_vert_out,
+                              void* stream);
 
 typedef struct vpho_obj_metric_tables {
     const double* bbox3d;
diff --git a/vpho_amd/csrc/metrics.hip b/vpho_amd/csrc/metrics.hip
--- a/vpho_amd/csrc/metrics.hip
+++ b/vpho_amd/csrc/metrics.hip
@@ -24,21 +24,29 @@
     return r;
 }
 
-__global__ __launch_bounds__(256) void hand_metrics_kernel(const float* __restrict__ pd, const float* __restrict__ gt, int n,
-                                                           float* __restrict__ mean_err, float* __restrict__ pa_mean_err,
-                                                           float* __restrict__ per_point) {
-    __shared__ double red[256];
-    __shared__ double T[12];
-    const int b = blockIdx.x, tid = threadIdx.x;
-    const float* A = pd + (long long)b * n * 3;
-    const float* B = gt + (long long)b * n * 3;
+struct PlainPts {
+    const float* p;
+    __device__ float operator()(int i, int c) const { return p[i * 3 + c]; }
+};
+struct PostPts {
+    const float* p; float sg, r0, r1, r2;
+    __device__ float operator()(int i, int c) const {
+        const float v = p[i * 3 + c];
+        return c == 0 ? v * sg + r0 : v + (c == 1 ? r1 : r2);
+    }
+};
+
+template <class Pts>
+__device__ inline void hand_metrics_pair(const Pts& A, const float* __restrict__ B, int n, double* red, double* T, float* __restrict__ per_point,
+                                         double& me_out, double& pa_out) {
+    const int tid = threadIdx.x;
     double sa[3] = {0, 0, 0}, sb[3] = {0, 0, 0}, se = 0;
     for (int i = tid; i < n; i += 256) {
         double d2 = 0;
-        for (int c = 0; c < 3; ++c) { sa[c] += A[i * 3 + c]; sb[c] += B[i * 3 + c]; const double d = (double)B[i * 3 + c] - A[i * 3 + c]; d2 += d * d; }
+        for (int c = 0; c < 3; ++c) { sa[c] += A(i, c); sb[c] += B[i * 3 + c]; const double d = (double)B[i * 3 + c] - A(i, c); d2 += d * d; }
         const double e = sqrt(d2);
         se += e;
-        if (per_point) per_point[(long long)b * n + i] = (float)e;
+        if (per_point) per_point[i] = (float)e;
     }
     double cA[3], cB[3];
     for (int c = 0; c < 3; ++c) { cA[c] = block_sum(sa[c], red) / n; cB[c] = block_sum(sb[c], red) / n; }
@@ -46,7 +54,7 @@
     double h[9] = {0}, va = 0;
     for (int i = tid; i < n; i += 256) {
         double a[3], bb[3];
-        for (int c = 0; c < 3; ++c) { a[c] = A[i * 3 + c] - cA[c]; bb[c] = B[i * 3 + c] - cB[c]; va += a[c] * a[c]; }
+        for (int c = 0; c < 3; ++c) { a[c] = A(i, c) - cA[c]; bb[c] = B[i * 3 + c] - cB[c]; va += a[c] * a[c]; }
         for (int r = 0; r < 3; ++r) for (int c = 0; c < 3; ++c) h[r * 3 + c] += a[r] * bb[c];
     }
     double H[3][3];
@@ -86,14 +94,82 @@
     for (int i = tid; i < n; i += 256) {
         double d2 = 0;
         for (int r = 0; r < 3; ++r) {
-            const double al = T[r * 3] * A[i * 3] + T[r * 3 + 1] * A[i * 3 + 1] + T[r * 3 + 2] * A[i * 3 + 2] + T[9 + r];
+            const double al = T[r * 3] * A(i, 0) + T[r * 3 + 1] * A(i, 1) + T[r * 3 + 2] * A(i, 2) + T[9 + r];
             const double d = (double)B[i * 3 + r] - al;
             d2 += d * d;
         }
         sp += sqrt(d2);
     }
-    const double pa = block_sum(sp, red) / n;
-    if (tid == 0) { mean_err[b] = (float)me; pa_mean_err[b] = (float)pa; }
+    pa_out = block_sum(sp, red) / n;
+    me_out = me;
+}
+
+__global__ __launch_bounds__(256) void hand_metrics_kernel(const float* __restrict__ pd, const float* __restrict__ gt, int n,
+                                                           float* __restrict__ mean_err, float* __restrict__ pa_mean_err,
+                                                           float* __restrict__ per_point) {
+    __shared__ double red[256];
+    __shared__ double T[12];
+    const int b = blockIdx.x;
+    double me, pa;
+    hand_metrics_pair(PlainPts{pd + (long long)b * n * 3}, gt + (long long)b * n * 3, n, red, T,
+                      per_point ? per_point + (long long)b * n : nullptr, me, pa);
+    if (threadIdx.x == 0) { mean_err[b] = (float)me; pa_mean_err[b] = (float)pa; }
+}
+
+struct MetricRowArgs {
+    const float *reg_joint, *agg_joint, *agg_vert, *first_joint; long long first_stride;
+    const float *root; const unsigned char* is_right; const float *gt_joint, *gt_vert;
+    const void* obj9; int obj_is_f64;
+    const float* first_ids; long long first_index;
+    int n_joint, n_vert, row_cols; long long pitch;
+    float* rows; float* agg_vert_out;
+};
+
+__global__ __launch_bounds__(256) void metric_rows_base_kernel(const MetricRowArgs a) {
+    __shared__ double red[256];
+    __shared__ double T[12];
+    const int b = blockIdx.x, tid = threadIdx.x, J = a.n_joint, V = a.n_vert;
+    const float sg = a.is_right[b] ? 1.f : -1.f, r0 = a.root[b * 3], r1 = a.root[b * 3 + 1], r2 = a.root[b * 3 + 2];
+    const PostPts regJ{a.reg_joint + (long long)b * J * 3, sg, r0, r1, r2}, aggJ{a.agg_joint + (long long)b * J * 3, sg, r0, r1, r2};
+    const PostPts aggV{a.agg_vert + (long long)b * V * 3, sg, r0, r1, r2}, firstJ{a.first_joint + (long long)b * a.first_stride, sg, r0, r1, r2};
+    const float* gtJ = a.gt_joint + (long long)b * J * 3;
+    const float* gtV = a.gt_vert + (long long)b * V * 3;
+    if (a.agg_vert_out)
+        for (int i = tid; i < V * 3; i += 256) a.agg_vert_out[(long long)b * V * 3 + i] = aggV(i / 3, i % 3);
+    double e_first = 0, e_ar = 0;
+    if (tid < 64) {
+        for (int i = tid; i < J; i += 64) {
+            double d1 = 0, d2 = 0;
+            for (int c = 0; c < 3; ++c) {
+                const double u = (double)firstJ(i, c) - gtJ[i * 3 + c], v = (double)aggJ(i, c) - regJ(i, c);
+                d1 += u * u; d2 += v * v;
+            }
+            e_first += sqrt(d1); e_ar += sqrt(d2);
+        }
+        e_first = wave_sum(e_first) / J; e_ar = wave_sum(e_ar) / J;
+    }
+    double me_reg, pa_reg, me_agg, pa_agg, me_v, pa_v;
+    hand_metrics_pair(regJ, gtJ, J, red, T, nullptr, me_reg, pa_reg);
+    hand_metrics_pair(aggJ, gtJ, J, red, T, nullptr, me_agg, pa_agg);
+    hand_metrics_pair(aggV, gtV, V, red, T, nullptr, me_v, pa_v);
+    float* row = a.rows + (long long)b * a.pitch;
+    for (int c = 11 + tid; c < a.row_cols; c += 256) row[c] = 0.f;
+    if (tid == 0) {
+        double t[3];
+        for (int c = 0; c < 3; ++c)
+            t[c] = a.obj_is_f64 ? (double)(float)((const double*)a.obj9)[(long long)b * 9 + 6 + c] : (double)((const float*)a.obj9)[(long long)b * 9 + 6 + c];
+        row[0] = a.first_ids ? a.first_ids[b] : (float)(a.first_index + b);
+        row[1] = (float)(me_reg * 1000.0);
+        row[2] = (float)(e_first * 1000.0);
+        row[3] = (float)(me_agg * 1000.0);
+        row[4] = (float)(me_v * 1000.0);
+        row[5] = (float)(e_ar * 1000.0);
+        row[6] = (float)sqrt((t[0] * t[0] + t[1] * t[1]) + t[2] * t[2]);
+        row[7] = a.is_right[b] ? 1.f : 0.f;
+        row[8] = (float)pa_reg * 1000.f;
+        row[9] = (float)pa_agg * 1000.f;
+        row[10] = (float)pa_v * 1000.f;
+    }
 }
 
 __global__ void obj_9d_to_rt_kernel(const double* __restrict__ pose9, const float* __restrict__ root, int n, double* __restrict__ rt) {
@@ -552,6 +628,25 @@
     return vpho::check_launch("hand_metrics_kernel");
 }
 
+extern "C" int vpho_metric_rows_base_f32(const float* reg_joint, const float* agg_joint, const float* agg_vert, const float* first_joint,
+                                         long long first_stride, const float* root_joint, const unsigned char* is_right, const float* gt_joint,
+                                         const float* gt_vert, const void* agg_obj_9d, int obj_is_f64, const float* first_ids, long long first_index,
+                                         int n_img, int n_joint, int n_vert, float* rows, long long pitch, int row_cols, float* agg_vert_out,
+                                         void* stream) {
+    VPHO_REQUIRE(reg_joint && agg_joint && agg_vert && first_joint && root_joint && is_right && gt_joint && gt_vert && agg_obj_9d && rows,
+                 "vpho_metric_rows_base_f32: bad argument");
+    VPHO_REQUIRE(n_img > 0 && n_joint >= 3 && n_vert >= 3 && row_cols >= 11 && pitch >= row_cols && first_stride >= (long long)n_joint * 3,
+                 "vpho_metric_rows_base_f32: bad shape (n_img %d, %d joints, %d vertices, %d columns, pitch %lld, stride %lld)", n_img, n_joint,
+                 n_vert, row_cols, pitch, first_stride);
+    MetricRowArgs a;
+    a.reg_joint = reg_joint; a.agg_joint = agg_joint; a.agg_vert = agg_vert; a.first_joint = first_joint; a.first_stride = first_stride;
+    a.root = root_joint; a.is_right = is_right; a.gt_joint = gt_joint; a.gt_vert = gt_vert; a.obj9 = agg_obj_9d; a.obj_is_f64 = obj_is_f64;
+    a.first_ids = first_ids; a.first_index = first_index; a.n_joint = n_joint; a.n_vert = n_vert; a.row_cols = row_cols; a.pitch = pitch;
+    a.rows = rows; a.agg_vert_out = agg_vert_out;
+    hipLaunchKernelGGL(metric_rows_base_kernel, dim3(n_img), dim3(256), 0, (hipStream_t)stream, a);
+    return vpho::check_launch("metric_rows_base_kernel");
+}
+
 extern "C" long long vpho_obj_metrics_workspace_bytes(const vpho_obj_metric_tables* t, int n_img, int max_verts) {
     if (!t || n_img <= 0 || max_verts <= 0 || t->n_sampled <= 0) return -1;
     return obj_carve(n_img, t->n_sampled, max_verts, nullptr).bytes;
diff --git a/vpho_amd/csrc/misc.hip b/vpho_amd/csrc/misc.hip
--- a/vpho_amd/csrc/misc.hip
+++ b/vpho_amd/csrc/misc.hip
@@ -97,6 +97,27 @@
         o[u] = accumulate ? (o[u] + v) : v;
     }
     stv<V>(op, o);
+}
+
+__global__ void resize_bilinear_pad_nhwc_kernel(const float* __restrict__ x, int N, int H, int W, int C, int ldx, int OH, int OW,
+                                                float* __restrict__ y, int ldy, int c_off, int CP) {
+    const long long i = (long long)blockIdx.x * blockDim.x + threadIdx.x;
+    if (i >= (long long)N * OH * OW * CP) return;
+    const int c = (int)(i % CP);
+    long long p = i / CP;
+    const int ox = (int)(p % OW); p /= OW;
+    const int oy = (int)(p % OH);
+    const long long n = p / OH;
+    float* op = y + ((n * OH + oy) * OW + ox) * (long long)ldy + c_off + c;
+    if (c >= C) { *op = 0.f; return; }
+    int y0, y1, x0, x1; float ly, lx;
+    lin_src(oy, (float)H / (float)OH, H, y0, y1, ly);
+    lin_src(ox, (float)W / (float)OW, W, x0, x1, lx);
+    const float hy = 1.f - ly, hx = 1.f - lx;
+    const float* b = x + n * H * W * (long long)ldx + c;
+    const float a00 = b[((long long)y0 * W + x0) * ldx], a01 = b[((long long)y0 * W + x1) * ldx];
+    const float a10 = b[((long long)y1 * W + x0) * ldx], a11 = b[((long long)y1 * W + x1) * ldx];
+    *op = hy * (hx * a00 + lx * a01) + ly * (hx * a10 + lx * a11);
 }
 
 struct RoiWin { int base, y0, x0, w, h; };
@@ -539,6 +560,15 @@
     return vpho::check_launch("resize_bilinear_nhwc_kernel");
 }
 
+extern "C" int vpho_resize_bilinear_pad_nhwc_f32(const float* x, int N, int H, int W, int C, int ldx, int OH, int OW,
+                                                 float* y, int ldy, int c_off, int c_end, void* stream) {
+    VPHO_REQUIRE(x && y && N > 0 && C > 0 && H > 0 && W > 0 && OH > 0 && OW > 0 && ldx >= C && c_off >= 0 && c_end >= c_off + C && ldy >= c_end,
+                 "vpho_resize_bilinear_pad_nhwc_f32: bad argument");
+    vpho::ProfScope prof(vpho::PROF_RESIZE, (hipStream_t)stream, 0.0, 4.0 * N * ((double)C * H * W + (double)OH * OW * (c_end - c_off)));
+    LAUNCH1D(resize_bilinear_pad_nhwc_kernel, (long long)N * OH * OW * (c_end - c_off), stream, x, N, H, W, C, ldx, OH, OW, y, ldy, c_off, c_end - c_off);
+    return vpho::check_launch("resize_bilinear_pad_nhwc_kernel");
+}
+
 extern "C" int vpho_resize_bilinear_rows_nhwc_f32(const float* x, int N, int H, int W, int C, int ldx, int OH, int OW, float* y, int ldy, int c_off,
                                                   int accumulate, const int* row_map, const int* row_count, int rows_hint, void* stream) {
     VPHO_REQUIRE(x && y && row_map && row_count && N > 0 && H > 0 && W > 0 && C > 0 && OH > 0 && OW > 0 && ldx >= C && ldy >= c_off + C && c_off >= 0,
diff --git a/vpho_amd/csrc/score_ode.hip b/vpho_amd/csrc/score_ode.hip
--- a/vpho_amd/csrc/score_ode.hip
+++ b/vpho_amd/csrc/score_ode.hip
@@ -1060,14 +1060,15 @@
     if (ynew) ynew[e] = v;
 }
 
-__global__ void f32_to_state_kernel(const float* __restrict__ x, long long n_el, int D, int Dp, double* __restrict__ y, float* __restrict__ X) {
+__global__ void f32_to_state_kernel(const float* __restrict__ x, long long n_el, int D, int Dp, double* __restrict__ y, float* __restrict__ X,
+                                    float scale, int scaled) {
     const long long i = (long long)blockIdx.x * blockDim.x + threadIdx.x;
     const long long R = n_el / D;
     if (i >= R * Dp) return;
     const long long r = i / Dp;
     const int c = (int)(i - r * Dp);
     if (c >= D) { X[i] = 0.f; return; }
-    const float v = x[r * D + c];
+    const float v = scaled ? x[r * D + c] * scale : x[r * D + c];
     y[r * D + c] = (double)v;
     X[i] = v;
 }
@@ -1353,6 +1354,7 @@
 
 struct Ctx {
     const vpho_score_weights* w; Workspace ws; int bs, S; long long R, n_el; int NH; hipStream_t s;
+    float init_scale = 1.f; int init_scaled = 0;
 };
 
 int prepare_cimg(Ctx& c, const float* feat_img) {
@@ -1556,7 +1558,7 @@
     VPHO_HIP(hipMemsetAsync(c.ws.nan_count, 0, 4, c.s));
     if (int e = prepare_cimg(c, feat_img)) return e;
     const int nb = (int)((c.R * w->Dp + 255) / 256);
-    hipLaunchKernelGGL(f32_to_state_kernel, dim3(nb), dim3(256), 0, c.s, x, c.n_el, w->D, w->Dp, c.ws.y, c.ws.X);
+    hipLaunchKernelGGL(f32_to_state_kernel, dim3(nb), dim3(256), 0, c.s, x, c.n_el, w->D, w->Dp, c.ws.y, c.ws.X, 1.f, 0);
     return eval_net(c, c.ws.X, t, 0, 0.f, out);
 }
 
@@ -1576,7 +1578,7 @@
     if (int e = prepare_cimg(c, feat_img)) return e;
     double* y = c.ws.y;
     double* ynew = c.ws.ynew;
-    hipLaunchKernelGGL(f32_to_state_kernel, dim3(nbX), dim3(256), 0, c.s, init_x, n_el, D, Dp, y, c.ws.X);
+    hipLaunchKernelGGL(f32_to_state_kernel, dim3(nbX), dim3(256), 0, c.s, init_x, n_el, D, Dp, y, c.ws.X, c.init_scale, c.init_scaled);
 
     std::vector<double> te(num_steps);
     {
@@ -1750,7 +1752,7 @@
     RkSetup su{T0, eps, rtol, atol, g_scale, num_steps, CTL_LOG_CAP, c.ws.te, c.ws.dense_p, c.ws.log};
     hipLaunchKernelGGL(rk_setup_kernel, dim3(1), dim3(1), 0, c.s, ctl, su);
     if (int e = prepare_cimg(c, feat_img)) return e;
-    hipLaunchKernelGGL(f32_to_state_kernel, dim3(nbX), dim3(256), 0, c.s, init_x, n_el, D, Dp, c.ws.y, c.ws.X);
+    hipLaunchKernelGGL(f32_to_state_kernel, dim3(nbX), dim3(256), 0, c.s, init_x, n_el, D, Dp, c.ws.y, c.ws.X, c.init_scale, c.init_scaled);
 
     if (int e = eval_rhs(c, c.ws.X, T0, c.ws.K, -1, nullptr, nullptr, nullptr, nullptr, true)) return e;
     {
@@ -1863,15 +1865,18 @@
 
 }
 
-extern "C" int vpho_ode_sample(const vpho_score_weights* w, const float* feat_img, int bs, int S, const float* init_x,
-                               double T0, double eps, int num_steps, double rtol, double atol,
-                               void* xs_out, int xs_is_f64, void* x_out, int x_is_f64, void* workspace, long long workspace_bytes,
-                               vpho_ode_stats* st, double* step_log, int step_log_cap, void* stream) {
+namespace {
+
+int ode_sample(const vpho_score_weights* w, const float* feat_img, int bs, int S, const float* init_x, float init_scale, int init_scaled,
+               double T0, double eps, int num_steps, double rtol, double atol,
+               void* xs_out, int xs_is_f64, void* x_out, int x_is_f64, void* workspace, long long workspace_bytes,
+               vpho_ode_stats* st, double* step_log, int step_log_cap, void* stream) {
     if (int e = check_weights(w)) return e;
     VPHO_REQUIRE(bs > 0 && S > 0 && num_steps >= 1 && feat_img && init_x && xs_out && x_out && workspace && st, "vpho_ode_sample: bad argument");
     VPHO_REQUIRE(T0 > eps, "vpho_ode_sample: T0 must exceed eps (backward integration)");
     Ctx c;
     c.w = w; c.bs = bs; c.S = S; c.R = (long long)bs * S; c.n_el = c.R * w->D; c.NH = w->nheads * 256; c.s = (hipStream_t)stream;
+    c.init_scale = init_scale; c.init_scaled = init_scaled;
     c.ws = carve(*w, bs, S, (char*)workspace);
     VPHO_REQUIRE(workspace_bytes >= c.ws.bytes, "vpho_ode_sample: workspace %lld < %lld bytes", workspace_bytes, c.ws.bytes);
     memset(st, 0, sizeof(*st));
@@ -1880,3 +1885,21 @@
         return ode_sample_host(c, feat_img, init_x, T0, eps, num_steps, rtol, atol, xs_out, xs_is_f64, x_out, x_is_f64, st, step_log, step_log_cap);
     return ode_sample_device(c, feat_img, init_x, T0, eps, num_steps, rtol, atol, xs_out, xs_is_f64, x_out, x_is_f64, st, step_log, step_log_cap);
 }
+
+}
+
+extern "C" int vpho_ode_sample(const vpho_score_weights* w, const float* feat_img, int bs, int S, const float* init_x,
+                               double T0, double eps, int num_steps, double rtol, double atol,
+                               void* xs_out, int xs_is_f64, void* x_out, int x_is_f64, void* workspace, long long workspace_bytes,
+                               vpho_ode_stats* st, double* step_log, int step_log_cap, void* stream) {
+    return ode_sample(w, feat_img, bs, S, init_x, 1.f, 0, T0, eps, num_steps, rtol, atol, xs_out, xs_is_f64, x_out, x_is_f64, workspace,
+                      workspace_bytes, st, step_log, step_log_cap, stream);
+}
+
+extern "C" int vpho_ode_sample_prior(const vpho_score_weights* w, const float* feat_img, int bs, int S, const float* prior, double sigma,
+                                     double T0, double eps, int num_steps, double rtol, double atol,
+                                     void* xs_out, int xs_is_f64, void* x_out, int x_is_f64, void* workspace, long long workspace_bytes,
+                                     vpho_ode_stats* st, double* step_log, int step_log_cap, void* stream) {
+    return ode_sample(w, feat_img, bs, S, prior, (float)sigma, 1, T0, eps, num_steps, rtol, atol, xs_out, xs_is_f64, x_out, x_is_f64, workspace,
+                      workspace_bytes, st, step_log, step_log_cap, stream);
+}
diff --git a/vpho_amd/evaluate.py b/vpho_amd/evaluate.py
--- a/vpho_amd/evaluate.py
+++ b/vpho_amd/evaluate.py
@@ -207,29 +207,33 @@
         raise ValueError('metric_rows: eval_physics needs the asset tables (object meshes)')
     if assets is None and layout.has('volume'):
         raise ValueError('metric_rows: eval_volume needs the asset tables (object meshes, hand faces)')
-    pp = postprocess(out, data['root_joint'], data['is_right'])
     bs, dev = gt_joint.shape[0], gt_joint.device
     rows = torch.empty((bs, layout.width), device=dev, dtype=torch.float32)
-    if torch.is_tensor(first_index):
-        rows[:, 0] = first_index.to(device=rows.device, dtype=torch.float32).reshape(bs)
-    else:
-        rows[:, 0] = torch.arange(first_index, first_index + bs, device=rows.device, dtype=torch.float32)
-    rows[:, 1] = mje_mm(pp['reg_hand_joint'], gt_joint)
-    rows[:, 2] = mje_mm(pp['first_hand_joint'], gt_joint)
-    rows[:, 3] = mje_mm(pp['agg_hand_joint'], gt_joint)
-    rows[:, 4] = mje_mm(pp['agg_hand_vert'], gt_vert)
-    rows[:, 5] = mje_mm(pp['agg_hand_joint'], pp['reg_hand_joint'])
-    rows[:, 6] = out['agg_obj_6d'][:, 6:].float().norm(dim=-1)
-    rows[:, 7] = data['is_right'].float()
-    rows[:, 8:ROW] = 0.0
     if gt_joint.is_cuda:
         from . import ops
-        c = lambda t: t.float().contiguous()
-        rows[:, 8] = ops.hand_metrics(c(pp['reg_hand_joint']), c(gt_joint))[1] * 1000.0
-        rows[:, 9] = ops.hand_metrics(c(pp['agg_hand_joint']), c(gt_joint))[1] * 1000.0
-        rows[:, 10] = ops.hand_metrics(c(pp['agg_hand_vert']), c(gt_vert))[1] * 1000.0
+        c = ops.f32c
+        pp = {}
+        if layout.has('physics') or layout.has('volume'):
+            pp['agg_hand_vert'] = torch.empty((bs,) + tuple(out['agg_hand_vert'].shape[1:]), device=dev, dtype=torch.float32)
+        ops.metric_rows_base(rows, ROW, c(out['reg_hand_joint']), c(out['agg_hand_joint']), c(out['agg_hand_vert']),
+                             c(out['diff_final_hand_joint'])[:, 0], c(data['root_joint']), data['is_right'], c(gt_joint), c(gt_vert),
+                             out['agg_obj_6d'], first_index, agg_vert_out=pp.get('agg_hand_vert'))
         if assets is not None and 'gt_obj_rt' in data:
             rows[:, OBJ_COL:OBJ_COL + 16] = object_metric_block(out, data, assets).float()
+    else:
+        pp = postprocess(out, data['root_joint'], data['is_right'])
+        if torch.is_tensor(first_index):
+            rows[:, 0] = first_index.to(device=rows.device, dtype=torch.float32).reshape(bs)
+        else:
+            rows[:, 0] = torch.arange(first_index, first_index + bs, device=rows.device, dtype=torch.float32)
+        rows[:, 1] = mje_mm(pp['reg_hand_joint'], gt_joint)
+        rows[:, 2] = mje_mm(pp['first_hand_joint'], gt_joint)
+        rows[:, 3] = mje_mm(pp['agg_hand_joint'], gt_joint)
+        rows[:, 4] = mje_mm(pp['agg_hand_vert'], gt_vert)
+        rows[:, 5] = mje_mm(pp['agg_hand_joint'], pp['reg_hand_joint'])
+        rows[:, 6] = out['agg_obj_6d'][:, 6:].float().norm(dim=-1)
+        rows[:, 7] = data['is_right'].float()
+        rows[:, 8:ROW] = 0.0
     for name, block in (('multi', lambda: multi_hypothesis_block(out, data, gt_joint, gt_vert, assets)),
                         ('physics', lambda: physics_block(pp, out, data, gt_vert, physics_meter(assets, dev))),
                         ('physics_multi', lambda: physics_multi_block(out, data, physics_meter(assets, dev, multi=True))),
diff --git a/vpho_amd/model/engine.py b/vpho_amd/model/engine.py
--- a/vpho_amd/model/engine.py
+++ b/vpho_amd/model/engine.py
@@ -233,10 +233,10 @@
         grouped = self.grouped and self.conv_terms == 0
         self._two_streams = self.feature_streams >= 2 and not grouped
         with ops.conv_split(self.conv_terms):
-            rgb = data['rgb'].float().contiguous()
+            rgb = ops.f32c(data['rgb'])
             bs = rgb.shape[0]
-            f32 = lambda k: data[k].float().contiguous()
-            left_u8 = (~data['is_right'].bool()).to(torch.uint8).contiguous()
+            f32 = lambda k: ops.f32c(data[k])
+            left_u8 = ops.not_flag_u8(data['is_right'])
             bb_h, bb_o, bb_hr, bb_or = f32('bbox_hand'), f32('bbox_obj'), f32('bbox_hand_rect'), f32('bbox_obj_rect')
             win_h = win_o = halo_h = halo_o = None
             if self.roi_window:
@@ -256,7 +256,7 @@
             pose = ops.rot6d_to_axis_angle(ops.linear(h, *hmn['pose'], acc64=a64), 16)
             shape = ops.linear(h, *hmn['shape'], acc64=a64)
             ctx = self.mano.shape(shape)
-            ho3d = data['is_ho3d'].to(torch.uint8).contiguous() if 'is_ho3d' in data else None
+            ho3d = ops.flag_u8(data['is_ho3d']) if 'is_ho3d' in data else None
             reg_vert, reg_joint = self.mano.fk(pose, ctx, 1, True, ho3d)
             tok_h = self._cross(self.cross['hand'], st_h, st_o, grav, left_u8)
             self._join()
@@ -280,7 +280,7 @@
         hand_feat = self._fpn_out('h', c2, p3[:bs], win_h, halo_h)
         obj_feat = self._fpn_out('o', c2, p3[bs:], win_o, halo_o)
         crop = torch.empty((2 * bs, R, R, 256), device=self.dev)
-        enc_in = torch.zeros((2 * bs, R, R, self.g_enc['cin_pad']), device=self.dev)
+        enc_in = torch.empty((2 * bs, R, R, self.g_enc['cin_pad']), device=self.dev)
         in_h, in_o = enc_in[:bs], enc_in[bs:]
         hf_hr = ops.roi_align_nhwc(hand_feat, bb_h, R, 0.25, win=win_h, out=crop[:bs])
         ops.roi_align_nhwc(hand_feat, bb_hr, R, 0.25, out=in_h, win=win_h)
@@ -292,8 +292,8 @@
         up = self._hm_up(crop, self.g_hm, groups=2)
         hm_hand = ops.conv2d_nhwc(up[:bs], *self.hm['hand']['final'])
         hm_obj = ops.conv2d_nhwc(up[bs:], *self.hm['obj']['final'])
-        ops.resize_bilinear_nhwc(ops.align_heatmap_nhwc(hm_hand, bb_h, bb_hr), R, R, out=in_h, c_off=256)
-        ops.resize_bilinear_nhwc(ops.align_heatmap_nhwc(hm_obj, bb_o, bb_or, flip_w=left_u8), R, R, out=in_o, c_off=256)
+        ops.resize_bilinear_pad_nhwc(ops.align_heatmap_nhwc(hm_hand, bb_h, bb_hr), R, R, out=in_h, c_off=256)
+        ops.resize_bilinear_pad_nhwc(ops.align_heatmap_nhwc(hm_obj, bb_o, bb_or, flip_w=left_u8), R, R, out=in_o, c_off=256)
         enc, st = self._encoder(enc_in, self.g_enc, groups=2)
         hand_heatmap, obj_heatmap = ops.nhwc_to_nchw(hm_hand), ops.nhwc_to_nchw(hm_obj)
         return (hand_feat, obj_feat, hf_hr, in_h[..., :self.enc['hand']['cin_pad']], in_o, hm_hand, hm_obj, hand_heatmap, obj_heatmap,
@@ -303,8 +303,8 @@
         (bb_h, bb_o, bb_hr, bb_or), (win_h, win_o, halo_h, halo_o) = bb, win
         bs, R, L = rgb.shape[0], cfg.roi_size, self.layers
         eh, eo = self.enc['hand'], self.enc['obj']
-        in_h = torch.zeros((bs, R, R, eh['cin_pad']), device=self.dev)
-        in_o = torch.zeros((bs, R, R, eo['cin_pad']), device=self.dev)
+        in_h = torch.empty((bs, R, R, eh['cin_pad']), device=self.dev)
+        in_o = torch.empty((bs, R, R, eo['cin_pad']), device=self.dev)
         c2 = self._stem(rgb)
         c4 = torch.empty((2 * bs, c2.shape[1] // 4, c2.shape[2] // 4, L['layer3_h'][-1]['c3'][0].shape[0]), device=c2.device)
         with self._side():
@@ -322,14 +322,14 @@
                 of_or_rect = ops.roi_align_nhwc(obj_feat, bb_or, R, 0.25)
                 ops.roi_align_nhwc(obj_feat, bb_or, R, 0.25, flip_w=left_u8, out=in_o)
             hm_obj = ops.conv2d_nhwc(self._hm_up(of_or_rect, self.hm['obj']), *self.hm['obj']['final'])
-            ops.resize_bilinear_nhwc(ops.align_heatmap_nhwc(hm_obj, bb_o, bb_or, flip_w=left_u8), R, R, out=in_o, c_off=256)
+            ops.resize_bilinear_pad_nhwc(ops.align_heatmap_nhwc(hm_obj, bb_o, bb_or, flip_w=left_u8), R, R, out=in_o, c_off=256)
             enc_o, st_o = self._encoder(in_o, eo)
             obj_heatmap = ops.nhwc_to_nchw(hm_obj)
         hand_feat = self._fpn_out('h', c2, self._top_down(self.fpn, '_h', c5[:bs], c4h, c3h), win_h, halo_h)
         hf_hr = ops.roi_align_nhwc(hand_feat, bb_h, R, 0.25, win=win_h)
         ops.roi_align_nhwc(hand_feat, bb_hr, R, 0.25, out=in_h, win=win_h)
         hm_hand = ops.conv2d_nhwc(self._hm_up(hf_hr, self.hm['hand']), *self.hm['hand']['final'])
-        ops.resize_bilinear_nhwc(ops.align_heatmap_nhwc(hm_hand, bb_h, bb_hr), R, R, out=in_h, c_off=256)
+        ops.resize_bilinear_pad_nhwc(ops.align_heatmap_nhwc(hm_hand, bb_h, bb_hr), R, R, out=in_h, c_off=256)
         enc_h, st_h = self._encoder(in_h, eh)
         hand_heatmap = ops.nhwc_to_nchw(hm_hand)
         self._join()
@@ -444,7 +444,7 @@
         A, M = self.agg, self.mano
         bs = obj_pose.shape[0]
         if mode_hand != DEFAULT_MODE or mode_obj != DEFAULT_MODE:
-            f32 = lambda k: data[k].float().contiguous()
+            f32 = lambda k: ops.f32c(data[k])
             Kmat = f32('cam_intr_crop_flip').view(bs, 9)
             res, dbg = {}, {}
             if mode_hand == DEFAULT_MODE or mode_obj == DEFAULT_MODE:
@@ -456,15 +456,15 @@
                 res.update(hand_agg_mano=mano, hand_agg_vert=vert, hand_agg_joint=joint)
             if mode_obj != DEFAULT_MODE:
                 oid = A.obj_ids(data['obj_name']) if oid is None else oid
-                isr = data['is_right'].to(torch.uint8).contiguous()
+                isr = ops.flag_u8(data['is_right'])
                 res['obj_agg_6d'], dbg['obj_mode'] = self._aggregate_obj_mode(mode_obj, f, obj_pose, f32('root_joint'), oid, isr, Kmat,
                                                                               f32('bbox_obj_rect'), k_obj)
             return res, dbg
-        f32 = lambda k: data[k].float().contiguous()
+        f32 = lambda k: ops.f32c(data[k])
         root_flip, root, Kmat = f32('root_joint_flip'), f32('root_joint'), f32('cam_intr_crop_flip').view(bs, 9)
         bb_h, bb_or = f32('bbox_hand'), f32('bbox_obj_rect')
-        isr = data['is_right'].to(torch.uint8).contiguous()
-        ungrasp = (~data['is_grasped'].bool()).to(torch.uint8).contiguous()
+        isr = ops.flag_u8(data['is_right'])
+        ungrasp = ops.not_flag_u8(data['is_grasped'])
         oid = A.obj_ids(data['obj_name']) if oid is None else oid
         ctx = f['mano_ctx']
         dbg = dict(hand_topk=[], hand_val=[])
@@ -529,7 +529,7 @@
             sig = 0.01 * (50 / 0.01) ** T0
             init_h = self._prior(bs * S, 96) if noise_hand is None else noise_hand.float()
             init_o = self._prior(bs * S, 9) if noise_obj is None else noise_obj.float()
-            init_h, init_o = init_h.to(self.dev, non_blocking=True) * sig, init_o.to(self.dev, non_blocking=True) * sig
+            init_h, init_o = init_h.to(self.dev, non_blocking=True).contiguous(), init_o.to(self.dev, non_blocking=True).contiguous()
             out = dict(reg_hand_vert=keep(f['reg_hand_vert']), reg_hand_joint=keep(f['reg_hand_joint']), hand_heatmap=keep(f['hand_heatmap']),
                        obj_heatmap=keep(f['obj_heatmap']), force_local=keep(f['force_local']))
             main = torch.cuda.current_stream()
@@ -540,11 +540,11 @@
 
             def run_obj():
                 with torch.cuda.device(self.dev), torch.cuda.stream(obj_stream):
-                    return self.score_obj.sample(f['encoding_obj'], init_o, S, T0, steps, xs_f64=True, x_f64=True)
+                    return self.score_obj.sample(f['encoding_obj'], init_o, S, T0, steps, xs_f64=True, x_f64=True, prior_sigma=sig)
 
             concurrent = os.environ.get('VPHO_SERIAL_SAMPLERS', '0') != '1' and not self.serial_samplers
             fut = self._obj_worker.submit(run_obj) if concurrent else None
-            xs_h, x_h, st_h = self.score_hand.sample(f['encoding_hand'], init_h, S, T0, steps, xs_f64=False, x_f64=False)
+            xs_h, x_h, st_h = self.score_hand.sample(f['encoding_hand'], init_h, S, T0, steps, xs_f64=False, x_f64=False, prior_sigma=sig)
             inproc = torch.empty((bs * S * steps, 58), device=self.dev)
             ops.rot6d_to_axis_angle(xs_h.view(bs * S * steps, 96), 16, out=inproc)
             ops.append_betas(f['mano_shape'], inproc, S * steps)
diff --git a/vpho_amd/ops.py b/vpho_amd/ops.py
--- a/vpho_amd/ops.py
+++ b/vpho_amd/ops.py
@@ -436,6 +436,9 @@
 lib.vpho_ode_sample.argtypes = [C.POINTER(ScoreWeights), C.c_void_p, C.c_int, C.c_int, C.c_void_p, C.c_double, C.c_double,
                                 C.c_int, C.c_double, C.c_double, C.c_void_p, C.c_int, C.c_void_p, C.c_int, C.c_void_p, C.c_longlong,
                                 C.POINTER(OdeStats), C.c_void_p, C.c_int, C.c_void_p]
+lib.vpho_ode_sample_prior.argtypes = [C.POINTER(ScoreWeights), C.c_void_p, C.c_int, C.c_int, C.c_void_p, C.c_double, C.c_double, C.c_double,
+                                      C.c_int, C.c_double, C.c_double, C.c_void_p, C.c_int, C.c_void_p, C.c_int, C.c_void_p, C.c_longlong,
+                                      C.POINTER(OdeStats), C.c_void_p, C.c_int, C.c_void_p]
 
 
 class ScoreNet:
@@ -494,7 +497,7 @@
                                    _ptr(out), _ptr(ws), ws.numel(), _stream()))
         return out
 
-    def sample(self, feat_img, init_x, S, T0, num_steps, xs_f64, x_f64=True, eps=1e-5, rtol=3e-3, atol=3e-4, log_cap=4096):
+    def sample(self, feat_img, init_x, S, T0, num_steps, xs_f64, x_f64=True, eps=1e-5, rtol=3e-3, atol=3e-4, log_cap=4096, prior_sigma=None):
         bs = feat_img.shape[0]
         R = bs * S
         assert init_x.shape == (R, self.D)
@@ -503,10 +506,13 @@
         x = torch.empty((R, self.D), device=self.device, dtype=torch.float64 if x_f64 else torch.float32)
         st = OdeStats()
         log = (C.c_double * (4 * log_cap))()
-        _check(lib.vpho_ode_sample(C.byref(self.c), _ptr(feat_img, torch.float32), bs, S, _ptr(init_x, torch.float32),
-                                   float(T0), float(eps), int(num_steps), float(rtol), float(atol), _ptr(xs),
-                                   1 if xs_f64 else 0, _ptr(x), 1 if x_f64 else 0, _ptr(ws), ws.numel(), C.byref(st), log, log_cap,
-                                   _stream()))
+        tail = (float(T0), float(eps), int(num_steps), float(rtol), float(atol), _ptr(xs), 1 if xs_f64 else 0, _ptr(x), 1 if x_f64 else 0,
+                _ptr(ws), ws.numel(), C.byref(st), log, log_cap, _stream())
+        if prior_sigma is None:
+            _check(lib.vpho_ode_sample(C.byref(self.c), _ptr(feat_img, torch.float32), bs, S, _ptr(init_x, torch.float32), *tail))
+        else:
+            _check(lib.vpho_ode_sample_prior(C.byref(self.c), _ptr(feat_img, torch.float32), bs, S, _ptr(init_x, torch.float32),
+                                             float(prior_sigma), *tail))
         n = min(st.n_log, log_cap)
         steps = [(log[4 * i], log[4 * i + 1], log[4 * i + 2], bool(log[4 * i + 3])) for i in range(n)]
         return xs, x, dict(nfev=st.nfev, n_accepted=st.n_accepted, n_rejected=st.n_rejected, nan_count=st.nan_count,
@@ -578,6 +584,15 @@
         return out
     _call('vpho_resize_bilinear_nhwc_f32', _f32(x), I(N), I(H), I(W), I(Cc), I(ldx), I(OH), I(OW), _f32(out), I(out.shape[-1]),
           I(c_off), I(1 if accumulate else 0))
+    return out
+
+
+def resize_bilinear_pad_nhwc(x, OH, OW, out, c_off, channels=None):
+    N, H, W, ldx = x.shape
+    Cc = ldx if channels is None else channels
+    assert out.shape[:3] == (N, OH, OW)
+    _call('vpho_resize_bilinear_pad_nhwc_f32', _f32(x), I(N), I(H), I(W), I(Cc), I(ldx), I(OH), I(OW), _f32(out), I(out.shape[-1]),
+          I(c_off), I(out.shape[-1]))
     return out
 
 
@@ -951,6 +966,48 @@
     pp = _new((n, P), pd) if per_point else None
     _call('vpho_hand_metrics_f32', _f32(pd), _f32(gt), I(n), I(P), _f32(me), _f32(pa), _f32(pp))
     return (me, pa, pp) if per_point else (me, pa)
+
+
+def flag_u8(flag, device=None):
+    if device is not None and flag.device != torch.device(device):
+        flag = flag.to(device)
+    if flag.dtype == torch.uint8 and flag.is_contiguous():
+        return flag
+    if flag.dtype == torch.bool and flag.is_contiguous():
+        return flag.view(torch.uint8)
+    return flag.to(torch.uint8).contiguous()
+
+
+def not_flag_u8(flag):
+    return torch.logical_not(flag).contiguous().view(torch.uint8)
+
+
+def f32c(t):
+    return t if t.dtype == torch.float32 and t.is_contiguous() else t.float().contiguous()
+
+
+def metric_rows_base(rows, row_cols, reg_joint, agg_joint, agg_vert, first_joint, root_joint, is_right, gt_joint, gt_vert, agg_obj_9d,
+                     first_index, agg_vert_out=None):
+    n, J, _ = reg_joint.shape
+    V = agg_vert.shape[1]
+    assert rows.dtype == torch.float32 and rows.dim() == 2 and rows.shape[0] == n and rows.stride(1) == 1 and rows.shape[1] >= row_cols
+    assert agg_joint.shape == gt_joint.shape == first_joint.shape == (n, J, 3) and agg_vert.shape == gt_vert.shape == (n, V, 3)
+    assert root_joint.shape == (n, 3) and is_right.shape == (n,) and agg_obj_9d.shape == (n, 9)
+    assert first_joint.dtype == torch.float32 and first_joint[0].is_contiguous() and first_joint.is_cuda and rows.is_cuda
+    if n > 1 and first_joint.stride(0) < J * 3:
+        first_joint = first_joint.contiguous()
+    stride = first_joint.stride(0) if n > 1 else J * 3
+    obj = agg_obj_9d if agg_obj_9d.dtype == torch.float64 else f32c(agg_obj_9d)
+    if torch.is_tensor(first_index):
+        ids, first = first_index.to(device=rows.device, dtype=torch.float32).reshape(n).contiguous(), 0
+    else:
+        ids, first = None, int(first_index)
+    if agg_vert_out is not None:
+        assert agg_vert_out.shape == (n, V, 3)
+    _call('vpho_metric_rows_base_f32', _f32(reg_joint), _f32(agg_joint), _f32(agg_vert), C.c_void_p(first_joint.data_ptr()), LL(stride),
+          _f32(root_joint), _u8(flag_u8(is_right, rows.device)), _f32(gt_joint), _f32(gt_vert), _ptr(obj), I(1 if obj.dtype == torch.float64 else 0),
+          _f32(ids), LL(first), I(n), I(J), I(V), _f32(rows), LL(rows.stride(0)), I(row_cols), _f32(agg_vert_out))
+    return rows
 
 
 def hand_metrics_multi(pd, gt, root_joint, is_right):
```
